# alshai/rowbowt

Hardware: AMD Instinct MI355X
Metric: reads/s (100 bp, count+locate) (higher is better)
Workload: dtype u32/u64

## Files before the change

### include/rbg.h

```cpp
#ifndef RBG_H
#define RBG_H

#include <stddef.h>
#include <stdint.h>

#ifdef __cplusplus
extern "C" {
#endif

#define RBG_ABI_VERSION 3

typedef struct rbg_index rbg_index;

enum { RBG_LOAD_NONE = 0, RBG_LOAD_SA = 1, RBG_LOAD_MA = 2, RBG_LOAD_DL = 4, RBG_LOAD_FT = 8 };

enum {
    RBG_OK = 0,
    RBG_EIO = -1,
    RBG_EFORMAT = -2,
    RBG_ENODEV = -3,
    RBG_EARG = -4,
    RBG_ENOMEM = -5,
    RBG_ENOTLOADED = -6
};

#define RBG_DEVICE_NONE (-1)

int rbg_abi_version(void);
const char *rbg_strerror(int code);


int rbg_load(const char *prefix, int flags, int device, rbg_index **out);

int rbg_build_from_runs(const uint8_t *heads, const uint64_t *lens, uint64_t R,
                        const uint64_t *ssa_y, const uint64_t *esa_y, int device, rbg_index **out);

int rbg_build_from_files(const char *bwt_fname, const char *ssa_fname, const char *esa_fname, int device,
                         rbg_index **out);

int rbg_convert_index(const char *prefix, int flags, const char *out_path);
int rbg_convert_raw(const char *bwt_fname, const char *ssa_fname, const char *esa_fname, const char *mab_fname,
                    const char *docs_fname, const char *out_path);
int rbg_load_cache(const char *path, int flags, int device, rbg_index **out);
int rbg_convert_runs(const uint8_t *heads, const uint64_t *lens, uint64_t R, const uint64_t *ssa_y ,
                     const uint64_t *esa_y, const char *out_path);
int rbg_convert_runs_markers(const uint8_t *heads, const uint64_t *lens, uint64_t R, const uint64_t *ssa_y, const uint64_t *esa_y,
                             const uint64_t *mk_start, const uint64_t *mk_end, uint64_t mk_nruns, const uint64_t *mk_off,
                             const uint64_t *mk_vals, const char *docs_text , const char *out_path);
int rbg_write_ftab(rbg_index *, uint64_t k, const char *path);
int rbg_check_ftab(rbg_index *, const char *path, uint64_t *k_out);
int rbg_set_markers(rbg_index *, const uint64_t *run_start, const uint64_t *run_end, uint64_t nruns,
                    const uint64_t *mk_off, const uint64_t *mk_vals);
int rbg_set_text_markers(rbg_index *, const uint64_t *run_start, const uint64_t *run_end, uint64_t nruns,
                         const uint64_t *mk_off, const uint64_t *mk_vals);
int rbg_load_text_markers(rbg_index *, const char *path);
int rbg_set_docs(rbg_index *, const char *names_joined, const uint64_t *starts, uint64_t ndocs);

void rbg_free(rbg_index *);


typedef struct rbg_info_t {
    uint64_t n;
    uint64_t r;
    uint32_t sigma;
    uint32_t pos_bytes;
    int32_t device;
    uint32_t has_tsa, has_markers, has_docs;
    uint64_t hbm_bytes;
    uint64_t marker_runs, marker_vals;
    uint32_t rank_bucket_shift, phi_bucket_shift;
    uint32_t slot_bytes;
    uint64_t rank_slots, rank_slots_overflow, phi_slots, phi_slots_overflow;
    uint64_t kmer_steps, kmer_symbols, pair_runs, triple_runs, quad_runs;
    uint64_t ftab_k;
    uint64_t quint_runs;
    uint64_t kmer_steps_requested, hbm_free_at_load, hbm_budget;
    uint64_t rank_layout;
    uint64_t replicas;
    uint64_t depth_runs[8];
} rbg_info_t;
enum { RBG_LAYOUT_AUTO = 0, RBG_LAYOUT_SLOTS = 1, RBG_LAYOUT_RUNS = 2, RBG_LAYOUT_PREFER_SLOTS = 3 };
int rbg_info(const rbg_index *, rbg_info_t *out);
int rbg_info_sized(const rbg_index *, rbg_info_t *out, uint64_t out_bytes);

typedef struct rbg_layout_info_t {
    uint32_t run_fmt;
    uint32_t depths_composed;
    uint32_t depth_mask_asked;
    uint32_t depth_mask_kept;
    uint32_t depths_dropped_budget;
    uint32_t rank_directories;
    uint32_t phi_directory;
    uint32_t fill_shift;
    uint64_t entries[8];
    uint64_t fillers[8];
    uint64_t dir_bytes[8];
    uint64_t phi_entries, phi_fillers, phi_dir_bytes, phi_dir_shift;
    uint64_t phi_slots, phi_slot_bytes;
    uint64_t rec_bytes[8];
    uint64_t rec_overflow[8];
    uint64_t budget_raised;
} rbg_layout_info_t;
int rbg_layout_info(const rbg_index *, rbg_layout_info_t *out, uint64_t out_bytes);

typedef struct rbg_jump_info_t {
    uint64_t k;
    uint64_t keys;
    uint64_t bytes;
    uint64_t buckets;
    double build_ms;
} rbg_jump_info_t;
int rbg_jump_info(const rbg_index *, rbg_jump_info_t *out);

int rbg_get_f(const rbg_index *, uint64_t f_out[256]);
int rbg_last_run_sample(const rbg_index *, uint64_t *out);

enum {
    RBG_ARR_RUN_HEADS = 0,
    RBG_ARR_RUN_START = 1,
    RBG_ARR_SAMPLES_LAST = 2,
    RBG_ARR_PRED_POS = 3,
    RBG_ARR_PHI_BASE = 4,
    RBG_ARR_MARKER_START = 5, RBG_ARR_MARKER_END = 6, RBG_ARR_MARKER_OFF = 7, RBG_ARR_MARKER_VALS = 8
};
int rbg_host_array(const rbg_index *, int which, uint64_t *dst, uint64_t cap, uint64_t *count);


int rbg_lf(rbg_index *, const uint64_t *lo, const uint64_t *hi, const uint8_t *sym, uint64_t N,
           uint64_t *lo_out, uint64_t *hi_out);
int rbg_find_range(rbg_index *, const uint8_t *seqs, const uint64_t *off, uint64_t N,
                   uint64_t *lo, uint64_t *hi);
int rbg_count(rbg_index *, const uint8_t *seqs, const uint64_t *off, uint64_t N, uint64_t *count);
int rbg_find_range_spans(rbg_index *, const uint8_t *base, const uint64_t *begin, const uint32_t *len, uint64_t N,
                         uint64_t *lo, uint64_t *hi, uint64_t *ssamp );

int rbg_find_range_w_toehold(rbg_index *, const uint8_t *seqs, const uint64_t *off, uint64_t N,
                             uint64_t *lo, uint64_t *hi, uint64_t *ssamp);
int rbg_locs_at(rbg_index *, const uint64_t *lo, const uint64_t *hi, const uint64_t *k, uint64_t N,
                uint64_t max_hits, uint64_t *loc_off, uint64_t **locs);
int rbg_markers_at(rbg_index *, const uint64_t *lo, const uint64_t *hi, uint64_t N,
                   uint64_t *mk_off, uint64_t **mk);
int rbg_find_range_w_markers(rbg_index *, const uint8_t *seqs, const uint64_t *off, uint64_t N,
                             uint64_t wsize, uint64_t max_range,
                             uint64_t *lo, uint64_t *hi, uint64_t *mk_off, uint64_t **mk);
typedef struct rbg_marker_seed {
    uint64_t lo, hi;
    uint64_t qstart;
    uint64_t qend;
    uint64_t mk_begin;
    uint64_t mk_end;
} rbg_marker_seed_t;
int rbg_get_markers_greedy_seeding(rbg_index *, const uint8_t *seqs, const uint64_t *off, uint64_t N,
                                   uint64_t wsize, uint64_t max_range, uint64_t ftab_k,
                                   uint64_t *seed_off, rbg_marker_seed_t **seeds, uint64_t **mk);
int rbg_get_markers_lmems(rbg_index *, const uint8_t *seqs, const uint64_t *off, uint64_t N,
                          uint64_t wsize, uint64_t max_range, uint64_t ftab_k,
                          uint64_t *seed_off, rbg_marker_seed_t **seeds, uint64_t **mk);
int rbg_greedy_longest_seed(rbg_index *, const uint8_t *seqs, const uint64_t *off, uint64_t N, uint64_t min_length,
                            uint64_t *lo, uint64_t *hi, uint64_t *qstart, uint64_t *qend, uint64_t *ssamp);
#define RBG_SEEDS_W_SAMPLE 1u
int rbg_get_seeds_greedy(rbg_index *, const uint8_t *seqs, const uint64_t *off, uint64_t N, uint64_t min_length, uint32_t flags,
                         uint64_t *seed_off, uint64_t **seeds);
int rbg_find_range_w_toehold_chkpnts(rbg_index *, const uint8_t *seqs, const uint64_t *off, uint64_t N, uint64_t wsize,
                                     uint64_t *seed_off, uint64_t **seeds);
int rbg_find_locs_greedy_seeding(rbg_index *, const uint8_t *seqs, const uint64_t *off, uint64_t N, uint64_t min_length,
                                 uint64_t max_hits, uint64_t *loc_off, uint64_t **locs);
int rbg_markers_at_locs(rbg_index *, const uint64_t *locs, const uint64_t *loc_off, const uint64_t *off, uint64_t N,
                        uint64_t *mk_off, uint64_t **mk);
int rbg_find_loc_markers_greedy_seeding(rbg_index *, const uint8_t *seqs, const uint64_t *off, uint64_t N, uint64_t min_length,
                                        uint64_t max_hits, uint64_t *loc_off, uint64_t **locs, uint64_t *mk_off, uint64_t **mk);
void rbg_free_buffer(void *);

int rbg_resolve_offset(const rbg_index *, uint64_t i, const char **name, uint64_t *offset);
int rbg_doc_table(rbg_index *, uint64_t *ndocs, const uint64_t **sorted_starts, const char *const **names, uint64_t *size);

enum { RBG_TEXT_MARKERS = 1 };
int rbg_align_text(rbg_index *, const uint64_t *lo, const uint64_t *hi, const uint64_t *k, uint64_t N, uint64_t max_hits, uint32_t flags,
                   const char *name_base, const uint64_t *name_begin, const uint32_t *name_len, const char **text, uint64_t *text_len);
int rbg_wait_text(rbg_index *, const char *text);
int rbg_release_text(rbg_index *, const char *text);
int rbg_reserve_text(rbg_index *, uint64_t bytes, int count);
#define RBG_SAM_SECONDARY 1u
int rbg_align_sam(rbg_index *, const char *seq_base, const uint64_t *seq_begin, const uint32_t *seq_len,
                  const char *qual_base , const uint64_t *qual_begin ,
                  const char *name_base, const uint64_t *name_begin, const uint32_t *name_len, uint64_t N,
                  uint64_t min_length, uint64_t max_hits, uint32_t flags, const char **text, uint64_t *text_len);
#define RBG_SAM_MAX_MISMATCH 8
int rbg_align_sam_extend(rbg_index *, const char *seq_base, const uint64_t *seq_begin, const uint32_t *seq_len,
                         const char *qual_base , const uint64_t *qual_begin ,
                         const char *name_base, const uint64_t *name_begin, const uint32_t *name_len, uint64_t N,
                         uint64_t min_length, uint64_t max_hits, uint32_t flags, uint32_t max_mismatch, const char **text, uint64_t *text_len);
typedef struct rbg_extend_t {
    uint32_t ext, nm;
    int32_t score;
    uint32_t steps;
    uint32_t mis_t[8];
    uint8_t mis_ref[8];
} rbg_extend_t;
int rbg_extend_left_dev(rbg_index *, const uint8_t *d_seqs, const uint64_t *d_off, uint64_t N, const uint32_t *d_item_seq ,
                        const uint32_t *d_item_a , const uint64_t *d_item_row , const uint64_t *d_item_limit , uint64_t M,
                        uint32_t max_mismatch, rbg_extend_t *d_out , void *stream);
int rbg_fl_prepare(rbg_index *);
int rbg_fl_info(const rbg_index *, uint64_t out[8]);
int rbg_fl_dev(rbg_index *, const uint64_t *d_rows, uint64_t M, uint8_t *d_sym, uint64_t *d_next, void *stream);
int rbg_extend_right_dev(rbg_index *, const uint8_t *d_seqs, const uint64_t *d_off, uint64_t N, const uint32_t *d_item_seq ,
                         const uint32_t *d_item_b , const uint64_t *d_item_row , const uint32_t *d_item_skip ,
                         const uint64_t *d_item_limit , uint64_t M, uint32_t max_mismatch, rbg_extend_t *d_out , void *stream);
int rbg_align_sam_extend_both(rbg_index *, const char *seq_base, const uint64_t *seq_begin, const uint32_t *seq_len,
                              const char *qual_base , const uint64_t *qual_begin, const char *name_base, const uint64_t *name_begin,
                              const uint32_t *name_len, uint64_t N, uint64_t min_length, uint64_t max_hits, uint32_t flags, uint32_t max_mismatch,
                              const char **text, uint64_t *text_len);
int rbg_sam_header(rbg_index *, const char *pg_line , char **text, uint64_t *text_len);
int rbg_extract_prepare(rbg_index *);
int rbg_extract_info(const rbg_index *, uint64_t out[8]);
int rbg_isa_dev(rbg_index *, const uint64_t *d_pos, uint64_t M, uint64_t *d_row, void *stream);
int rbg_isa(rbg_index *, const uint64_t *pos, uint64_t M, uint64_t *row);
int rbg_extract_dev(rbg_index *, const uint64_t *d_pos, const uint32_t *d_len, const uint64_t *d_out_off, uint64_t M, uint8_t *d_out ,
                    uint32_t *d_got , void *stream);
int rbg_extract(rbg_index *, const uint64_t *pos, const uint64_t *len, uint64_t M, uint8_t *out, uint64_t *got);
size_t rbg_sa_tmp_bytes(uint64_t n, uint32_t pos_bytes);
int rbg_suffix_array_dev(const uint8_t *d_text, uint64_t n, void *d_sa, uint32_t pos_bytes, void *d_tmp, size_t tmp_bytes, void *stream);
int rbg_sa_info(uint64_t out[8]);
size_t rbg_text_runs_tmp_bytes(uint64_t n, uint32_t pos_bytes);
int rbg_text_runs_plan_dev(const uint8_t *d_text, const void *d_sa, uint64_t n, uint32_t pos_bytes, void *d_tmp, size_t tmp_bytes, uint64_t *R, void *stream);
int rbg_text_runs_fill_dev(const uint8_t *d_text, const void *d_sa, uint64_t n, uint32_t pos_bytes, const void *d_tmp, size_t tmp_bytes, uint64_t R,
                           uint8_t *d_heads, uint64_t *d_lens, uint64_t *d_ssa, uint64_t *d_esa, void *stream);
int rbg_build_from_text(const uint8_t *text, uint64_t n, int flags, int device, rbg_index **out);
int rbg_convert_text(const uint8_t *text, uint64_t n, const char *docs_text , int flags, int device, const char *out_path);
#define RBG_REPORT_LMEM 1u
#define RBG_REPORT_HEURISTIC 2u
#define RBG_REPORT_BEST_STRAND 4u
#define RBG_REPORT_CLEAR_CONFLICTING 8u
#define RBG_REPORT_CLEAR_IDENTICAL 16u
typedef struct rbg_report_params {
    uint64_t wsize, max_range, min_range, ftab_k, read_len, min_seed_len;
    uint32_t flags;
} rbg_report_params_t;
typedef struct rbg_report_seed { uint64_t range_size, query_start, query_len, mk_begin, mk_end; uint32_t strand , pad; } rbg_report_seed_t;
int rbg_markers_report(rbg_index *, const uint8_t *seqs, const uint64_t *off, uint64_t N, const uint8_t *first_fwd ,
                       const rbg_report_params_t *params, uint64_t *seed_off, rbg_report_seed_t **seeds, uint64_t **mk);
int rbg_markers_report_text(rbg_index *, const uint8_t *seqs, const uint64_t *off, uint64_t N, const uint8_t *first_fwd ,
                            const rbg_report_params_t *params, const char *name_base, const uint64_t *name_begin, const uint32_t *name_len,
                            const char **text, uint64_t *text_len);
#define RBG_TALLY_PER_READ 1u
#define RBG_TALLY_DROP_SITE_CONFLICTS 2u
typedef struct rbg_tally rbg_tally;
typedef struct rbg_tally_entry { uint64_t marker, n_fwd, n_rev, len_sum; } rbg_tally_entry_t;
int rbg_tally_create(rbg_index *, uint64_t distinct_hint, rbg_tally **out);
void rbg_tally_free(rbg_tally *);
int rbg_tally_reset(rbg_tally *);
int rbg_tally_reserve(rbg_tally *, uint64_t extra);
size_t rbg_tally_add_tmp_bytes(uint64_t R);
int rbg_tally_add_dev(rbg_tally *, const rbg_report_seed_t *d_recs, uint64_t R, const uint64_t *d_mk, uint64_t M_upper, void *d_tmp, size_t tmp_bytes,
                      void *stream);
int rbg_markers_tally(rbg_index *, const uint8_t *seqs, const uint64_t *off, uint64_t N, const uint8_t *first_fwd ,
                      const rbg_report_params_t *params, rbg_tally *);
int rbg_tally_add_entries(rbg_tally *, const rbg_tally_entry_t *entries, uint64_t count);
int rbg_tally_export(rbg_tally *, uint64_t *count, rbg_tally_entry_t **entries);
int rbg_tally_info(rbg_tally *, uint64_t out[6]);
int rbg_markers_tally_reads(rbg_index *, const uint8_t *seqs, const uint64_t *off, uint64_t N, const uint8_t *first_fwd ,
                            const rbg_report_params_t *params, uint32_t tally_flags, rbg_tally *);
size_t rbg_tally_add_reads_tmp_bytes(uint64_t N, uint64_t R);
int rbg_tally_add_reads_dev(rbg_tally *, const rbg_report_seed_t *d_recs, uint64_t R, const uint64_t *d_rep_off , uint64_t N,
                            const uint64_t *d_mk, uint64_t M_upper, uint32_t tally_flags, void *d_tmp, size_t tmp_bytes, void *stream);
int rbg_tally_read_info(rbg_tally *, uint64_t out[4]);

int rbg_find_range_dev(rbg_index *, const uint8_t *d_seqs, const uint64_t *d_off, uint64_t N,
                       uint64_t *d_lo, uint64_t *d_hi, void *stream);
int rbg_find_range_w_toehold_dev(rbg_index *, const uint8_t *d_seqs, const uint64_t *d_off, uint64_t N,
                                 uint64_t *d_lo, uint64_t *d_hi, uint64_t *d_ssamp, void *stream);
size_t rbg_pack_ws_bytes(uint64_t N, uint64_t total_bytes);
int rbg_pack_reads_dev(rbg_index *, const uint8_t *d_seqs, const uint64_t *d_off, uint64_t N, uint64_t total_bytes,
                       void *d_ws, size_t ws_bytes, void *stream);
int rbg_find_range_packed_dev(rbg_index *, const void *d_ws, const uint8_t *d_seqs, const uint64_t *d_off, uint64_t N,
                              uint64_t total_bytes, uint64_t *d_lo, uint64_t *d_hi, void *stream);
int rbg_find_range_w_toehold_packed_dev(rbg_index *, const void *d_ws, const uint8_t *d_seqs, const uint64_t *d_off, uint64_t N,
                                        uint64_t total_bytes, uint64_t *d_lo, uint64_t *d_hi, uint64_t *d_ssamp, void *stream);
size_t rbg_locate_plan_tmp_bytes(uint64_t N);
int rbg_locate_plan_dev(rbg_index *, const uint64_t *d_lo, const uint64_t *d_hi, uint64_t N, uint64_t max_hits,
                        uint64_t *d_loc_off, void *d_tmp, size_t tmp_bytes, void *stream);
size_t rbg_locate_order_ws_bytes(uint64_t N);
int rbg_locate_order_dev(rbg_index *, const uint64_t *d_k, uint64_t N, void *d_ws, size_t ws_bytes, void *stream);
int rbg_locate_fill_dev(rbg_index *, const uint64_t *d_lo, const uint64_t *d_hi, const uint64_t *d_k, uint64_t N,
                        uint64_t max_hits, const uint64_t *d_loc_off, uint64_t *d_locs, const void *d_order, void *stream);
int rbg_locate_fill_dev32(rbg_index *, const uint64_t *d_lo, const uint64_t *d_hi, const uint64_t *d_k, uint64_t N,
                          uint64_t max_hits, const uint64_t *d_loc_off, uint32_t *d_locs32, const void *d_order, void *stream);
int rbg_locate_fill_offset_dev(rbg_index *, const uint64_t *d_lo, const uint64_t *d_hi, const uint64_t *d_k, uint64_t N,
                               uint64_t max_hits, const uint64_t *d_loc_off, uint64_t *d_locs, const uint64_t *d_sub,
                               const void *d_order, void *stream);
int rbg_greedy_longest_seed_dev(rbg_index *, const uint8_t *d_seqs, const uint64_t *d_off, uint64_t N, uint64_t min_length,
                                uint64_t *d_lo, uint64_t *d_hi, uint64_t *d_qstart, uint64_t *d_qend, uint64_t *d_ssamp,
                                void *stream);
int rbg_marker_seeds_plan_dev(rbg_index *, const uint8_t *d_seqs, const uint64_t *d_off, uint64_t N, uint64_t wsize,
                              uint64_t max_range, uint64_t ftab_k, uint64_t *d_seed_off, uint64_t *d_mk_off, void *d_tmp, size_t tmp_bytes,
                              void *stream);
int rbg_marker_seeds_fill_dev(rbg_index *, const uint8_t *d_seqs, const uint64_t *d_off, uint64_t N, uint64_t wsize,
                              uint64_t max_range, uint64_t ftab_k, const uint64_t *d_seed_off, const uint64_t *d_mk_off,
                              rbg_marker_seed_t *d_seeds, uint64_t *d_mk, void *stream);
size_t rbg_marker_seeds_log_bytes(const rbg_index *, uint64_t N, uint32_t seeds_per_read);
int rbg_marker_seeds_plan_log_dev(rbg_index *, const uint8_t *d_seqs, const uint64_t *d_off, uint64_t N, uint64_t wsize,
                                  uint64_t max_range, uint64_t ftab_k, uint64_t *d_seed_off, uint64_t *d_mk_off, void *d_tmp,
                                  size_t tmp_bytes, void *d_log, size_t log_bytes, void *stream);
int rbg_marker_seeds_fill_log_dev(rbg_index *, const uint8_t *d_seqs, const uint64_t *d_off, uint64_t N, uint64_t wsize,
                                  uint64_t max_range, uint64_t ftab_k, const uint64_t *d_seed_off, const uint64_t *d_mk_off,
                                  rbg_marker_seed_t *d_seeds, uint64_t *d_mk, void *d_log, size_t log_bytes, void *stream);
size_t rbg_marker_lmems_tmp_bytes(uint64_t N, uint64_t total);
int rbg_marker_lmems_plan_dev(rbg_index *, const uint8_t *d_seqs, const uint64_t *d_off, uint64_t N, uint64_t total, uint64_t wsize,
                              uint64_t max_range, uint64_t ftab_k, uint64_t *d_mk_off, void *d_tmp, size_t tmp_bytes, void *stream);
int rbg_marker_lmems_fill_dev(rbg_index *, const uint8_t *d_seqs, const uint64_t *d_off, uint64_t N, uint64_t total, uint64_t wsize,
                              uint64_t max_range, uint64_t ftab_k, const void *d_tmp, rbg_marker_seed_t *d_seeds, uint64_t *d_mk, void *stream);
size_t rbg_greedy_seeds_tmp_bytes(uint64_t N);
int rbg_greedy_seeds_plan_dev(rbg_index *, const uint8_t *d_seqs, const uint64_t *d_off, uint64_t N, uint64_t min_length, uint32_t flags,
                              uint64_t *d_seed_off, void *d_tmp, size_t tmp_bytes, void *stream);
int rbg_greedy_seeds_fill_dev(rbg_index *, const uint8_t *d_seqs, const uint64_t *d_off, uint64_t N, uint64_t min_length, uint32_t flags,
                              const uint64_t *d_seed_off, uint64_t *d_lo, uint64_t *d_hi, uint64_t *d_qstart, uint64_t *d_qend,
                              uint64_t *d_ssamp, void *stream);
size_t rbg_toehold_chkpnts_tmp_bytes(uint64_t N);
int rbg_toehold_chkpnts_slots_dev(rbg_index *, const uint64_t *d_off, uint64_t N, uint64_t wsize, uint64_t *d_slot_off, void *d_tmp,
                                  size_t tmp_bytes, void *stream);
int rbg_find_range_w_toehold_chkpnts_dev(rbg_index *, const uint8_t *d_seqs, const uint64_t *d_off, uint64_t N, uint64_t wsize,
                                         const uint64_t *d_slot_off, uint64_t *d_cnt, uint64_t *d_lo, uint64_t *d_hi,
                                         uint64_t *d_qstart, uint64_t *d_qend, uint64_t *d_ssamp, void *stream);
size_t rbg_read_strands_bytes(uint64_t total_bytes);
int rbg_read_strands_dev(rbg_index *, const uint8_t *d_seqs, const uint64_t *d_off, uint64_t N, uint64_t total_bytes, uint8_t *d_seqs2, uint64_t *d_off2,
                         void *stream);
size_t rbg_marker_seeds_canon_tmp_bytes(uint64_t S);
int rbg_marker_seeds_canon_dev(rbg_index *, rbg_marker_seed_t *d_seeds, uint64_t S, uint64_t *d_mk, uint64_t min_range, uint32_t flags, uint64_t read_len,
                               void *d_tmp, size_t tmp_bytes, void *stream);
size_t rbg_report_select_tmp_bytes(uint64_t N);
int rbg_report_select_dev(rbg_index *, const rbg_marker_seed_t *d_seeds, const uint64_t *d_seed_off, const uint64_t *d_off2, uint64_t N,
                          const uint8_t *d_first_fwd, const rbg_report_params_t *params, uint64_t *d_rep_off, rbg_report_seed_t *d_out,
                          uint32_t *d_out_read, void *d_tmp, size_t tmp_bytes, void *stream);
int rbg_markers_plan_dev(rbg_index *, const uint64_t *d_lo, const uint64_t *d_hi, uint64_t N,
                         uint64_t *d_mk_off, void *d_tmp, size_t tmp_bytes, void *stream);
int rbg_markers_fill_dev(rbg_index *, const uint64_t *d_lo, const uint64_t *d_hi, uint64_t N,
                         const uint64_t *d_mk_off, uint64_t *d_mk, void *stream);
size_t rbg_loc_markers_tmp_bytes(uint64_t N);
int rbg_loc_markers_plan_dev(rbg_index *, const uint64_t *d_locs, const uint64_t *d_loc_off, const uint64_t *d_off, uint64_t N,
                             uint64_t *d_mk_off, void *d_tmp, size_t tmp_bytes, void *stream);
int rbg_loc_markers_fill_dev(rbg_index *, const uint64_t *d_locs, const uint64_t *d_loc_off, const uint64_t *d_off, uint64_t N,
                             const uint64_t *d_mk_off, uint64_t *d_mk, void *stream);

#define RBG_DOCS_MAX 65536u
#define RBG_DOC_NONE 0xFFFFFFFFu
int rbg_docs_prepare(rbg_index *);
size_t rbg_doc_hits_words(const rbg_index *);
int rbg_resolve_offsets_dev(rbg_index *, const uint64_t *d_locs, uint64_t M, uint32_t *d_doc, uint64_t *d_offset , void *stream);
int rbg_resolve_offsets_dev32(rbg_index *, const uint32_t *d_locs32, uint64_t M, uint32_t *d_doc, uint64_t *d_offset , void *stream);
int rbg_doc_hits_dev(rbg_index *, const uint64_t *d_locs, const uint64_t *d_loc_off, uint64_t N, uint64_t *d_sets ,
                     uint32_t *d_ndocs , uint32_t *d_nodoc , uint64_t *d_doc_reads ,
                     void *stream);
int rbg_doc_hits_dev32(rbg_index *, const uint32_t *d_locs32, const uint64_t *d_loc_off, uint64_t N, uint64_t *d_sets ,
                       uint32_t *d_ndocs , uint32_t *d_nodoc , uint64_t *d_doc_reads ,
                       void *stream);
int rbg_doc_hits(rbg_index *, const uint8_t *seqs, const uint64_t *off, uint64_t N, uint64_t max_hits, uint64_t *lo, uint64_t *hi, uint64_t *sets ,
                 uint32_t *ndocs , uint32_t *nodoc , uint64_t *doc_reads );
#define RBG_LOCATE_DOCS_MAX 1024u
int rbg_locate_doc_hits_dev(rbg_index *, const uint64_t *d_lo, const uint64_t *d_hi, const uint64_t *d_k, uint64_t N, uint64_t max_hits,
                            const void *d_order , uint64_t *d_sets , uint32_t *d_ndocs ,
                            uint32_t *d_nodoc , uint64_t *d_doc_reads ,
                            uint64_t *d_doc_locs , void *stream);
int rbg_doc_hits_locs(rbg_index *, const uint8_t *seqs, const uint64_t *off, uint64_t N, uint64_t max_hits, uint64_t *lo, uint64_t *hi,
                      uint64_t *sets , uint32_t *ndocs , uint32_t *nodoc ,
                      uint64_t *doc_reads , uint64_t *doc_locs );

int rbg_counters(rbg_index *, uint64_t out[4]);
int rbg_counters_reset(rbg_index *);
int rbg_combine_stats(rbg_index *, uint64_t out[2]);

int rbg_replicate(rbg_index *primary, int device, rbg_index **replica_out);
int rbg_replicate_many(rbg_index *primary, const int *devices, int G, rbg_index **replicas_out );
int rbg_replicate_stats(const rbg_index *replica, double out[3]);
int rbg_replica_pointer_check(const rbg_index *replica, uint64_t out[4]);
int rbg_shard_bounds(uint64_t n_items, int rank, int world, uint64_t *begin, uint64_t *end);
int rbg_find_range_sharded(rbg_index *const *replicas, int G, const uint8_t *seqs, const uint64_t *off, uint64_t N,
                           uint64_t *lo, uint64_t *hi, uint64_t *ssamp );
int rbg_counters_allreduce(rbg_index *, void *nccl_comm, void *stream, uint64_t out[4]);
int rbg_counters_allreduce_local(rbg_index *const *replicas, int G, uint64_t out[4]);
int rbg_comm_cache_clear(void);

enum { RBG_SS_STEPS = 0,
       RBG_SS_SLOTS,
       RBG_SS_DENSE,
       RBG_SS_SEARCH,
       RBG_SS_FTAB,
       RBG_SS_RESAMPLE,
       RBG_SS_CHUNKS,
       RBG_SS_SYMBOLS,
       RBG_SEARCH_STATS };
enum { RBG_LS_PHI_STEPS = 0,
       RBG_LS_PHI_SEARCH,
       RBG_LS_CHAINS,
       RBG_LS_LOCS,
       RBG_LOCATE_STATS };
enum { RBG_SD_MARKER_QUERIES = 8,
       RBG_SD_MARKER_DIR,
       RBG_SD_MARKER_PROBES,
       RBG_SD_MARKER_OFF,
       RBG_SD_MARKER_VALS,
       RBG_SD_SEED_RECS,
       RBG_SD_SEQUENCES,
       RBG_SEED_STATS };
int rbg_greedy_longest_seed_stats_dev(rbg_index *, const uint8_t *d_seqs, const uint64_t *d_off, uint64_t N, uint64_t min_length,
                                      uint64_t *d_lo, uint64_t *d_hi, uint64_t *d_qstart, uint64_t *d_qend, uint64_t *d_ssamp,
                                      uint64_t *d_stats , void *stream);
int rbg_marker_seeds_stats_dev(rbg_index *, const uint8_t *d_seqs, const uint64_t *d_off, uint64_t N, uint64_t wsize, uint64_t max_range,
                               uint64_t *d_seed_off, uint64_t *d_mk_off, void *d_tmp, size_t tmp_bytes, rbg_marker_seed_t *d_seeds,
                               uint64_t *d_mk, uint64_t *d_stats , void *stream);
int rbg_find_range_stats_dev(rbg_index *, const uint8_t *d_seqs, const uint64_t *d_off, uint64_t N, uint64_t *d_lo,
                             uint64_t *d_hi, uint64_t *d_ssamp ,
                             uint64_t *d_stats , void *stream);
int rbg_locate_fill_stats_dev(rbg_index *, const uint64_t *d_lo, const uint64_t *d_hi, const uint64_t *d_k, uint64_t N,
                              uint64_t max_hits, const uint64_t *d_loc_off, uint64_t *d_locs, const void *d_order,
                              uint64_t *d_stats , void *stream);

int rbg_sample_reads_dev(const uint8_t *d_text, uint64_t unit, uint64_t H, uint64_t L, uint64_t m, uint64_t seed,
                         uint64_t first_read, uint64_t N, uint32_t sub_ppm, uint8_t *d_seqs, uint64_t *d_off,
                         uint64_t *d_start , void *stream);
int rbg_sample_reads_pangenome_dev(const uint8_t *d_base, const uint64_t *d_sites, const uint8_t *d_alt, const uint8_t *d_G, uint64_t S,
                                   const uint32_t *d_site_dir, uint32_t site_dir_shift, uint64_t unit, uint64_t H, uint64_t L, uint64_t m,
                                   uint64_t seed, uint64_t first_read, uint64_t N, uint32_t sub_ppm, uint8_t *d_seqs, uint64_t *d_off,
                                   uint64_t *d_start , void *stream);

enum { RBG_OPT_BLOCK_THREADS = 1, RBG_OPT_RANK_BUCKET_SHIFT = 2, RBG_OPT_PHI_BUCKET_SHIFT = 3, RBG_OPT_POS_BYTES = 4,
       RBG_OPT_KMER_STEPS = 5, RBG_OPT_HBM_BUDGET_MB = 6, RBG_OPT_FTAB_K = 7, RBG_OPT_PACKED_READS = 8,
       RBG_OPT_DEEP_BUCKET_SHIFT = 9, RBG_OPT_DENSE_OVERFLOW = 10, RBG_OPT_RANK_LAYOUT = 11,
       RBG_OPT_RUN_DEPTHS = 14 ,
       RBG_OPT_RUN_PHI = 16 ,
       RBG_OPT_RUN_REC = 17 ,
       RBG_OPT_RUN_REC_DEPTHS = 18 ,
       RBG_OPT_EXTRACT_CHUNK = 20 ,
       RBG_OPT_JUMP_K = 19  };
int rbg_set_default_option(int opt, int64_t value);
int rbg_get_default_option(int opt, int64_t *value);

#ifdef __cplusplus
}
#endif
#endif
```

### rowbowt_amd/capi.py

```python
import ctypes as C
import enum
import os
import weakref

import numpy as np

_HERE = os.path.dirname(os.path.abspath(__file__))
_SO = os.path.join(_HERE, "librbg.so")

U64 = C.c_uint64
VP = C.c_void_p
MAXU = 2**64 - 1
DEVICE_NONE = -1

OPT_BLOCK_THREADS, OPT_RANK_BUCKET_SHIFT, OPT_PHI_BUCKET_SHIFT, OPT_POS_BYTES, OPT_KMER_STEPS, OPT_HBM_BUDGET_MB, OPT_FTAB_K, OPT_PACKED_READS, OPT_DEEP_BUCKET_SHIFT, OPT_DENSE_OVERFLOW, OPT_RANK_LAYOUT = range(1, 12)
OPT_RUN_DEPTHS, OPT_RUN_PHI, OPT_RUN_REC, OPT_RUN_REC_DEPTHS = 14, 16, 17, 18
OPT_EXTRACT_CHUNK = 20
OPT_JUMP_K = 19
ABI_VERSION = 3
MAX_KMER_DEPTH = 8
LAYOUT_AUTO, LAYOUT_SLOTS, LAYOUT_RUNS, LAYOUT_PREFER_SLOTS = 0, 1, 2, 3
SEEDS_W_SAMPLE = 1
(ARR_RUN_HEADS, ARR_RUN_START, ARR_SAMPLES_LAST, ARR_PRED_POS, ARR_PHI_BASE,
 ARR_MARKER_START, ARR_MARKER_END, ARR_MARKER_OFF, ARR_MARKER_VALS) = range(9)


class LoadRbwtFlag(enum.IntFlag):
    NONE = 0
    SA = 1
    MA = 2
    DL = 4
    FT = 8


class RbgError(RuntimeError):
    def __init__(self, code, what):
        self.code = code
        super().__init__(f"{what}: {lib().rbg_strerror(code).decode()} ({code})")


class Info(C.Structure):
    _fields_ = [("n", U64), ("r", U64), ("sigma", C.c_uint32), ("pos_bytes", C.c_uint32), ("device", C.c_int32),
                ("has_tsa", C.c_uint32), ("has_markers", C.c_uint32), ("has_docs", C.c_uint32),
                ("hbm_bytes", U64), ("marker_runs", U64), ("marker_vals", U64),
                ("rank_bucket_shift", C.c_uint32), ("phi_bucket_shift", C.c_uint32), ("slot_bytes", C.c_uint32),
                ("rank_slots", U64), ("rank_slots_overflow", U64), ("phi_slots", U64), ("phi_slots_overflow", U64),
                ("kmer_steps", U64), ("kmer_symbols", U64), ("pair_runs", U64), ("triple_runs", U64), ("quad_runs", U64), ("ftab_k", U64), ("quint_runs", U64),
                ("kmer_steps_requested", U64), ("hbm_free_at_load", U64), ("hbm_budget", U64), ("rank_layout", U64), ("replicas", U64),
                ("depth_runs", U64 * 8)]


class LayoutInfo(C.Structure):
    _fields_ = [("run_fmt", C.c_uint32), ("depths_composed", C.c_uint32), ("depth_mask_asked", C.c_uint32), ("depth_mask_kept", C.c_uint32),
                ("depths_dropped_budget", C.c_uint32), ("rank_directories", C.c_uint32),
                ("phi_directory", C.c_uint32), ("fill_shift", C.c_uint32),
                ("entries", U64 * 8), ("fillers", U64 * 8), ("dir_bytes", U64 * 8),
                ("phi_entries", U64), ("phi_fillers", U64), ("phi_dir_bytes", U64), ("phi_dir_shift", U64), ("phi_slots", U64), ("phi_slot_bytes", U64), ("rec_bytes", U64 * 8), ("rec_overflow", U64 * 8), ("budget_raised", U64)]


class JumpInfo(C.Structure):
    _fields_ = [("k", U64), ("keys", U64), ("bytes", U64), ("buckets", U64), ("build_ms", C.c_double)]


class ReportParams(C.Structure):
    _fields_ = [(n, U64) for n in ("wsize", "max_range", "min_range", "ftab_k", "read_len", "min_seed_len")] + [("flags", C.c_uint32)]


REPORT_LMEM, REPORT_HEURISTIC, REPORT_BEST_STRAND, REPORT_CLEAR_CONFLICTING, REPORT_CLEAR_IDENTICAL = 1, 2, 4, 8, 16
REPORT_SEED = np.dtype([("range_size", "<u8"), ("query_start", "<u8"), ("query_len", "<u8"), ("mk_begin", "<u8"), ("mk_end", "<u8"),
                        ("strand", "<u4"), ("pad", "<u4")])


TALLY_ENTRY = np.dtype([("marker", "<u8"), ("n_fwd", "<u8"), ("n_rev", "<u8"), ("len_sum", "<u8")])
TALLY_INFO = ("entries", "capacity", "grows", "records", "elements", "dropped")
TALLY_PER_READ, TALLY_DROP_SITE_CONFLICTS = 1, 2
TALLY_READ_INFO = ("reads", "elements_seen", "lost", "site_dropped")
DOCS_MAX = 1 << 16
SAM_MAX_MISMATCH = 8
EXTEND = np.dtype([("ext", np.uint32), ("nm", np.uint32), ("score", np.int32), ("steps", np.uint32), ("mis_t", np.uint32, 8), ("mis_ref", np.uint8, 8)])
SAM_SECONDARY = 1
LOCATE_DOCS_MAX = 1024
DOC_NONE = 0xFFFFFFFF


def report_params(wsize=19, max_range=1000, min_range=0, ftab_k=0, read_len=101, min_seed_len=0, lmem=False, heuristic=False, best_strand=False,
                  clear_conflicting=False, clear_identical=False):
    flags = ((REPORT_LMEM if lmem else 0) | (REPORT_HEURISTIC if heuristic else 0) | (REPORT_BEST_STRAND if best_strand else 0)
             | (REPORT_CLEAR_CONFLICTING if clear_conflicting else 0) | (REPORT_CLEAR_IDENTICAL if clear_identical else 0))
    return ReportParams(wsize, max_range & MAXU, min_range, ftab_k, read_len, min_seed_len, flags)


_PROTOS = [
    ("rbg_abi_version", C.c_int, []),
    ("rbg_strerror", C.c_char_p, [C.c_int]),
    ("rbg_load", C.c_int, [C.c_char_p, C.c_int, C.c_int, C.POINTER(VP)]),
    ("rbg_build_from_runs", C.c_int, [VP, VP, U64, VP, VP, C.c_int, C.POINTER(VP)]),
    ("rbg_build_from_files", C.c_int, [C.c_char_p, C.c_char_p, C.c_char_p, C.c_int, C.POINTER(VP)]),
    ("rbg_convert_index", C.c_int, [C.c_char_p, C.c_int, C.c_char_p]),
    ("rbg_convert_raw", C.c_int, [C.c_char_p, C.c_char_p, C.c_char_p, C.c_char_p, C.c_char_p, C.c_char_p]),
    ("rbg_load_cache", C.c_int, [C.c_char_p, C.c_int, C.c_int, C.POINTER(VP)]),
    ("rbg_doc_table", C.c_int, [VP, C.POINTER(U64), C.POINTER(VP), C.POINTER(VP), C.POINTER(U64)]),
    ("rbg_align_text", C.c_int, [VP, VP, VP, VP, U64, U64, C.c_uint32, VP, VP, VP, C.POINTER(VP), C.POINTER(U64)]),
    ("rbg_wait_text", C.c_int, [VP, VP]),
    ("rbg_release_text", C.c_int, [VP, VP]),
    ("rbg_reserve_text", C.c_int, [VP, U64, C.c_int]),
    ("rbg_convert_runs", C.c_int, [VP, VP, U64, VP, VP, C.c_char_p]),
    ("rbg_convert_runs_markers", C.c_int, [VP, VP, U64, VP, VP, VP, VP, U64, VP, VP, C.c_char_p, C.c_char_p]),
    ("rbg_write_ftab", C.c_int, [VP, U64, C.c_char_p]),
    ("rbg_check_ftab", C.c_int, [VP, C.c_char_p, C.POINTER(U64)]),
    ("rbg_set_markers", C.c_int, [VP, VP, VP, U64, VP, VP]),
    ("rbg_set_docs", C.c_int, [VP, C.c_char_p, VP, U64]),
    ("rbg_free", None, [VP]),
    ("rbg_info", C.c_int, [VP, C.POINTER(Info)]),
    ("rbg_info_sized", C.c_int, [VP, C.POINTER(Info), U64]),
    ("rbg_layout_info", C.c_int, [VP, C.POINTER(LayoutInfo), U64]),
    ("rbg_jump_info", C.c_int, [VP, C.POINTER(JumpInfo)]),
    ("rbg_get_f", C.c_int, [VP, VP]),
    ("rbg_last_run_sample", C.c_int, [VP, C.POINTER(U64)]),
    ("rbg_host_array", C.c_int, [VP, C.c_int, VP, U64, C.POINTER(U64)]),
    ("rbg_lf", C.c_int, [VP, VP, VP, VP, U64, VP, VP]),
    ("rbg_find_range", C.c_int, [VP, VP, VP, U64, VP, VP]),
    ("rbg_count", C.c_int, [VP, VP, VP, U64, VP]),
    ("rbg_find_range_w_toehold", C.c_int, [VP, VP, VP, U64, VP, VP, VP]),
    ("rbg_find_range_spans", C.c_int, [VP, VP, VP, VP, U64, VP, VP, VP]),
    ("rbg_locs_at", C.c_int, [VP, VP, VP, VP, U64, U64, VP, C.POINTER(VP)]),
    ("rbg_markers_at", C.c_int, [VP, VP, VP, U64, VP, C.POINTER(VP)]),
    ("rbg_find_range_w_markers", C.c_int, [VP, VP, VP, U64, U64, U64, VP, VP, VP, C.POINTER(VP)]),
    ("rbg_get_markers_greedy_seeding", C.c_int, [VP, VP, VP, U64, U64, U64, U64, VP, C.POINTER(VP), C.POINTER(VP)]),
    ("rbg_greedy_longest_seed", C.c_int, [VP, VP, VP, U64, U64, VP, VP, VP, VP, VP]),
    ("rbg_find_locs_greedy_seeding", C.c_int, [VP, VP, VP, U64, U64, U64, VP, C.POINTER(VP)]),
    ("rbg_free_buffer", None, [VP]),
    ("rbg_resolve_offset", C.c_int, [VP, U64, C.POINTER(C.c_char_p), C.POINTER(U64)]),
    ("rbg_find_range_dev", C.c_int, [VP, VP, VP, U64, VP, VP, VP]),
    ("rbg_find_range_w_toehold_dev", C.c_int, [VP, VP, VP, U64, VP, VP, VP, VP]),
    ("rbg_pack_ws_bytes", C.c_size_t, [U64, U64]),
    ("rbg_pack_reads_dev", C.c_int, [VP, VP, VP, U64, U64, VP, C.c_size_t, VP]),
    ("rbg_find_range_packed_dev", C.c_int, [VP, VP, VP, VP, U64, U64, VP, VP, VP]),
    ("rbg_find_range_w_toehold_packed_dev", C.c_int, [VP, VP, VP, VP, U64, U64, VP, VP, VP, VP]),
    ("rbg_locate_plan_tmp_bytes", C.c_size_t, [U64]),
    ("rbg_locate_plan_dev", C.c_int, [VP, VP, VP, U64, U64, VP, VP, C.c_size_t, VP]),
    ("rbg_locate_order_ws_bytes", C.c_size_t, [U64]),
    ("rbg_locate_order_dev", C.c_int, [VP, VP, U64, VP, C.c_size_t, VP]),
    ("rbg_locate_fill_dev", C.c_int, [VP, VP, VP, VP, U64, U64, VP, VP, VP, VP]),
    ("rbg_locate_fill_offset_dev", C.c_int, [VP, VP, VP, VP, U64, U64, VP, VP, VP, VP, VP]),
    ("rbg_greedy_longest_seed_dev", C.c_int, [VP, VP, VP, U64, U64, VP, VP, VP, VP, VP, VP]),
    ("rbg_marker_seeds_plan_dev", C.c_int, [VP, VP, VP, U64, U64, U64, U64, VP, VP, VP, C.c_size_t, VP]),
    ("rbg_marker_seeds_fill_dev", C.c_int, [VP, VP, VP, U64, U64, U64, U64, VP, VP, VP, VP, VP]),
    ("rbg_markers_plan_dev", C.c_int, [VP, VP, VP, U64, VP, VP, C.c_size_t, VP]),
    ("rbg_markers_fill_dev", C.c_int, [VP, VP, VP, U64, VP, VP, VP]),
    ("rbg_marker_seeds_log_bytes", C.c_size_t, [VP, U64, C.c_uint32]),
    ("rbg_marker_seeds_plan_log_dev", C.c_int, [VP, VP, VP, U64, U64, U64, U64, VP, VP, VP, C.c_size_t, VP, C.c_size_t, VP]),
    ("rbg_marker_seeds_fill_log_dev", C.c_int, [VP, VP, VP, U64, U64, U64, U64, VP, VP, VP, VP, VP, C.c_size_t, VP]),
    ("rbg_locate_fill_dev32", C.c_int, [VP, VP, VP, VP, U64, U64, VP, VP, VP, VP]),
    ("rbg_greedy_longest_seed_stats_dev", C.c_int, [VP, VP, VP, U64, U64, VP, VP, VP, VP, VP, VP, VP]),
    ("rbg_marker_seeds_stats_dev", C.c_int, [VP, VP, VP, U64, U64, U64, VP, VP, VP, C.c_size_t, VP, VP, VP, VP]),
    ("rbg_find_range_stats_dev", C.c_int, [VP, VP, VP, U64, VP, VP, VP, VP, VP]),
    ("rbg_locate_fill_stats_dev", C.c_int, [VP, VP, VP, VP, U64, U64, VP, VP, VP, VP, VP]),
    ("rbg_sample_reads_dev", C.c_int, [VP, U64, U64, U64, U64, U64, U64, U64, C.c_uint32, VP, VP, VP, VP]),
    ("rbg_sample_reads_pangenome_dev", C.c_int, [VP, VP, VP, VP, U64, VP, C.c_uint32, U64, U64, U64, U64, U64, U64, U64, C.c_uint32, VP, VP, VP, VP]),
    ("rbg_replicate", C.c_int, [VP, C.c_int, C.POINTER(VP)]),
    ("rbg_replicate_many", C.c_int, [VP, C.POINTER(C.c_int), C.c_int, C.POINTER(VP)]),
    ("rbg_replicate_stats", C.c_int, [VP, C.POINTER(C.c_double)]),
    ("rbg_replica_pointer_check", C.c_int, [VP, VP]),
    ("rbg_comm_cache_clear", C.c_int, []),
    ("rbg_shard_bounds", C.c_int, [U64, C.c_int, C.c_int, C.POINTER(U64), C.POINTER(U64)]),
    ("rbg_find_range_sharded", C.c_int, [VP, C.c_int, VP, VP, U64, VP, VP, VP]),
    ("rbg_counters_allreduce", C.c_int, [VP, VP, VP, VP]),
    ("rbg_counters_allreduce_local", C.c_int, [VP, C.c_int, VP]),
    ("rbg_counters", C.c_int, [VP, VP]),
    ("rbg_counters_reset", C.c_int, [VP]),
    ("rbg_combine_stats", C.c_int, [VP, VP]),
    ("rbg_get_markers_lmems", C.c_int, [VP, VP, VP, U64, U64, U64, U64, VP, C.POINTER(VP), C.POINTER(VP)]),
    ("rbg_marker_lmems_tmp_bytes", C.c_size_t, [U64, U64]),
    ("rbg_marker_lmems_plan_dev", C.c_int, [VP, VP, VP, U64, U64, U64, U64, U64, VP, VP, C.c_size_t, VP]),
    ("rbg_marker_lmems_fill_dev", C.c_int, [VP, VP, VP, U64, U64, U64, U64, U64, VP, VP, VP, VP]),
    ("rbg_get_seeds_greedy", C.c_int, [VP, VP, VP, U64, U64, C.c_uint32, VP, C.POINTER(VP)]),
    ("rbg_greedy_seeds_tmp_bytes", C.c_size_t, [U64]),
    ("rbg_greedy_seeds_plan_dev", C.c_int, [VP, VP, VP, U64, U64, C.c_uint32, VP, VP, C.c_size_t, VP]),
    ("rbg_greedy_seeds_fill_dev", C.c_int, [VP, VP, VP, U64, U64, C.c_uint32, VP, VP, VP, VP, VP, VP, VP]),
    ("rbg_find_range_w_toehold_chkpnts", C.c_int, [VP, VP, VP, U64, U64, VP, C.POINTER(VP)]),
    ("rbg_toehold_chkpnts_tmp_bytes", C.c_size_t, [U64]),
    ("rbg_toehold_chkpnts_slots_dev", C.c_int, [VP, VP, U64, U64, VP, VP, C.c_size_t, VP]),
    ("rbg_find_range_w_toehold_chkpnts_dev", C.c_int, [VP, VP, VP, U64, U64, VP, VP, VP, VP, VP, VP, VP, VP]),
    ("rbg_set_text_markers", C.c_int, [VP, VP, VP, U64, VP, VP]),
    ("rbg_load_text_markers", C.c_int, [VP, C.c_char_p]),
    ("rbg_loc_markers_tmp_bytes", C.c_size_t, [U64]),
    ("rbg_loc_markers_plan_dev", C.c_int, [VP, VP, VP, VP, U64, VP, VP, C.c_size_t, VP]),
    ("rbg_loc_markers_fill_dev", C.c_int, [VP, VP, VP, VP, U64, VP, VP, VP]),
    ("rbg_markers_at_locs", C.c_int, [VP, VP, VP, VP, U64, VP, C.POINTER(VP)]),
    ("rbg_find_loc_markers_greedy_seeding", C.c_int, [VP, VP, VP, U64, U64, U64, VP, C.POINTER(VP), VP, C.POINTER(VP)]),
    ("rbg_read_strands_bytes", C.c_size_t, [U64]),
    ("rbg_read_strands_dev", C.c_int, [VP, VP, VP, U64, U64, VP, VP, VP]),
    ("rbg_marker_seeds_canon_tmp_bytes", C.c_size_t, [U64]),
    ("rbg_marker_seeds_canon_dev", C.c_int, [VP, VP, U64, VP, U64, C.c_uint32, U64, VP, C.c_size_t, VP]),
    ("rbg_report_select_tmp_bytes", C.c_size_t, [U64]),
    ("rbg_report_select_dev", C.c_int, [VP, VP, VP, VP, U64, VP, VP, VP, VP, VP, VP, C.c_size_t, VP]),
    ("rbg_markers_report", C.c_int, [VP, VP, VP, U64, VP, VP, VP, C.POINTER(VP), C.POINTER(VP)]),
    ("rbg_markers_report_text", C.c_int, [VP, VP, VP, U64, VP, VP, VP, VP, VP, C.POINTER(VP), C.POINTER(U64)]),
    ("rbg_tally_create", C.c_int, [VP, U64, C.POINTER(VP)]),
    ("rbg_tally_free", None, [VP]),
    ("rbg_tally_reset", C.c_int, [VP]),
    ("rbg_tally_reserve", C.c_int, [VP, U64]),
    ("rbg_tally_add_tmp_bytes", C.c_size_t, [U64]),
    ("rbg_tally_add_dev", C.c_int, [VP, VP, U64, VP, U64, VP, C.c_size_t, VP]),
    ("rbg_markers_tally", C.c_int, [VP, VP, VP, U64, VP, VP, VP]),
    ("rbg_tally_add_entries", C.c_int, [VP, VP, U64]),
    ("rbg_tally_export", C.c_int, [VP, C.POINTER(U64), C.POINTER(VP)]),
    ("rbg_tally_info", C.c_int, [VP, VP]),
    ("rbg_markers_tally_reads", C.c_int, [VP, VP, VP, U64, VP, VP, C.c_uint32, VP]),
    ("rbg_tally_add_reads_tmp_bytes", C.c_size_t, [U64, U64]),
    ("rbg_tally_add_reads_dev", C.c_int, [VP, VP, U64, VP, U64, VP, U64, C.c_uint32, VP, C.c_size_t, VP]),
    ("rbg_tally_read_info", C.c_int, [VP, VP]),
    ("rbg_docs_prepare", C.c_int, [VP]),
    ("rbg_doc_hits_words", C.c_size_t, [VP]),
    ("rbg_resolve_offsets_dev", C.c_int, [VP, VP, U64, VP, VP, VP]),
    ("rbg_resolve_offsets_dev32", C.c_int, [VP, VP, U64, VP, VP, VP]),
    ("rbg_doc_hits_dev", C.c_int, [VP, VP, VP, U64, VP, VP, VP, VP, VP]),
    ("rbg_doc_hits_dev32", C.c_int, [VP, VP, VP, U64, VP, VP, VP, VP, VP]),
    ("rbg_doc_hits", C.c_int, [VP, VP, VP, U64, U64, VP, VP, VP, VP, VP, VP]),
    ("rbg_locate_doc_hits_dev", C.c_int, [VP, VP, VP, VP, U64, U64, VP, VP, VP, VP, VP, VP, VP]),
    ("rbg_doc_hits_locs", C.c_int, [VP, VP, VP, U64, U64, VP, VP, VP, VP, VP, VP, VP]),
    ("rbg_align_sam", C.c_int, [VP, VP, VP, VP, VP, VP, VP, VP, VP, U64, U64, U64, C.c_uint32, C.POINTER(VP), C.POINTER(U64)]),
    ("rbg_sam_header", C.c_int, [VP, C.c_char_p, C.POINTER(VP), C.POINTER(U64)]),
    ("rbg_align_sam_extend", C.c_int, [VP, VP, VP, VP, VP, VP, VP, VP, VP, U64, U64, U64, C.c_uint32, C.c_uint32, C.POINTER(VP), C.POINTER(U64)]),
    ("rbg_extend_left_dev", C.c_int, [VP, VP, VP, U64, VP, VP, VP, VP, U64, C.c_uint32, VP, VP]),
    ("rbg_fl_prepare", C.c_int, [VP]),
    ("rbg_fl_info", C.c_int, [VP, VP]),
    ("rbg_fl_dev", C.c_int, [VP, VP, U64, VP, VP, VP]),
    ("rbg_extend_right_dev", C.c_int, [VP, VP, VP, U64, VP, VP, VP, VP, VP, U64, C.c_uint32, VP, VP]),
    ("rbg_align_sam_extend_both", C.c_int, [VP, VP, VP, VP, VP, VP, VP, VP, VP, U64, U64, U64, C.c_uint32, C.c_uint32, C.POINTER(VP), C.POINTER(U64)]),
    ("rbg_extract_prepare", C.c_int, [VP]),
    ("rbg_extract_info", C.c_int, [VP, VP]),
    ("rbg_isa_dev", C.c_int, [VP, VP, U64, VP, VP]),
    ("rbg_isa", C.c_int, [VP, VP, U64, VP]),
    ("rbg_extract_dev", C.c_int, [VP, VP, VP, VP, U64, VP, VP, VP]),
    ("rbg_extract", C.c_int, [VP, VP, VP, U64, VP, VP]),
    ("rbg_sa_tmp_bytes", C.c_size_t, [U64, C.c_uint32]),
    ("rbg_suffix_array_dev", C.c_int, [VP, U64, VP, C.c_uint32, VP, C.c_size_t, VP]),
    ("rbg_sa_info", C.c_int, [VP]),
    ("rbg_text_runs_tmp_bytes", C.c_size_t, [U64, C.c_uint32]),
    ("rbg_text_runs_plan_dev", C.c_int, [VP, VP, U64, C.c_uint32, VP, C.c_size_t, C.POINTER(U64), VP]),
    ("rbg_text_runs_fill_dev", C.c_int, [VP, VP, U64, C.c_uint32, VP, C.c_size_t, U64, VP, VP, VP, VP, VP]),
    ("rbg_build_from_text", C.c_int, [VP, U64, C.c_int, C.c_int, C.POINTER(VP)]),
    ("rbg_convert_text", C.c_int, [VP, U64, C.c_char_p, C.c_int, C.c_int, C.c_char_p]),
    ("rbg_set_default_option", C.c_int, [C.c_int, C.c_int64]),
    ("rbg_get_default_option", C.c_int, [C.c_int, C.POINTER(C.c_int64)]),
]
EXPORTS = [p[0] for p in _PROTOS]
_OPTIONAL = {"rbg_jump_info"}

_lib = None


def _one_hip_runtime():
    import importlib.util
    import sys
    if "torch" in sys.modules or os.environ.get("RBG_NO_TORCH_PRELOAD") == "1":
        return
    try:
        if importlib.util.find_spec("torch") is not None:
            import torch
    except Exception:
        pass


def lib():
    global _lib
    if _lib is None:
        if not os.path.exists(_SO):
            raise ImportError(f"{_SO} is missing: build it with `make -C rowbowt_amd/csrc` "
                              "(or __graft_entry__.build()); there is no CPU fallback")
        _one_hip_runtime()
        L = C.CDLL(_SO)
        L.rbg_abi_version.restype = C.c_int
        L.rbg_abi_version.argtypes = []
        have = L.rbg_abi_version()
        if have != ABI_VERSION:
            raise ImportError(f"{_SO} reports ABI {have}, this binding is written against ABI {ABI_VERSION}: rebuild it with `make -C rowbowt_amd/csrc`")
        for name, res, args in _PROTOS:
            if name in _OPTIONAL and not hasattr(L, name):
                continue
            fn = getattr(L, name)
            fn.restype = res
            fn.argtypes = args
        _lib = L
    return _lib


def _check(rc, what):
    if rc != 0:
        raise RbgError(rc, what)


def _p(a):
    return a.ctypes.data_as(VP) if a is not None else None


def _u64(a):
    return np.ascontiguousarray(a, dtype=np.uint64)


def pack_reads(reads):
    off = np.zeros(len(reads) + 1, dtype=np.uint64)
    if len(reads):
        off[1:] = np.cumsum([len(r) for r in reads], dtype=np.uint64)
    seqs = np.frombuffer(b"".join(reads), dtype=np.uint8).copy() if len(reads) else np.zeros(0, np.uint8)
    return seqs, off


def convert_index(prefix, flags, out_path):
    _check(lib().rbg_convert_index(os.fsencode(prefix), int(flags), os.fsencode(out_path)), "rbg_convert_index")


def convert_raw(bwt, ssa=None, esa=None, mab=None, docs=None, out_path=None):
    e = lambda x: os.fsencode(x) if x else None
    _check(lib().rbg_convert_raw(e(bwt), e(ssa), e(esa), e(mab), e(docs), e(out_path)), "rbg_convert_raw")


def convert_runs(heads, lens, ssa=None, esa=None, out_path=None, markers=None, docs_text=None):
    heads = np.ascontiguousarray(heads, dtype=np.uint8)
    lens = np.ascontiguousarray(lens, dtype=np.uint64)
    ssa = None if ssa is None else np.ascontiguousarray(ssa, dtype=np.uint64)
    esa = None if esa is None else np.ascontiguousarray(esa, dtype=np.uint64)
    mk = [None] * 4 if markers is None else [np.ascontiguousarray(a, dtype=np.uint64) for a in markers]
    _check(lib().rbg_convert_runs_markers(_p(heads), _p(lens), len(heads), _p(ssa) if ssa is not None else None, _p(esa) if esa is not None else None,
                                          _p(mk[0]) if markers is not None else None, _p(mk[1]) if markers is not None else None,
                                          len(mk[0]) if markers is not None else 0, _p(mk[2]) if markers is not None else None,
                                          _p(mk[3]) if markers is not None else None, docs_text.encode() if docs_text else None,
                                          os.fsencode(out_path)), "rbg_convert_runs_markers")


SA_INFO = ("rounds", "sorted", "tmp_bytes", "n", "pos_bytes", "tied_after_first")


def _text_bytes(text):
    return np.frombuffer(text, dtype=np.uint8) if isinstance(text, (bytes, bytearray, memoryview)) else np.ascontiguousarray(text, dtype=np.uint8)


def convert_text(text, out_path, docs_text=None, sa=True, device=0):
    t = _text_bytes(text)
    _check(lib().rbg_convert_text(_p(t), len(t), docs_text.encode() if docs_text else None, int(LoadRbwtFlag.SA) if sa else 0, device, os.fsencode(out_path)),
           "rbg_convert_text")


def sa_info():
    out = np.zeros(8, np.uint64)
    _check(lib().rbg_sa_info(_p(out)), "rbg_sa_info")
    return {k: int(v) for k, v in zip(SA_INFO, out)}


def _pos_bytes_of(n, pos_bytes):
    return pos_bytes or (8 if n >= 0xFFFFFFF0 else 4)


def suffix_array(text, pos_bytes=0):
    import torch
    n = int(text.numel())
    pb = _pos_bytes_of(n, pos_bytes)
    assert text.dtype == torch.uint8 and text.is_contiguous()
    with torch.cuda.device(text.device):
        sa = torch.empty(max(n, 1), dtype=torch.int32 if pb == 4 else torch.int64, device=text.device)
        nb = lib().rbg_sa_tmp_bytes(n, pb)
        tmp = torch.empty(nb + 256, dtype=torch.uint8, device=text.device)
        at = (-tmp.data_ptr()) % 256
        rc = lib().rbg_suffix_array_dev(text.data_ptr() if n else None, n, sa.data_ptr(), pb, tmp.data_ptr() + at, nb, torch.cuda.current_stream().cuda_stream)
        torch.cuda.synchronize()
    _check(rc, "rbg_suffix_array_dev")
    return sa[:n]


def text_runs(text, sa):
    import torch
    n = int(text.numel())
    pb = sa.element_size()
    assert text.dtype == torch.uint8 and text.is_contiguous() and sa.is_contiguous() and int(sa.numel()) == n and pb in (4, 8)
    L = lib()
    with torch.cuda.device(text.device):
        nb = L.rbg_text_runs_tmp_bytes(n, pb)
        tmp = torch.empty(nb + 256, dtype=torch.uint8, device=text.device)
        at = (-tmp.data_ptr()) % 256
        st = torch.cuda.current_stream().cuda_stream
        R = U64()
        _check(L.rbg_text_runs_plan_dev(text.data_ptr(), sa.data_ptr(), n, pb, tmp.data_ptr() + at, nb, C.byref(R), st), "rbg_text_runs_plan_dev")
        r = int(R.value)
        heads = torch.empty(r, dtype=torch.uint8, device=text.device)
        lens, ssa, esa = (torch.empty(r, dtype=torch.int64, device=text.device) for _ in range(3))
        rc = L.rbg_text_runs_fill_dev(text.data_ptr(), sa.data_ptr(), n, pb, tmp.data_ptr() + at, nb, r, heads.data_ptr(), lens.data_ptr(), ssa.data_ptr(),
                                      esa.data_ptr(), st)
        torch.cuda.synchronize()
    _check(rc, "rbg_text_runs_fill_dev")
    u = lambda t: t.cpu().numpy().view(np.uint64).copy()
    return dict(heads=heads.cpu().numpy().copy(), lens=u(lens), ssa=u(ssa), esa=u(esa), n=n, r=r)


def set_default_option(opt, value):
    _check(lib().rbg_set_default_option(opt, value), "rbg_set_default_option")


def get_default_option(opt):
    v = C.c_int64(0)
    _check(lib().rbg_get_default_option(opt, C.byref(v)), "rbg_get_default_option")
    return int(v.value)


class default_option:

    def __init__(self, opt, value):
        self.opt, self.value = opt, value

    def __enter__(self):
        self.prev = get_default_option(self.opt)
        set_default_option(self.opt, self.value)
        return self

    def __exit__(self, *exc):
        set_default_option(self.opt, self.prev)
        return False


def _take(ptr, n):
    if n == 0 or not ptr.value:
        lib().rbg_free_buffer(ptr)
        return np.zeros(0, dtype=np.uint64)
    mem = (C.c_char * (n * 8)).from_address(ptr.value)
    weakref.finalize(mem, lib().rbg_free_buffer, VP(ptr.value))
    return np.frombuffer(mem, dtype=np.uint64)


class Tally:

    def __init__(self, rb, distinct_hint=0):
        self.L = lib()
        self.rb = rb
        self.h = VP()
        _check(self.L.rbg_tally_create(rb.h, distinct_hint, C.byref(self.h)), "rbg_tally_create")

    def close(self):
        if self.h:
            self.L.rbg_tally_free(self.h)
            self.h = None

    def __del__(self):
        try:
            if self.rb.h:
                self.close()
        except Exception:
            pass

    def reset(self):
        _check(self.L.rbg_tally_reset(self.h), "rbg_tally_reset")

    def reserve(self, extra):
        _check(self.L.rbg_tally_reserve(self.h, extra), "rbg_tally_reserve")

    def add_entries(self, entries):
        e = np.ascontiguousarray(entries, dtype=TALLY_ENTRY)
        _check(self.L.rbg_tally_add_entries(self.h, _p(e), len(e)), "rbg_tally_add_entries")

    def export(self):
        n, ptr = U64(), VP()
        _check(self.L.rbg_tally_export(self.h, C.byref(n), C.byref(ptr)), "rbg_tally_export")
        return _take(ptr, 4 * n.value).view(TALLY_ENTRY)

    def info(self):
        out = np.zeros(6, np.uint64)
        _check(self.L.rbg_tally_info(self.h, _p(out)), "rbg_tally_info")
        return dict(zip(TALLY_INFO, (int(v) for v in out)))

    def read_info(self):
        out = np.zeros(4, np.uint64)
        _check(self.L.rbg_tally_read_info(self.h, _p(out)), "rbg_tally_read_info")
        return dict(zip(TALLY_READ_INFO, (int(v) for v in out)))


class RowBowt:

    def __init__(self, handle):
        self.h = handle
        self.L = lib()

    def close(self):
        if self.h:
            self.L.rbg_free(self.h)
            self.h = None

    def __del__(self):
        try:
            self.close()
        except Exception:
            pass

    @classmethod
    def from_runs(cls, heads, lens, ssa=None, esa=None, device=0):
        heads = np.ascontiguousarray(heads, dtype=np.uint8)
        lens = _u64(lens)
        ssa = _u64(ssa) if ssa is not None else None
        esa = _u64(esa) if esa is not None else None
        h = VP()
        _check(lib().rbg_build_from_runs(_p(heads), _p(lens), len(heads), _p(ssa), _p(esa), device, C.byref(h)),
               "rbg_build_from_runs")
        return cls(h)

    @classmethod
    def from_text(cls, text, sa=True, device=0):
        t = _text_bytes(text)
        h = VP()
        _check(lib().rbg_build_from_text(_p(t), len(t), int(LoadRbwtFlag.SA) if sa else 0, device, C.byref(h)), "rbg_build_from_text")
        return cls(h)

    @classmethod
    def from_files(cls, bwt, ssa=None, esa=None, device=0):
        h = VP()
        _check(lib().rbg_build_from_files(os.fsencode(bwt), os.fsencode(ssa) if ssa else None,
                                          os.fsencode(esa) if esa else None, device, C.byref(h)), "rbg_build_from_files")
        return cls(h)

    def set_markers(self, run_start, run_end, mk_off, mk_vals):
        a = [_u64(v) for v in (run_start, run_end, mk_off, mk_vals)]
        _check(self.L.rbg_set_markers(self.h, _p(a[0]), _p(a[1]), len(a[0]), _p(a[2]), _p(a[3])), "rbg_set_markers")

    def set_text_markers(self, run_start, run_end, mk_off, mk_vals):
        a = [_u64(v) for v in (run_start, run_end, mk_off, mk_vals)]
        _check(self.L.rbg_set_text_markers(self.h, _p(a[0]), _p(a[1]), len(a[0]), _p(a[2]), _p(a[3])), "rbg_set_text_markers")

    def load_text_markers(self, path):
        _check(self.L.rbg_load_text_markers(self.h, os.fsencode(path)), f"rbg_load_text_markers({path})")

    def set_docs(self, names, starts):
        joined = b"\0".join(n.encode() for n in names) + b"\0"
        s = _u64(starts)
        _check(self.L.rbg_set_docs(self.h, joined, _p(s), len(names)), "rbg_set_docs")

    @classmethod
    def from_cache(cls, path, flags=LoadRbwtFlag.NONE, device=0):
        h = VP()
        _check(lib().rbg_load_cache(os.fsencode(path), int(flags), device, C.byref(h)), "rbg_load_cache")
        return cls(h)

    def write_ftab(self, k, path):
        _check(self.L.rbg_write_ftab(self.h, k, os.fsencode(path)), "rbg_write_ftab")

    def check_ftab(self, path):
        k = U64()
        _check(self.L.rbg_check_ftab(self.h, os.fsencode(path), C.byref(k)), "rbg_check_ftab")
        return k.value

    def info(self):
        i = Info()
        _check(self.L.rbg_info(self.h, C.byref(i)), "rbg_info")
        return i

    def jump_info(self):
        i = JumpInfo()
        _check(self.L.rbg_jump_info(self.h, C.byref(i)), "rbg_jump_info")
        return i

    def layout_info(self):
        i = LayoutInfo()
        _check(self.L.rbg_layout_info(self.h, C.byref(i), C.sizeof(i)), "rbg_layout_info")
        return i

    def get_f(self):
        out = np.zeros(256, dtype=np.uint64)
        _check(self.L.rbg_get_f(self.h, _p(out)), "rbg_get_f")
        return out

    def last_run_sample(self):
        v = U64()
        _check(self.L.rbg_last_run_sample(self.h, C.byref(v)), "rbg_last_run_sample")
        return v.value

    def host_array(self, which):
        cnt = U64()
        _check(self.L.rbg_host_array(self.h, which, None, 0, C.byref(cnt)), "rbg_host_array")
        out = np.zeros(cnt.value, dtype=np.uint64)
        _check(self.L.rbg_host_array(self.h, which, _p(out), cnt.value, C.byref(cnt)), "rbg_host_array")
        return out

    def LF(self, lo, hi, sym):
        lo, hi = _u64(lo), _u64(hi)
        sym = np.ascontiguousarray(sym, dtype=np.uint8)
        N = len(lo)
        nlo, nhi = np.zeros(N, np.uint64), np.zeros(N, np.uint64)
        _check(self.L.rbg_lf(self.h, _p(lo), _p(hi), _p(sym), N, _p(nlo), _p(nhi)), "rbg_lf")
        return nlo, nhi

    def find_range(self, seqs, off):
        N = len(off) - 1
        lo, hi = np.zeros(N, np.uint64), np.zeros(N, np.uint64)
        _check(self.L.rbg_find_range(self.h, _p(seqs), _p(off), N, _p(lo), _p(hi)), "rbg_find_range")
        return lo, hi

    def count(self, seqs, off):
        N = len(off) - 1
        cnt = np.zeros(N, np.uint64)
        _check(self.L.rbg_count(self.h, _p(seqs), _p(off), N, _p(cnt)), "rbg_count")
        return cnt

    def find_range_spans(self, buf, begin, length, toehold=False):
        buf = np.ascontiguousarray(buf, dtype=np.uint8)
        begin = _u64(begin)
        length = np.ascontiguousarray(length, dtype=np.uint32)
        N = len(begin)
        lo, hi = np.zeros(N, np.uint64), np.zeros(N, np.uint64)
        k = np.zeros(N, np.uint64) if toehold else None
        _check(self.L.rbg_find_range_spans(self.h, _p(buf), _p(begin), _p(length), N, _p(lo), _p(hi), _p(k)), "rbg_find_range_spans")
        return (lo, hi, k) if toehold else (lo, hi)

    def find_range_w_toehold(self, seqs, off):
        N = len(off) - 1
        lo, hi, k = np.zeros(N, np.uint64), np.zeros(N, np.uint64), np.zeros(N, np.uint64)
        _check(self.L.rbg_find_range_w_toehold(self.h, _p(seqs), _p(off), N, _p(lo), _p(hi), _p(k)),
               "rbg_find_range_w_toehold")
        return lo, hi, k

    def locs_at(self, lo, hi, k, max_hits=MAXU):
        lo, hi, k = _u64(lo), _u64(hi), _u64(k)
        N = len(lo)
        loc_off = np.zeros(N + 1, np.uint64)
        ptr = VP()
        _check(self.L.rbg_locs_at(self.h, _p(lo), _p(hi), _p(k), N, max_hits, _p(loc_off), C.byref(ptr)), "rbg_locs_at")
        return loc_off, _take(ptr, int(loc_off[N]))

    def markers_at(self, lo, hi):
        lo, hi = _u64(lo), _u64(hi)
        N = len(lo)
        mk_off = np.zeros(N + 1, np.uint64)
        ptr = VP()
        _check(self.L.rbg_markers_at(self.h, _p(lo), _p(hi), N, _p(mk_off), C.byref(ptr)), "rbg_markers_at")
        return mk_off, _take(ptr, int(mk_off[N]))

    def find_range_w_markers(self, seqs, off, wsize, max_range=MAXU):
        N = len(off) - 1
        lo, hi, mk_off = np.zeros(N, np.uint64), np.zeros(N, np.uint64), np.zeros(N + 1, np.uint64)
        ptr = VP()
        _check(self.L.rbg_find_range_w_markers(self.h, _p(seqs), _p(off), N, wsize, max_range & MAXU,
                                               _p(lo), _p(hi), _p(mk_off), C.byref(ptr)), "rbg_find_range_w_markers")
        return lo, hi, mk_off, _take(ptr, int(mk_off[N]))

    def get_markers_greedy_seeding(self, seqs, off, wsize, max_range=MAXU, ftab_k=0):
        N = len(off) - 1
        seed_off = np.zeros(N + 1, np.uint64)
        ps, pm = VP(), VP()
        _check(self.L.rbg_get_markers_greedy_seeding(self.h, _p(seqs), _p(off), N, wsize, max_range & MAXU, ftab_k, _p(seed_off),
                                                     C.byref(ps), C.byref(pm)), "rbg_get_markers_greedy_seeding")
        S = int(seed_off[N])
        seeds = _take(ps, 6 * S).reshape(S, 6)
        nmk = int(seeds[-1, 5]) if S else 0
        return seed_off, seeds, _take(pm, nmk)

    def get_markers_lmems(self, seqs, off, wsize, max_range=MAXU, ftab_k=0):
        N = len(off) - 1
        seed_off = np.zeros(N + 1, np.uint64)
        ps, pm = VP(), VP()
        _check(self.L.rbg_get_markers_lmems(self.h, _p(seqs), _p(off), N, wsize, max_range & MAXU, ftab_k, _p(seed_off),
                                            C.byref(ps), C.byref(pm)), "rbg_get_markers_lmems")
        S = int(seed_off[N])
        seeds = _take(ps, 6 * S).reshape(S, 6)
        nmk = int(seeds[-1, 5]) if S else 0
        return seed_off, seeds, _take(pm, nmk)

    def _seed_arrays(self, seed_off, ptr):
        S = int(seed_off[-1])
        a = _take(ptr, 5 * S).reshape(5, S)
        return (seed_off,) + tuple(a[t] for t in range(5))

    def get_seeds_greedy(self, seqs, off, min_length, w_sample=True):
        N = len(off) - 1
        seed_off = np.zeros(N + 1, np.uint64)
        ptr = VP()
        _check(self.L.rbg_get_seeds_greedy(self.h, _p(seqs), _p(off), N, min_length, SEEDS_W_SAMPLE if w_sample else 0, _p(seed_off),
                                           C.byref(ptr)), "rbg_get_seeds_greedy")
        return self._seed_arrays(seed_off, ptr)

    def find_range_w_toehold_chkpnts(self, seqs, off, wsize):
        N = len(off) - 1
        seed_off = np.zeros(N + 1, np.uint64)
        ptr = VP()
        _check(self.L.rbg_find_range_w_toehold_chkpnts(self.h, _p(seqs), _p(off), N, wsize, _p(seed_off), C.byref(ptr)),
               "rbg_find_range_w_toehold_chkpnts")
        return self._seed_arrays(seed_off, ptr)

    def greedy_longest_seed(self, seqs, off, min_length):
        N = len(off) - 1
        a = [np.zeros(N, np.uint64) for _ in range(5)]
        _check(self.L.rbg_greedy_longest_seed(self.h, _p(seqs), _p(off), N, min_length, *[_p(x) for x in a]),
               "rbg_greedy_longest_seed")
        return a

    def find_locs_greedy_seeding(self, seqs, off, min_length, max_hits=MAXU):
        N = len(off) - 1
        loc_off = np.zeros(N + 1, np.uint64)
        ptr = VP()
        _check(self.L.rbg_find_locs_greedy_seeding(self.h, _p(seqs), _p(off), N, min_length, max_hits, _p(loc_off), C.byref(ptr)),
               "rbg_find_locs_greedy_seeding")
        return loc_off, _take(ptr, int(loc_off[N]))

    def markers_at_locs(self, locs, loc_off, off):
        locs, loc_off, off = _u64(locs), _u64(loc_off), _u64(off)
        N = len(off) - 1
        mk_off = np.zeros(N + 1, np.uint64)
        ptr = VP()
        _check(self.L.rbg_markers_at_locs(self.h, _p(locs), _p(loc_off), _p(off), N, _p(mk_off), C.byref(ptr)), "rbg_markers_at_locs")
        return mk_off, _take(ptr, int(mk_off[N]))

    def find_loc_markers_greedy_seeding(self, seqs, off, min_length, max_hits=MAXU):
        N = len(off) - 1
        loc_off, mk_off = np.zeros(N + 1, np.uint64), np.zeros(N + 1, np.uint64)
        lp, mp = VP(), VP()
        _check(self.L.rbg_find_loc_markers_greedy_seeding(self.h, _p(seqs), _p(off), N, min_length, max_hits, _p(loc_off), C.byref(lp),
                                                          _p(mk_off), C.byref(mp)), "rbg_find_loc_markers_greedy_seeding")
        return loc_off, _take(lp, int(loc_off[N])), mk_off, _take(mp, int(mk_off[N]))

    def resolve_offset(self, i):
        name, off = C.c_char_p(), U64()
        _check(self.L.rbg_resolve_offset(self.h, i, C.byref(name), C.byref(off)), "rbg_resolve_offset")
        return name.value.decode(), off.value

    def docs_prepare(self):
        _check(self.L.rbg_docs_prepare(self.h), "rbg_docs_prepare")

    def doc_hits_words(self):
        return int(self.L.rbg_doc_hits_words(self.h))

    def resolve_offsets(self, locs):
        import torch
        locs = _u64(locs)
        M = len(locs)
        self.docs_prepare()
        info = self.info()
        with torch.cuda.device(info.device):
            d_locs = torch.from_numpy(locs.view(np.int64)).cuda()
            d_doc = torch.empty(max(M, 1), dtype=torch.int32, device="cuda")
            d_off = torch.empty(max(M, 1), dtype=torch.int64, device="cuda")
            st = torch.cuda.current_stream().cuda_stream
            _check(self.L.rbg_resolve_offsets_dev(self.h, d_locs.data_ptr() if M else None, M, d_doc.data_ptr(), d_off.data_ptr(), st), "rbg_resolve_offsets_dev")
            torch.cuda.synchronize()
            return d_doc[:M].cpu().numpy().view(np.uint32), d_off[:M].cpu().numpy().view(np.uint64)

    def locate_doc_hits(self, d_lo, d_hi, d_k, max_hits=MAXU, order=True, doc_locs=False):
        import torch
        N = int(d_lo.numel())
        W = self.doc_hits_words()
        nd = self.doc_table(names=False)[0]
        with torch.cuda.device(d_lo.device):
            st = torch.cuda.current_stream().cuda_stream
            ws = None
            if order and N:
                ws_bytes = int(self.L.rbg_locate_order_ws_bytes(N))
                ws = torch.empty(ws_bytes, dtype=torch.uint8, device=d_lo.device)
                _check(self.L.rbg_locate_order_dev(self.h, d_k.data_ptr(), N, ws.data_ptr(), ws_bytes, st), "rbg_locate_order_dev")
            sets = torch.zeros((N, W), dtype=torch.int64, device=d_lo.device)
            ndocs, nodoc = (torch.zeros(N, dtype=torch.int32, device=d_lo.device) for _ in range(2))
            reads = torch.zeros(nd, dtype=torch.int64, device=d_lo.device)
            locs = torch.zeros(nd, dtype=torch.int64, device=d_lo.device) if doc_locs else None
            _check(self.L.rbg_locate_doc_hits_dev(self.h, d_lo.data_ptr(), d_hi.data_ptr(), d_k.data_ptr(), N, max_hits, ws.data_ptr() if ws is not None else None,
                                                  sets.data_ptr(), ndocs.data_ptr(), nodoc.data_ptr(), reads.data_ptr(),
                                                  locs.data_ptr() if doc_locs else None, st), "rbg_locate_doc_hits_dev")
        return (sets, ndocs, nodoc, reads, locs) if doc_locs else (sets, ndocs, nodoc, reads)

    def doc_hits(self, seqs, off, max_hits=MAXU, doc_locs=False):
        seqs, off = np.ascontiguousarray(seqs, dtype=np.uint8), _u64(off)
        N = len(off) - 1
        self.docs_prepare()
        W = self.doc_hits_words()
        nd = self.doc_table(names=False)[0]
        lo, hi = np.zeros(N, np.uint64), np.zeros(N, np.uint64)
        sets = np.zeros((N, W), np.uint64)
        ndocs, nodoc = np.zeros(N, np.uint32), np.zeros(N, np.uint32)
        doc_reads = np.zeros(nd, np.uint64)
        if doc_locs:
            dl = np.zeros(nd, np.uint64)
            _check(self.L.rbg_doc_hits_locs(self.h, _p(seqs), _p(off), N, max_hits, _p(lo), _p(hi), _p(sets), _p(ndocs), _p(nodoc), _p(doc_reads), _p(dl)),
                   "rbg_doc_hits_locs")
            return lo, hi, sets, ndocs, nodoc, doc_reads, dl
        _check(self.L.rbg_doc_hits(self.h, _p(seqs), _p(off), N, max_hits, _p(lo), _p(hi), _p(sets), _p(ndocs), _p(nodoc), _p(doc_reads)), "rbg_doc_hits")
        return lo, hi, sets, ndocs, nodoc, doc_reads

    def doc_table(self, names=True):
        nd, size, ps, pn = U64(), U64(), VP(), VP()
        _check(self.L.rbg_doc_table(self.h, C.byref(nd), C.byref(ps), C.byref(pn), C.byref(size)), "rbg_doc_table")
        n = int(nd.value)
        starts = np.ctypeslib.as_array(C.cast(ps, C.POINTER(U64)), shape=(n,)).copy()
        got = [C.cast(pn, C.POINTER(C.c_char_p))[j].decode() for j in range(n)] if names else None
        return n, starts, got, int(size.value)

    def align_text(self, lo, hi, k, names, max_hits=MAXU, markers=False):
        lo, hi = (np.ascontiguousarray(a, dtype=np.uint64) for a in (lo, hi))
        k = None if k is None else np.ascontiguousarray(k, dtype=np.uint64)
        blob = b"".join(names)
        nlen = np.array([len(x) for x in names], dtype=np.uint32)
        nbeg = np.zeros(len(names), dtype=np.uint64)
        if len(names) > 1:
            nbeg[1:] = np.cumsum(nlen[:-1], dtype=np.uint64)
        buf = C.create_string_buffer(blob, len(blob) + 1)
        text, n = VP(), U64()
        _check(self.L.rbg_align_text(self.h, _p(lo), _p(hi), _p(k) if k is not None else None, len(names), max_hits, 1 if markers else 0, buf, _p(nbeg), _p(nlen), C.byref(text), C.byref(n)), "rbg_align_text")
        try:
            _check(self.L.rbg_wait_text(self.h, text), "rbg_wait_text")
            return C.string_at(text, n.value)
        finally:
            self.L.rbg_release_text(self.h, text)

    def align_sam_extend(self, seqs, quals, names, min_length=20, max_hits=16, secondary=False, max_mismatch=4, right=False):
        return self._sam_lines(seqs, quals, names, min_length, max_hits, secondary, max_mismatch, right)

    def fl_prepare(self):
        _check(self.L.rbg_fl_prepare(self.h), "rbg_fl_prepare")

    def fl_info(self):
        out = np.zeros(8, np.uint64)
        _check(self.L.rbg_fl_info(self.h, _p(out)), "rbg_fl_info")
        return dict(prepared=bool(out[0]), bytes=int(out[1]), runs=[int(v) for v in out[2:6]], shift=[(int(out[6]) >> (8 * j)) & 0xFF for j in range(4)],
                    dir_entries=int(out[7]))

    def fl(self, rows):
        import torch
        rows = _u64(rows)
        M = len(rows)
        with torch.cuda.device(self.info().device):
            d_rows = torch.from_numpy(rows.view(np.int64)).cuda()
            d_sym = torch.full((max(M, 1),), 0xA5, dtype=torch.uint8, device="cuda")
            d_next = torch.full((max(M, 1),), -6, dtype=torch.int64, device="cuda")
            rc = self.L.rbg_fl_dev(self.h, d_rows.data_ptr() if M else None, M, d_sym.data_ptr(), d_next.data_ptr(), torch.cuda.current_stream().cuda_stream)
            torch.cuda.synchronize()
            sym, nxt = d_sym.cpu().numpy()[:M].copy(), d_next.cpu().numpy()[:M].view(np.uint64).copy()
        _check(rc, "rbg_fl_dev")
        return sym, nxt

    def extract_prepare(self):
        _check(self.L.rbg_extract_prepare(self.h), "rbg_extract_prepare")

    def extract_info(self):
        out = np.zeros(8, np.uint64)
        _check(self.L.rbg_extract_info(self.h, _p(out)), "rbg_extract_info")
        keys = ("bytes", "samples", "shift", "dir_entries", "second_kind", "max_gap", "build_us")
        return dict(prepared=bool(out[0]), **{k: int(v) for k, v in zip(keys, out[1:])})

    def isa(self, pos):
        import torch
        pos = _u64(pos)
        M = len(pos)
        with torch.cuda.device(self.info().device):
            d_pos = torch.from_numpy(pos.view(np.int64)).cuda()
            d_row = torch.full((max(M, 1),), -6, dtype=torch.int64, device="cuda")
            rc = self.L.rbg_isa_dev(self.h, d_pos.data_ptr() if M else None, M, d_row.data_ptr(), torch.cuda.current_stream().cuda_stream)
            torch.cuda.synchronize()
            row = d_row.cpu().numpy()[:M].view(np.uint64).copy()
        _check(rc, "rbg_isa_dev")
        return row

    def extract_dev(self, d_pos, d_len, d_out_off, d_out, d_got):
        import torch
        M = int(d_pos.numel())
        assert int(d_len.numel()) == M and int(d_out_off.numel()) == M and int(d_got.numel()) >= M
        assert d_pos.element_size() == 8 and d_out_off.element_size() == 8 and d_len.element_size() == 4 and d_got.element_size() == 4 and d_out.element_size() == 1
        with torch.cuda.device(self.info().device):
# ... 209 lines not shown
```

### rowbowt_amd/csrc/k_jump.hip

```cpp
#include "rbg_device.hpp"
#include "rbg_jump.h"

namespace rbg {
namespace {

__global__ __launch_bounds__(256) void k_jump_expand(const uint64_t *__restrict__ plo, const uint64_t *__restrict__ phi, const uint64_t base,
                                                     const uint64_t cnt, const uint8_t *__restrict__ major_byte, uint64_t *__restrict__ clo,
                                                     uint64_t *__restrict__ chi, uint8_t *__restrict__ sym) {
    const uint64_t stride = static_cast<uint64_t>(gridDim.x) * blockDim.x;
    for (uint64_t j = static_cast<uint64_t>(blockIdx.x) * blockDim.x + threadIdx.x; j < 4 * cnt; j += stride) {
        const uint64_t par = base + (j >> 2);
        clo[j] = plo[par];
        chi[j] = phi[par];
        sym[j] = major_byte[j & 3u];
    }
}

__global__ __launch_bounds__(256) void k_jump_keep(const uint64_t *__restrict__ nlo, const uint64_t *__restrict__ nhi, const uint4 *__restrict__ pkey,
                                                   const uint64_t base, const uint64_t N, const uint32_t level, uint64_t *__restrict__ olo,
                                                   uint64_t *__restrict__ ohi, uint4 *__restrict__ okey, unsigned long long *__restrict__ count) {
    const uint32_t lane = threadIdx.x & (kWave - 1);
    const uint64_t stride = static_cast<uint64_t>(gridDim.x) * blockDim.x;
    for (uint64_t wb = static_cast<uint64_t>(blockIdx.x) * blockDim.x + (threadIdx.x & ~(kWave - 1)); wb < N; wb += stride) {
        const uint64_t j = wb + lane;
        const bool keep = j < N && nlo[j] <= nhi[j];
        const uint64_t bal = __ballot(keep);
        unsigned long long at = 0;
        if (lane == 0 && bal) at = atomicAdd(count, static_cast<unsigned long long>(__popcll(bal)));
        at = __shfl(at, 0);
        if (keep) {
            const uint64_t o = at + static_cast<uint64_t>(__popcll(bal & ((uint64_t(1) << lane) - 1u)));
            uint4 kk = pkey[base + (j >> 2)];
            JumpKey key{{kk.x, kk.y, kk.z, kk.w}};
            jump_key_set(key, level, static_cast<uint32_t>(j & 3u));
            olo[o] = nlo[j];
            ohi[o] = nhi[j];
            okey[o] = make_uint4(key.w[0], key.w[1], key.w[2], key.w[3]);
        }
    }
}

__global__ __launch_bounds__(256) void k_jump_meta(const uint64_t cnt, const uint32_t K, uint2 *__restrict__ meta) {
    const uint64_t stride = static_cast<uint64_t>(gridDim.x) * blockDim.x;
    for (uint64_t i = static_cast<uint64_t>(blockIdx.x) * blockDim.x + threadIdx.x; i < cnt; i += stride)
        meta[i] = make_uint2(static_cast<uint32_t>(i), K);
}

__global__ __launch_bounds__(256) void k_jump_insert(const uint4 *__restrict__ keys, const uint64_t *__restrict__ lo, const uint64_t *__restrict__ hi,
                                                     const uint64_t *__restrict__ ss, const uint64_t cnt, uint32_t *__restrict__ tab, const uint64_t nb,
                                                     unsigned long long *__restrict__ inserted) {
    const uint64_t stride = static_cast<uint64_t>(gridDim.x) * blockDim.x;
    for (uint64_t i = static_cast<uint64_t>(blockIdx.x) * blockDim.x + threadIdx.x; i < cnt; i += stride) {
        const uint64_t l = lo[i], h = hi[i], k = ss ? ss[i] : 0;
        if (l > h || h > 0xFFFFFFFFull) continue;
        uint32_t kk;
        if (k == ~uint64_t(0)) kk = 0xFFFFFFFFu;
        else if (k >= 0xFFFFFFF0ull) continue;
        else kk = static_cast<uint32_t>(k);
        const uint4 kw = keys[i];
        const JumpKey key{{kw.x, kw.y, kw.z, kw.w}};
        uint64_t b = jump_home(jump_hash(key), nb);
        for (uint64_t step = 0; step < nb; ++step) {
            bool done = false;
            for (uint32_t s = 0; s < 2 && !done; ++s) {
                uint32_t *slot = tab + (2 * b + s) * kJumpSlotWords;
                if (atomicCAS(slot + 7, kJumpEmptyTag, kJumpFullTag) == kJumpEmptyTag) {
                    reinterpret_cast<uint4 *>(slot)[0] = kw;
                    reinterpret_cast<uint4 *>(slot)[1] = make_uint4(static_cast<uint32_t>(l), static_cast<uint32_t>(h), kk, kJumpFullTag);
                    done = true;
                }
            }
            if (done) { atomicAdd(inserted, 1ull); break; }
            b = b + 1 == nb ? 0 : b + 1;
        }
    }
}

struct DevBuf {
    void *p = nullptr;
    size_t bytes = 0;
    ~DevBuf() { if (p) (void)hipFree(p); }
    hipError_t alloc(size_t b) { bytes = b; return hipMalloc(&p, b ? b : 1); }
    template <typename T> T *as() const { return static_cast<T *>(p); }
};

}

constexpr uint64_t kJumpChunkParents = uint64_t(1) << 24;

int launch_build_jump(const DevIndex &ix, const LaunchCfg &cfg, uint32_t K, uint64_t table_budget, uint64_t peak_budget, void **tab,
                      uint64_t *tab_bytes, uint64_t *buckets, uint64_t *keys, const char **why, void *stream) {
    *tab = nullptr; *tab_bytes = 0; *buckets = 0; *keys = 0; *why = nullptr;
    if (ix.pos_bytes != 4) { *why = "8-byte positions (the table holds 4-byte states)"; return 0; }
    if (ix.layout != 2 || ix.nmajor != 4 || !ix.stage_ok) { *why = "only the staged search of the run-indexed layout over four major symbols uses it"; return 0; }
    if (K < kJumpMinK || K > kJumpMaxK) return static_cast<int>(hipErrorInvalidValue);
    hipStream_t st = static_cast<hipStream_t>(stream);
    DevIndex plain = ix;
    plain.jump = nullptr;
    plain.jump_buckets = 0;
    plain.jump_k = 0;
    uint64_t C = kJumpChunkParents;
    while (C > (uint64_t(1) << 12) && 4 * C * 33 > peak_budget / 4) C >>= 1;
    if (4 * C * 33 + 1024 > peak_budget) { *why = "its build scratch exceeds what the HBM budget leaves"; return 0; }
    DevBuf clo, chi, nlo, nhi, sym, mb, cnt_d;
    DevBuf lv_lo[2], lv_hi[2], lv_key[2];
    uint64_t cap[2] = {0, 0};
    hipError_t e = hipSuccess;
    auto scratch = [&]() {
        return clo.bytes + chi.bytes + nlo.bytes + nhi.bytes + sym.bytes + 32 * (cap[0] + cap[1]);
    };
    bool over = false;
    auto grow = [&](int w, uint64_t need, uint64_t used) -> hipError_t {
        if (need <= cap[w]) return hipSuccess;
        const uint64_t nc = std::max<uint64_t>(need, cap[w] + cap[w] / 2);
        if (scratch() + 32 * nc > peak_budget) { over = true; return hipSuccess; }
        DevBuf a, b, c;
        hipError_t r = a.alloc(nc * 8);
        if (r == hipSuccess) r = b.alloc(nc * 8);
        if (r == hipSuccess) r = c.alloc(nc * 16);
        if (r == hipSuccess && used) r = hipMemcpyAsync(a.p, lv_lo[w].p, used * 8, hipMemcpyDeviceToDevice, st);
        if (r == hipSuccess && used) r = hipMemcpyAsync(b.p, lv_hi[w].p, used * 8, hipMemcpyDeviceToDevice, st);
        if (r == hipSuccess && used) r = hipMemcpyAsync(c.p, lv_key[w].p, used * 16, hipMemcpyDeviceToDevice, st);
        if (r == hipSuccess) r = hipStreamSynchronize(st);
        if (r != hipSuccess) return r;
        std::swap(lv_lo[w].p, a.p); std::swap(lv_lo[w].bytes, a.bytes);
        std::swap(lv_hi[w].p, b.p); std::swap(lv_hi[w].bytes, b.bytes);
        std::swap(lv_key[w].p, c.p); std::swap(lv_key[w].bytes, c.bytes);
        cap[w] = nc;
        return hipSuccess;
    };
    e = clo.alloc(4 * C * 8);
    if (e == hipSuccess) e = chi.alloc(4 * C * 8);
    if (e == hipSuccess) e = nlo.alloc(4 * C * 8);
    if (e == hipSuccess) e = nhi.alloc(4 * C * 8);
    if (e == hipSuccess) e = sym.alloc(4 * C);
    if (e == hipSuccess) e = mb.alloc(256);
    if (e == hipSuccess) e = cnt_d.alloc(2 * sizeof(unsigned long long));
    if (e == hipSuccess) {
        uint8_t lut2[256], inv[256] = {0};
        e = hipMemcpy(lut2, ix.lut2, 256, hipMemcpyDeviceToHost);
        for (int b = 0; b < 256; ++b)
            if (lut2[b] != 0xFF) inv[lut2[b] & 3u] = static_cast<uint8_t>(b);
        if (e == hipSuccess) e = hipMemcpy(mb.p, inv, 256, hipMemcpyHostToDevice);
    }
    if (e == hipSuccess) e = grow(0, 1, 0);
    if (e == hipSuccess && over) { *why = "its build scratch exceeds what the HBM budget leaves"; return 0; }
    if (e == hipSuccess) {
        const uint64_t lo0 = 0, hi0 = ix.n - 1;
        const uint4 k0 = make_uint4(0, 0, 0, 0);
        e = hipMemcpy(lv_lo[0].p, &lo0, 8, hipMemcpyHostToDevice);
        if (e == hipSuccess) e = hipMemcpy(lv_hi[0].p, &hi0, 8, hipMemcpyHostToDevice);
        if (e == hipSuccess) e = hipMemcpy(lv_key[0].p, &k0, 16, hipMemcpyHostToDevice);
    }
    if (e != hipSuccess) return static_cast<int>(e);
    uint64_t F = 1;
    int cur = 0;
    for (uint32_t level = 0; level < K; ++level) {
        const int nx = cur ^ 1;
        const unsigned long long zero = 0;
        if ((e = hipMemcpy(cnt_d.p, &zero, sizeof(zero), hipMemcpyHostToDevice)) != hipSuccess) return static_cast<int>(e);
        uint64_t used = 0;
        for (uint64_t base = 0; base < F; base += C) {
            const uint64_t cnt = std::min<uint64_t>(C, F - base);
            if ((e = grow(nx, used + 4 * cnt, used)) != hipSuccess) return static_cast<int>(e);
            if (over) { *why = "its build scratch exceeds what the HBM budget leaves"; return 0; }
            hipLaunchKernelGGL(k_jump_expand, dim3(grid_for(cfg, 4 * cnt)), dim3(256), 0, st, lv_lo[cur].as<uint64_t>(), lv_hi[cur].as<uint64_t>(), base, cnt,
                               mb.as<uint8_t>(), clo.as<uint64_t>(), chi.as<uint64_t>(), sym.as<uint8_t>());
            if ((e = hipGetLastError()) != hipSuccess) return static_cast<int>(e);
            if (int rc = launch_lf(plain, cfg, clo.as<uint64_t>(), chi.as<uint64_t>(), sym.as<uint8_t>(), 4 * cnt, nlo.as<uint64_t>(), nhi.as<uint64_t>(), st)) return rc;
            hipLaunchKernelGGL(k_jump_keep, dim3(grid_for(cfg, 4 * cnt)), dim3(256), 0, st, nlo.as<uint64_t>(), nhi.as<uint64_t>(), lv_key[cur].as<uint4>(), base,
                               4 * cnt, level, lv_lo[nx].as<uint64_t>(), lv_hi[nx].as<uint64_t>(), lv_key[nx].as<uint4>(), cnt_d.as<unsigned long long>());
            if ((e = hipGetLastError()) != hipSuccess) return static_cast<int>(e);
            unsigned long long got = 0;
            if ((e = hipMemcpyAsync(&got, cnt_d.p, sizeof(got), hipMemcpyDeviceToHost, st)) != hipSuccess) return static_cast<int>(e);
            if ((e = hipStreamSynchronize(st)) != hipSuccess) return static_cast<int>(e);
            used = got;
        }
        F = used;
        cur = nx;
        if (F == 0) break;
    }
    *keys = F;
    const uint64_t nb = jump_buckets_for(F);
    const uint64_t bytes = nb * kJumpBucketBytes;
    if (F == 0 || nb >= (uint64_t(1) << 32)) { *why = F ? "more keys than the table addresses" : "no K-mer occurs"; return 0; }
    if (bytes > table_budget || bytes + scratch() > peak_budget) {
        *why = "the table exceeds the bytes allowed for it (what the HBM budget leaves; by default also half the replica)";
        return 0;
    }
    void *t = nullptr;
    if ((e = hipMalloc(&t, bytes)) != hipSuccess) { (void)hipGetLastError(); *why = "hipMalloc of the table failed"; return 0; }
    int rc = static_cast<int>(hipMemsetAsync(t, 0, bytes, st));
    if (!rc) rc = static_cast<int>(hipMemsetAsync(cnt_d.p, 0, sizeof(unsigned long long), st));
    for (uint64_t base = 0; !rc && base < F; base += 4 * C) {
        const uint64_t cnt = std::min<uint64_t>(4 * C, F - base);
        hipLaunchKernelGGL(k_jump_meta, dim3(grid_for(cfg, cnt)), dim3(256), 0, st, cnt, K, clo.as<uint2>());
        rc = static_cast<int>(hipGetLastError());
        if (!rc) rc = launch_find_range_runs_packed(plain, cfg, clo.as<uint2>(), lv_key[cur].as<uint4>() + base, cnt, chi.as<uint64_t>(), nlo.as<uint64_t>(),
                                                    ix.has_tsa ? nhi.as<uint64_t>() : nullptr, st);
        if (!rc) {
            hipLaunchKernelGGL(k_jump_insert, dim3(grid_for(cfg, cnt)), dim3(256), 0, st, lv_key[cur].as<uint4>() + base, chi.as<uint64_t>(), nlo.as<uint64_t>(),
                               ix.has_tsa ? nhi.as<uint64_t>() : nullptr, cnt, static_cast<uint32_t *>(t), nb, cnt_d.as<unsigned long long>());
            rc = static_cast<int>(hipGetLastError());
        }
    }
    unsigned long long ins = 0;
    if (!rc) rc = static_cast<int>(hipMemcpyAsync(&ins, cnt_d.p, sizeof(ins), hipMemcpyDeviceToHost, st));
    if (!rc) rc = static_cast<int>(hipStreamSynchronize(st));
    if (rc) { (void)hipFree(t); return rc; }
    *tab = t;
    *tab_bytes = bytes;
    *buckets = nb;
    *keys = ins;
    return 0;
}

}
```

### rowbowt_amd/csrc/k_runs.hip

```cpp
#include <type_traits>

#include "rbg_runs2_device.hpp"
#include "rbg_chain_walk.hpp"
#include "rbg_locate_docs.hpp"
#include "rbg_jump.h"
#include "rbg_launch.hpp"

namespace rbg {
namespace {

struct PackedBits {
    const uint4 *__restrict__ cp;
    uint4 w;
    uint32_t widx, navail;
    uint64_t sr;
    __device__ __forceinline__ uint32_t next_word() {
        if (widx == 4) { w = *cp++; widx = 0; }
        const uint32_t v = w.x;
        w.x = w.y; w.y = w.z; w.z = w.w;
        ++widx;
        return v;
    }
    __device__ __forceinline__ uint32_t take(uint32_t nb) {
        if (navail < nb) { sr |= static_cast<uint64_t>(next_word()) << navail; navail += 32; }
        const uint32_t v = static_cast<uint32_t>(sr & ((uint64_t(1) << nb) - 1));
        sr >>= nb;
        navail -= nb;
        return v;
    }
};

template <bool GLDS>
__device__ __forceinline__ bool jump_probe_wave(const void *__restrict__ tab, const uint64_t nb, const bool probing, const JumpKey &key, uint32_t v[3],
                                                uint32_t &buckets, lds_byte *tile) {
    uint32_t state = probing ? kJumpNext : kJumpAbsent;
    uint64_t b = probing ? jump_home(jump_hash(key), nb) : 0u;
    uint64_t left = nb;
    while (__ballot(state == kJumpNext)) {
        const bool undecided = state == kJumpNext;
        uint32_t w[16];
        quad_fetch_issue<GLDS>(reinterpret_cast<uint64_t>(tab) + (undecided ? b : 0u) * kJumpBucketBytes, w, tile);
        quad_fetch_take<GLDS>(w, tile);
        if (undecided) {
            ++buckets;
            state = jump_bucket(w, key, v);
            b = jump_next(b, nb);
            if (--left == 0 && state == kJumpNext) state = kJumpAbsent;
        }
    }
    return state <= kJumpHit1;
}

template <typename P, bool TOEHOLD, bool PACKED = false, bool STATS = false, bool GLDS = false, bool STAGE = false>
__global__ __launch_bounds__(512, STATS ? 2 : 4) void k_find_range_runs(const DevIndex ix, const void *__restrict__ src_a,
                                                        const void *__restrict__ src_b, const uint64_t N,
                                                        uint64_t *__restrict__ lo_out, uint64_t *__restrict__ hi_out,
                                                        uint64_t *__restrict__ ss_out, unsigned long long *__restrict__ stats,
                                                        const uint32_t *__restrict__ sel, const uint32_t *__restrict__ nsel) {
    const uint64_t Neff = sel ? static_cast<uint64_t>(*nsel) : N;
    const uint8_t *__restrict__ seqs = static_cast<const uint8_t *>(src_a);
    const uint64_t *__restrict__ off = static_cast<const uint64_t *>(src_b);
    const uint4 *__restrict__ chunks = static_cast<const uint4 *>(src_a);
    const uint2 *__restrict__ meta = static_cast<const uint2 *>(src_b);
    __shared__ uint8_t s_lut[256];
    __shared__ uint8_t s_lut2[256];
    __shared__ uint8_t s_mslot[4];
    __shared__ __align__(16) unsigned char s_tile[GLDS ? 8 * kTileBytes : 16];
    __shared__ uint32_t s_codes[STAGE ? 8 * kStageWords * 64 : 1];
    for (int t = threadIdx.x; t < 256; t += blockDim.x) {
        s_lut[t] = ix.lut[t];
        s_lut2[t] = ix.nmajor ? ix.lut2[t] : 0xFFu;
    }
    RBG_RUN_SEARCH2_SHARED;
    const RunSearch2<P> S2 = stage_run_search2<P>(ix, s_tab_first, s_ent2, s_dir2, s_rec2, s_dyn);
    const uint32_t *tab_first = s_tab_first;
    lds_byte *tile = (lds_byte *)s_tile + (GLDS ? (threadIdx.x >> 6) * kTileBytes : 0u);
    if (PACKED || STAGE) {
        for (int t = threadIdx.x; t < 256; t += blockDim.x)
            if (s_lut2[t] != 0xFFu) s_mslot[s_lut2[t] & 3u] = s_lut[t];
        __syncthreads();
    }
    const uint32_t D = ix.run_ksteps, DMASK = ix.run_depth_mask | 1u;
    const uint32_t M = ix.nmajor;
    const uint32_t lane = threadIdx.x & (kWave - 1);
    lds_u32 *codes = (lds_u32 *)s_codes + (STAGE ? (threadIdx.x >> 6) * (kStageWords * 64u) + lane : 0u);
    const StageTab stage_tab{ix.stage_code[0], ix.stage_code[1], ix.stage_byte[0], ix.stage_byte[1], ix.stage_shift};
    const bool stage_on = STAGE && ix.stage_ok != 0 && M == 4;

    unsigned long long c_occ = 0, c_reads = 0;
    uint32_t c_matched = 0;
    unsigned long long st[kStatSearchN] = {0, 0, 0, 0, 0, 0, 0, 0};
    const uint64_t stride = static_cast<uint64_t>(gridDim.x) * blockDim.x;
    const uint64_t wave_first = static_cast<uint64_t>(blockIdx.x) * blockDim.x + (threadIdx.x & ~(kWave - 1));
    for (uint64_t base = wave_first; base < Neff; base += stride) {
        bool valid = base + lane < Neff;
        const uint64_t i = (sel && valid) ? static_cast<uint64_t>(sel[base + lane]) : base + lane;
        uint64_t beg = 0, p = 0;
        PackedBits bs{chunks, make_uint4(0, 0, 0, 0), 4u, 0u, 0ull};
        if (PACKED) {
            if (valid) {
                const uint2 mt = meta[i];
                if (mt.y & 0x80000000u) valid = false;
                else { p = mt.y; bs.cp = chunks + mt.x; }
            }
        } else if (valid) { beg = off[i]; p = off[i + 1]; }
        bool staged = false;
        if constexpr (STAGE && !PACKED) {
            if (stage_on && __ballot(valid && p - beg > kStageCap) == 0) {
                uint32_t nch = 0;
                const bool bad = valid && stage_read(reinterpret_cast<const uint4 *>(seqs), beg, p, stage_tab, codes, nch);
                if (STATS) st[kStChunks] += nch;
                staged = __ballot(bad) == 0;
                if (staged) { p -= beg; beg = 0; }
                else if (STATS) st[kStChunks] -= nch;
            }
        }
        auto walk = [&](auto staged_tag) __attribute__((always_inline)) {
            constexpr bool STAGED = decltype(staged_tag)::value;
            const uint64_t p_end = p;
            uint64_t p_min = p;
            const uint32_t m32 = static_cast<uint32_t>(p);
            uint64_t lo = 0, hi = ix.n - 1;
            uint64_t k = TOEHOLD ? ix.last_run_sample : 0;
            bool alive = valid;
            bool pend = false;
            uint32_t pend_d = 0, pend_rec = 0;
            uint64_t pend_e = 0;
            ByteCursor rd{reinterpret_cast<const uint4 *>(seqs), ~uint64_t(0), make_uint4(0, 0, 0, 0)};
            bool jumped = false;
            if constexpr (STAGED && sizeof(P) == 4) {
                if (ix.jump) {
                    const bool probing = valid && m32 >= ix.jump_k;
                    JumpKey key{{codes[0], codes[64], codes[128], codes[192]}};
                    jump_key_mask(key, ix.jump_k);
                    uint32_t v[3] = {0, 0, 0}, nbk = 0;
                    if (jump_probe_wave<GLDS>(ix.jump, ix.jump_buckets, probing, key, v, nbk, tile)) {
                        lo = v[0]; hi = v[1];
                        if (TOEHOLD) k = v[2] == 0xFFFFFFFFu ? ~uint64_t(0) : static_cast<uint64_t>(v[2]);
                        p -= ix.jump_k;
                        jumped = true;
                        if (STATS) st[kStSymbols] += ix.jump_k;
                    }
                    if (STATS) st[kStFtab] += nbk;
                }
            }
            if (!jumped && valid && ix.ftab_k && p - beg >= ix.ftab_k) {
                uint64_t idx = 0;
                bool all_major = true;
                PackedBits probe = bs;
                if constexpr (STAGED) {
                    const uint32_t w0 = codes[0];
                    idx = ix.ftab_k >= 16u ? w0 : (w0 & ((1u << (2u * ix.ftab_k)) - 1u));
                } else if (PACKED) {
                    idx = probe.take(2 * ix.ftab_k);
                } else {
                    uint64_t pw = 1;
                    for (uint32_t t = 1; t <= ix.ftab_k; ++t) {
                        const uint32_t mm = s_lut2[rd.at(p - t)];
                        all_major = all_major && mm != 0xFFu;
                        idx += (mm & 3u) * pw;
                        pw *= M;
                    }
                }
                uint64_t flo, fhi2, fk;
                if (STATS) { if (!STAGED) p_min = p - ix.ftab_k; if (all_major) st[kStFtab] += 1; }
                if (all_major && ftab_lookup<P>(ix, idx, flo, fhi2, fk)) {
                    if (PACKED) bs = probe;
                    lo = flo; hi = fhi2;
                    if (TOEHOLD) k = fk;
                    p -= ix.ftab_k;
                    if (STATS) st[kStSymbols] += ix.ftab_k;
                    if (hi < lo) { alive = false; p = beg; }
                }
            }
            struct Pick { uint32_t d, adv, rec; bool ok; };
            auto pick_at = [&](const uint64_t pp) __attribute__((always_inline)) -> Pick {
                Pick s{0u, 1u, 0u, true};
                if constexpr (STAGED) {
                    s.adv = pp < D ? static_cast<uint32_t>(pp) : D;
                    s.adv = 32u - static_cast<uint32_t>(__clz(DMASK & ((2u << (s.adv - 1)) - 1u)));
                    const uint32_t t0 = m32 - static_cast<uint32_t>(pp);
                    const lds_u32 *cw = codes + (t0 >> 4) * 64u;
                    const uint32_t v = __builtin_amdgcn_alignbit(cw[64], cw[0], (t0 & 15u) * 2u) & ((1u << (2u * s.adv)) - 1u);
                    s.rec = run_record(tab_first, s.adv, s.adv == 1 ? static_cast<uint32_t>(s_mslot[v]) : v);
                    s.d = s.adv - 1;
                } else if (PACKED) {
                    s.adv = pp < D ? static_cast<uint32_t>(pp) : D;
                    s.adv = 32u - static_cast<uint32_t>(__clz(DMASK & ((2u << (s.adv - 1)) - 1u)));
                    const uint32_t v = bs.take(2 * s.adv);
                    s.rec = run_record(tab_first, s.adv, s.adv == 1 ? static_cast<uint32_t>(s_mslot[v]) : v);
                    s.d = s.adv - 1;
                } else {
                    const uint64_t q = pp - 1;
                    const uint32_t c = rd.at(q);
                    if (STATS && q < p_min) p_min = q;
                    const uint32_t m0 = s_lut2[c];
                    uint32_t acc = m0;
                    if (m0 != 0xFFu) {
                        uint32_t pw = M, run_acc = m0;
    #pragma unroll 1
                        for (uint32_t t = 1; t < static_cast<uint32_t>(kMaxRunDepth); ++t) {
                            if (t >= D || q < beg + t) break;
                            const uint32_t mm = s_lut2[rd.at(q - t)];
                            if (STATS && q - t < p_min) p_min = q - t;
                            if (mm == 0xFFu) break;
                            run_acc += mm * pw;
                            pw *= M;
                            if ((DMASK >> t) & 1u) { s.adv = t + 1; acc = run_acc; }
                        }
                    }
                    if (s.adv == 1) {
                        const uint32_t slot = s_lut[c];
                        if (slot == 0xFFu || slot >= static_cast<uint32_t>(kLdsSyms)) s.ok = false;
                        else s.rec = run_record(tab_first, 1u, slot);
                    } else {
                        s.d = s.adv - 1;
                        s.rec = run_record(tab_first, s.adv, acc);
                    }
                }
                return s;
            };
            constexpr bool AHEAD = !PACKED || STAGED;
            Pick cur{0u, 1u, 0u, false};
            RunHot Rcur{0, 0};
            if (AHEAD && alive && p > beg) {
                cur = pick_at(p);
                if (cur.ok) Rcur = load_run_tab<P>(S2, cur.d, cur.rec);
            }
            while (__ballot(alive && p > beg)) {
                bool stepping = alive && p > beg;
                if (!AHEAD && stepping) {
                    cur = pick_at(p);
                    if (cur.ok) Rcur = load_run_tab<P>(S2, cur.d, cur.rec);
                }
                if (stepping && !cur.ok) { alive = false; stepping = false; }
                const uint32_t d = cur.d, adv = cur.adv, rec = cur.rec;
                const RunHot R = Rcur;
                const uint64_t p_next = p - adv;
                if (AHEAD && stepping && p_next > beg) {
                    cur = pick_at(p_next);
                    if (cur.ok) Rcur = load_run_tab<P>(S2, cur.d, cur.rec);
                }
                RunStep r;
                lane_lf2_quad<P, STATS, false, GLDS>(S2, stepping, d, rec, R, lo, hi + 1, r, st, tile);
                if (stepping) {
                    if (STATS) st[kStSymbols] += adv;
                    const uint64_t c_inside = r.c_upto - r.c_before;
                    if (c_inside == 0) {
                        alive = false;
                    } else {
                        if (TOEHOLD) {
                            if (r.inside) k = k - adv;
                            else { pend = true; pend_d = d; pend_rec = rec; pend_e = r.samp_e; k = 0; }
                        }
                        lo = r.F + r.c_before;
                        hi = lo + c_inside - 1;
                        p = p_next;
                    }
                }
            }
            if (TOEHOLD && alive && pend) {
                k += run_step_sample2<P>(ix, S2, pend_d, pend_rec, pend_e);
                if (STATS) st[kStResample] += 1;
            }
            if (STATS && !PACKED && !STAGED && p_end > p_min) st[kStChunks] += ((p_end - 1) >> 4) - (p_min >> 4) + 1;
            if (STATS && PACKED && valid) st[kStChunks] += (p_end + 63) >> 6;
            if (!alive) { lo = 1; hi = 0; k = 0; }
            if (valid) {
                lo_out[i] = lo;
                hi_out[i] = hi;
                if (TOEHOLD) ss_out[i] = k;
                c_reads += 1;
                if (alive) { c_matched += 1; c_occ += hi - lo + 1; }
            }
        };
        if (STAGE && staged) walk(std::integral_constant<bool, STAGE>{}); else walk(std::false_type{});
    }
    c_reads = wave_sum(c_reads);
    const unsigned long long w_matched = wave_sum(static_cast<unsigned long long>(c_matched));
    c_occ = wave_sum(c_occ);
    if (lane == 0 && c_reads) {
        atomicAdd(&ix.counters[0], c_reads);
        if (w_matched) atomicAdd(&ix.counters[1], w_matched);
        if (c_occ) atomicAdd(&ix.counters[2], c_occ);
    }
    if (STATS) {
#pragma unroll
        for (int t = 0; t < kStatSearchN; ++t) {
            const unsigned long long v = wave_sum(st[t]);
            if (lane == 0 && v) atomicAdd(&stats[t], v);
        }
    }
}

template <typename P> struct ChunkR { static constexpr int v = 8; };

template <typename P, typename OUT = uint64_t, bool STATS = false, bool SUB = false, bool HI8 = false>
__global__ __launch_bounds__(256, 4) void k_locate_fill_runs2(const DevIndex ix, const uint64_t *__restrict__ lo,
                                                          const uint64_t *__restrict__ hi, const uint64_t *__restrict__ k,
                                                          const uint64_t N, const uint64_t max_hits,
                                                          const uint64_t *__restrict__ loc_off, OUT *__restrict__ locs,
                                                          const uint64_t *__restrict__ sub, const uint32_t *__restrict__ order,
                                                          const uint64_t *__restrict__ skeys, unsigned long long *__restrict__ stats) {
    constexpr int kChunkR = ChunkR<P>::v;
    using Stage = ChainStage<P, kChunkR, SUB, true, HI8>;
    __shared__ Stage S;
    chain_fill_walk<P, OUT, STATS, SUB, HI8, kChunkR, 1>(ix, S, lo, hi, k, N, max_hits, loc_off, locs, sub, order, skeys, stats,
                                                         [&](const uint64_t k1, unsigned long long &cost) { return run_phi<P, STATS>(ix, k1, cost); });
}

extern __shared__ unsigned long long locate_docs_lds[];
template <typename P, bool LOCS>
__global__ __launch_bounds__(kLocDocBlock) void k_locate_docs_runs2(const DevIndex ix, const DocTable t, const uint64_t *__restrict__ lo,
                                                                   const uint64_t *__restrict__ hi, const uint64_t *__restrict__ k, const uint64_t N,
                                                                   const uint64_t max_hits, const uint32_t *__restrict__ order,
                                                                   const uint64_t *__restrict__ skeys, uint64_t *__restrict__ sets,
                                                                   uint32_t *__restrict__ ndocs_out, uint32_t *__restrict__ nodoc_out,
                                                                   unsigned long long *__restrict__ doc_reads, unsigned long long *__restrict__ doc_locs) {
    locate_docs_walk<P, LOCS>(ix, t, locate_docs_lds, lo, hi, k, N, max_hits, order, skeys, sets, ndocs_out, nodoc_out, doc_reads, doc_locs,
                              [&](const uint64_t k1, unsigned long long &cost) { return run_phi<P>(ix, k1, cost); });
}

}

int launch_find_range_runs_impl(const DevIndex &ix, const LaunchCfg &cfg, const void *src_a, const void *src_b, uint64_t N,
                                uint64_t *lo, uint64_t *hi, uint64_t *ssamp, void *stream, bool packed, unsigned long long *stats,
                                const uint32_t *sel = nullptr, const uint32_t *nsel = nullptr) {
    if (N == 0) return 0;
    const size_t lds = run_search2_lds(ix);
    static const bool glds = [] { const char *e = std::getenv("RBG_REC_FETCH"); return !(e && std::strcmp(e, "quad") == 0); }();
    static const bool stage = [] { const char *e = std::getenv("RBG_STAGE_READS"); return !(e && e[0] == '0'); }();
    if (stats && packed) return static_cast<int>(hipErrorNotSupported);
    const LaunchCfg c = runs512_cfg(cfg);
    const dim3 grid(sel ? std::min(grid_for(c, N), 256) : grid_for(c, N)), block(512);
    return with_pos(ix.pos_bytes, [&](auto p) { return with_flag(ssamp != nullptr, [&](auto toe) {
        auto search = [&](auto pk, auto sts, auto gl, auto sg) {
            constexpr bool GL = decltype(gl)::value, SG = decltype(sg)::value;
            return launch_lds(k_find_range_runs<pos_t<decltype(p)>, decltype(toe)::value, decltype(pk)::value, decltype(sts)::value, GL, SG>, grid, block, lds,
                              (GL ? 8 * kTileBytes : 0) + (SG ? 8 * kStageWaveBytes : 0), stream, ix, src_a, src_b, N, lo, hi, ssamp, stats, sel, nsel);
        };
        auto fetch = [&](auto pk, auto sts) {
            if constexpr (!decltype(pk)::value) { if (glds && stage && !sel) return search(no, sts, yes, yes); }
            return glds ? search(pk, sts, yes, no) : search(pk, sts, no, no);
        };
        if (stats) return fetch(no, yes);
        return packed ? fetch(yes, no) : fetch(no, no);
    }); });
}

int launch_find_range_runs(const DevIndex &ix, const LaunchCfg &cfg, const uint8_t *seqs, const uint64_t *off, uint64_t N,
                           uint64_t *lo, uint64_t *hi, uint64_t *ssamp, void *stream, unsigned long long *stats) {
    return launch_find_range_runs_impl(ix, cfg, seqs, off, N, lo, hi, ssamp, stream, false, stats);
}

int launch_find_range_runs_sel(const DevIndex &ix, const LaunchCfg &cfg, const uint8_t *seqs, const uint64_t *off, uint64_t N, uint64_t *lo,
                               uint64_t *hi, uint64_t *ssamp, const uint32_t *sel, const uint32_t *nsel, void *stream) {
    return launch_find_range_runs_impl(ix, cfg, seqs, off, N, lo, hi, ssamp, stream, false, nullptr, sel, nsel);
}

int launch_find_range_runs_packed(const DevIndex &ix, const LaunchCfg &cfg, const uint2 *meta, const uint4 *chunks, uint64_t N,
                                  uint64_t *lo, uint64_t *hi, uint64_t *ssamp, void *stream) {
    return launch_find_range_runs_impl(ix, cfg, chunks, meta, N, lo, hi, ssamp, stream, true, nullptr);
}

int launch_locate_fill_runs(const DevIndex &ix, const LaunchCfg &cfg, const uint64_t *lo, const uint64_t *hi, const uint64_t *k,
                            uint64_t N, uint64_t max_hits, const uint64_t *loc_off, uint64_t *locs, const uint64_t *sub,
                            const void *order, const uint64_t *skeys, void *stream, unsigned long long *stats, uint32_t *locs32) {
    if (N == 0) return 0;
    const dim3 grid(grid_for(cfg, N)), block(256);
    const uint32_t *perm = static_cast<const uint32_t *>(order);
    return chain_fill_variants(ix, stats, sub, locs, locs32, [&](auto p, auto sts, auto sb, auto h8, auto *dst) {
        return launch_grid(k_locate_fill_runs2<pos_t<decltype(p)>, std::remove_pointer_t<decltype(dst)>, decltype(sts)::value, decltype(sb)::value, decltype(h8)::value>,
                           grid, block, 0, stream, ix, lo, hi, k, N, max_hits, loc_off, dst, sub, perm, skeys, stats);
    });
}

int launch_locate_doc_hits_runs(const DevIndex &ix, const DocTable &t, const uint64_t *lo, const uint64_t *hi, const uint64_t *k, uint64_t N, uint64_t max_hits,
                                const void *order, const uint64_t *skeys, uint64_t *sets, uint32_t *ndocs_out, uint32_t *nodoc_out, uint64_t *doc_reads,
                                uint64_t *doc_locs, void *stream) {
    if (t.ndocs == 0 || t.ndocs > kLocDocLdsDocs) return static_cast<int>(hipErrorInvalidValue);
    if (N == 0) return 0;
    const dim3 grid(locate_docs_grid(N)), block(kLocDocBlock);
    const uint32_t *perm = static_cast<const uint32_t *>(order);
    unsigned long long *dr = reinterpret_cast<unsigned long long *>(doc_reads), *dl = reinterpret_cast<unsigned long long *>(doc_locs);
    const size_t lds = locate_docs_lds_bytes(t.ndocs, t.ndir, doc_locs != nullptr);
    return with_pos(ix.pos_bytes, [&](auto p) { return with_flag(doc_locs != nullptr, [&](auto lc) {
        return launch_lds(k_locate_docs_runs2<pos_t<decltype(p)>, decltype(lc)::value>, grid, block, lds, 0, stream,
                          ix, t, lo, hi, k, N, max_hits, perm, skeys, sets, ndocs_out, nodoc_out, dr, dl);
    }); });
}

}
```

### rowbowt_amd/csrc/rbg_dev.h

```cpp
#pragma once

#include <hip/hip_runtime.h>

#include <algorithm>
#include <cstddef>
#include <cstdint>
#include <cstdio>
#include <vector>

#include "rbg_mkdir.hpp"
#include "rbg_fl.hpp"
#include "rbg_isa.hpp"

namespace rbg {

template <typename P>
struct RunEnt {
    P start;
    P cum;
};

template <typename P>
struct PhiEnt {
    P pos;
    P base;
};

struct Samp48 {
    uint16_t w[3];
};
struct Ent48 {
    uint32_t key_lo, val_lo;
    uint16_t key_hi, val_hi;
};
static_assert(sizeof(Ent48) == 12, "three words per entry");
template <typename P> struct PhiFmt;
template <> struct PhiFmt<uint32_t> {
    static constexpr size_t ent_bytes = 8, spare = 1;
    static void put_ent(void *base, uint64_t i, uint64_t key, uint64_t val) { static_cast<PhiEnt<uint32_t> *>(base)[i] = {static_cast<uint32_t>(key), static_cast<uint32_t>(val)}; }
};
template <> struct PhiFmt<uint64_t> {
    static constexpr size_t ent_bytes = sizeof(Ent48), spare = 3;
    static void put_ent(void *base, uint64_t i, uint64_t key, uint64_t val) {
        static_cast<Ent48 *>(base)[i] = {static_cast<uint32_t>(key), static_cast<uint32_t>(val), static_cast<uint16_t>(key >> 32), static_cast<uint16_t>(val >> 32)};
    }
};
template <typename P> struct RunsFmt;
template <> struct RunsFmt<uint32_t> {
    static constexpr size_t ent_bytes = 8, samp_bytes = 4, spare = 1;
    static void put_ent(void *base, uint64_t i, uint64_t key, uint64_t val) { static_cast<RunEnt<uint32_t> *>(base)[i] = {static_cast<uint32_t>(key), static_cast<uint32_t>(val)}; }
    static void put_samp(void *base, uint64_t i, uint64_t v) { static_cast<uint32_t *>(base)[i] = static_cast<uint32_t>(v); }
};
template <> struct RunsFmt<uint64_t> {
    static constexpr size_t ent_bytes = 16, samp_bytes = sizeof(Samp48), spare = 1;
    static void put_ent(void *base, uint64_t i, uint64_t key, uint64_t val) { static_cast<RunEnt<uint64_t> *>(base)[i] = {key, val}; }
    static void put_samp(void *base, uint64_t i, uint64_t v) {
        static_cast<Samp48 *>(base)[i] = {{static_cast<uint16_t>(v), static_cast<uint16_t>(v >> 16), static_cast<uint16_t>(v >> 32)}};
    }
};

struct alignas(16) RankSlot {
    uint32_t r0, w1, w2, w3;
};
constexpr int kSlotRuns = 4;
constexpr int kSlotRunsWide = 2;
constexpr uint32_t kMaxNarrowShift = 8, kMaxWideShift = 12;
template <typename P>
struct alignas(4 * sizeof(P)) PhiSlot {
    P dprev, d0, d1, meta;
};
struct alignas(16) PhiSlotPacked {
    uint64_t w0, w1;
};
constexpr uint32_t kPhiPackedPosBits = 38, kPhiPackedMaxShift = 6;
constexpr uint32_t kSlotOvf = 7;
constexpr uint32_t kPhiOvf = 3;
constexpr uint32_t kMaxSlotShift = 8;

struct DevSym {
    const void *ent;
    const void *samp;
    const void *slots;
    const uint32_t *ord;
    uint64_t F;
    uint32_t shift;
    uint32_t nruns;
};

constexpr int kLdsSyms = 8;
constexpr int kMaxMajor = 4;

struct DevRunTab2 {
    uint64_t F;
    uint64_t first;
    uint64_t dir_off;
    uint32_t dir_shift, pad;
};
static_assert(sizeof(DevRunTab2) == 32, "two 16-byte reads per record");
constexpr uint32_t kRunHotShiftBit = 56;
struct RunDir64 { uint32_t count, hi; };
constexpr uint32_t kRec2Pivots = 12;
constexpr uint32_t kRec2Overflow = 16u;
constexpr uint32_t kRec2Compact = 32u;
constexpr uint32_t kRec2CompactIn = 10;
struct alignas(64) RunRec2 {
    uint32_t e0;
    uint32_t hi;
    uint32_t meta;
    uint32_t cum_end;
    uint32_t ent[kRec2Pivots];
};
static_assert(sizeof(RunRec2) == 64, "one sector per bucket");
constexpr uint32_t kRunFillShift = 30;
struct PhiEnt12 { uint32_t pos_lo, base_lo, base_hi; };
static_assert(sizeof(PhiEnt12) == 12, "three words per entry");
constexpr uint32_t kPhiSuperShift = 16;

constexpr int kMaxRunDepth = 8;
constexpr int kLdsRunDepth = 5;
constexpr int kMaxLdsRunTabs = kLdsSyms + 16 + 64 + 256 + 1024 + kLdsRunDepth;


struct DevIndex {
    uint64_t n, r;
    uint64_t last_run_sample;
    const DevSym *syms;
    uint32_t sigma;
    uint32_t pos_bytes;
    const void *phi_ent;
    const void *phi_slots;
    const uint32_t *phi_ord;
    uint32_t phi_shift;
    uint32_t has_tsa;
    const uint64_t *mk_start, *mk_end, *mk_off, *mk_vals;
    uint64_t mk_nruns;
    const uint32_t *mk_bucket;
    uint32_t mk_shift;
    const MkRec *mk_rec;
    unsigned long long *counters;
    const uint8_t *lut;
    const DevSym *pairs;
    const DevSym *triples;
    const DevSym *quads;
    const DevSym *quints;
    const uint8_t *lut2;
    uint32_t nmajor;
    uint32_t kmer_steps;
    const void *ftab;
    uint32_t ftab_k;
    uint32_t phi_packed;
    const uint8_t *dense;
    uint32_t layout;
    uint32_t run_ksteps;
    uint32_t run_ntabs;
    const void *run_samp[kMaxRunDepth];
    uint32_t run_tab_first[kMaxRunDepth + 1];
    const uint32_t *phi_dir;
    uint32_t phi_dir_shift;
    uint32_t run_depth_mask;
    uint32_t phi_super_shift;
    uint32_t run_fill_shift;
    const void *run_ent2[kMaxRunDepth];
    const void *run_dir2[kMaxRunDepth];
    const DevRunTab2 *run_tabs2;
    const uint64_t *run_hot;
    uint32_t run_uni_depth;
    uint32_t run_uni_stride;
    uint32_t run_uni_shift;
    const RunRec2 *run_rec2[kMaxRunDepth];
    const uint64_t *phi_super;
    uint64_t phi_m;
    uint64_t phi_last_pos, phi_last_base;
    const uint64_t *order_docs;
    uint32_t order_ndocs, order_dbits, order_lowbits, order_obits;
    uint32_t stage_ok, stage_shift;
    uint32_t stage_code[2];
    uint32_t stage_byte[2];
    const void *jump;
    uint64_t jump_buckets;
    uint32_t jump_k;
    uint32_t tmk_shift;
    const uint64_t *tmk_start, *tmk_end, *tmk_off, *tmk_vals;
    uint64_t tmk_nruns;
    const uint32_t *tmk_bucket;
    const MkRec *tmk_rec;
};

enum SearchStat {
    kStSteps = 0,
    kStSlots,
    kStDense,
    kStSearch,
    kStFtab,
    kStResample,
    kStChunks,
    kStSymbols,
    kStatSearchN
};
static_assert(kMkStatRuns == kStatSearchN + 2, "marker_span_arrays counts the run starts / ends it reads behind the search counters");
enum LocateStat {
    kLsPhiSteps = 0,
    kLsPhiOvf,
    kLsChains,
    kLsLocs,
    kStatLocateN
};

template <typename P>
struct SeedLogRec {
    P lo, hi;
    uint32_t qs, qe, mb, me;
};
struct SeedLogWin {
    uint32_t src, cnt;
};
struct SeedLog {
    unsigned char *base;
    uint64_t stride;
    uint32_t qs, qw;
    uint32_t *nsel;
    unsigned long long *stats = nullptr;
};
enum SeedStat {
    kSdMarkerQueries = kStatSearchN,
    kSdMarkerDir,
    kSdMarkerProbes,
    kSdMarkerOff,
    kSdMarkerVals,
    kSdSeedRecs,
    kSdSequences,
    kSeedStatN
};
constexpr uint32_t kSeedLogOverflow = 0xFFFFFFFFu;
constexpr uint32_t kSeedLogWindows = 6, kSeedLogSeedsDefault = 12;
inline size_t seed_log_rec_bytes(uint32_t pos_bytes) { return pos_bytes == 4 ? sizeof(SeedLogRec<uint32_t>) : sizeof(SeedLogRec<uint64_t>); }
inline size_t seed_log_stride(uint32_t pos_bytes, uint32_t seeds_per_read) {
    return 8 + static_cast<size_t>(seeds_per_read) * seed_log_rec_bytes(pos_bytes) + kSeedLogWindows * sizeof(SeedLogWin);
}
inline size_t seed_log_bytes(uint64_t N, uint32_t pos_bytes, uint32_t seeds_per_read) {
    return static_cast<size_t>(N) * seed_log_stride(pos_bytes, seeds_per_read) + 64 + (N + 4) * 4;
}
inline SeedLog make_seed_log(void *scratch, size_t bytes, uint64_t N, uint32_t pos_bytes) {
    SeedLog lg{nullptr, 0, 0, kSeedLogWindows, nullptr, nullptr};
    if (!scratch || N == 0 || (reinterpret_cast<uintptr_t>(scratch) & 15)) return lg;
    const size_t tail = 64 + (N + 4) * 4, fixed = 8 + kSeedLogWindows * sizeof(SeedLogWin), rec = seed_log_rec_bytes(pos_bytes);
    if (bytes < tail + N * (fixed + 2 * rec)) return lg;
    size_t q = ((bytes - tail) / N - fixed) / rec;
    if (q > 255) q = 255;
    lg.qs = static_cast<uint32_t>(q);
    lg.stride = fixed + q * rec;
    lg.base = static_cast<unsigned char *>(scratch);
    lg.nsel = reinterpret_cast<uint32_t *>(lg.base + ((N * lg.stride + 15) & ~size_t(15)));
    return lg;
}

struct ComposeTable {
    const void *ent;
    const void *samp;
    uint64_t nruns, total, F;
};
struct ComposedLevel {
    void *ent = nullptr;
    void *samp = nullptr;
    uint64_t entries = 0;
    std::vector<uint64_t> nruns, total, F, first;
};
int compose_levels_device(uint32_t pos_bytes, uint64_t n, uint32_t M, const ComposeTable *major, const void *g_start, const uint32_t *g_id,
                          const void *g_samp, uint64_t g_n, uint32_t kmax, bool with_samples, std::vector<ComposedLevel> &out, void *stream,
                          uint32_t keep_mask = 0 ,
                          bool *inputs_released = nullptr );

inline double host_memory_available() {
    double avail = 1e18;
    if (FILE *f = std::fopen("/proc/meminfo", "r")) {
        char line[256];
        while (std::fgets(line, sizeof line, f)) {
            unsigned long long kb = 0;
            if (std::sscanf(line, "MemAvailable: %llu kB", &kb) == 1) { avail = static_cast<double>(kb) * 1024.0; break; }
        }
        std::fclose(f);
    }
    unsigned long long mx = 0, cur = 0;
    bool have_mx = false, have_cur = false;
    if (FILE *f = std::fopen("/sys/fs/cgroup/memory.max", "r")) { have_mx = std::fscanf(f, "%llu", &mx) == 1; std::fclose(f); }
    if (FILE *f = std::fopen("/sys/fs/cgroup/memory.current", "r")) { have_cur = std::fscanf(f, "%llu", &cur) == 1; std::fclose(f); }
    if (have_mx && have_cur && mx > cur) avail = std::min(avail, static_cast<double>(mx - cur));
    else if (have_mx && have_cur) avail = 0;
    return avail;
}


struct LaunchCfg {
    int block_threads = 256;
    int max_blocks = 0;
};

int launch_find_range(const DevIndex &ix, const LaunchCfg &cfg, const uint8_t *seqs, const uint64_t *off, uint64_t N,
                      uint64_t *lo, uint64_t *hi, uint64_t *ssamp , void *stream);
int launch_find_range_runs(const DevIndex &ix, const LaunchCfg &cfg, const uint8_t *seqs, const uint64_t *off, uint64_t N,
                           uint64_t *lo, uint64_t *hi, uint64_t *ssamp , void *stream,
                           unsigned long long *stats = nullptr );
int launch_find_range_runs_sel(const DevIndex &ix, const LaunchCfg &cfg, const uint8_t *seqs, const uint64_t *off, uint64_t N, uint64_t *lo,
                               uint64_t *hi, uint64_t *ssamp , const uint32_t *sel, const uint32_t *nsel, void *stream);
int launch_find_range_runs_packed(const DevIndex &ix, const LaunchCfg &cfg, const uint2 *meta, const uint4 *chunks, uint64_t N,
                                  uint64_t *lo, uint64_t *hi, uint64_t *ssamp , void *stream);
int launch_locate_fill_runs(const DevIndex &ix, const LaunchCfg &cfg, const uint64_t *lo, const uint64_t *hi, const uint64_t *k,
                            uint64_t N, uint64_t max_hits, const uint64_t *loc_off, uint64_t *locs, const uint64_t *sub,
                            const void *order, const uint64_t *skeys, void *stream, unsigned long long *stats = nullptr ,
                            uint32_t *locs32 = nullptr);
int launch_lf_runs(const DevIndex &ix, const LaunchCfg &cfg, const uint64_t *lo, const uint64_t *hi, const uint8_t *sym, uint64_t N,
                   uint64_t *lo_out, uint64_t *hi_out, void *stream);
int launch_find_range_markers_runs(const DevIndex &ix, const LaunchCfg &cfg, const uint8_t *seqs, const uint64_t *off, uint64_t N,
                                   uint64_t wsize, uint64_t max_range, uint64_t *lo, uint64_t *hi, uint64_t *cnt, const uint64_t *mk_off,
                                   uint64_t *mk, bool fill, void *stream);
int launch_greedy_seed_runs(const DevIndex &ix, const LaunchCfg &cfg, const uint8_t *seqs, const uint64_t *off, uint64_t N,
                            uint64_t min_length, uint64_t *lo, uint64_t *hi, uint64_t *qs, uint64_t *qe, uint64_t *ss, void *stream,
                            unsigned long long *stats = nullptr );
int launch_marker_seeds_runs(const DevIndex &ix, const LaunchCfg &cfg, const uint8_t *seqs, const uint64_t *off, uint64_t N, uint64_t wsize,
                             uint64_t max_range, uint64_t *seed_cnt, uint64_t *mk_cnt, const uint64_t *seed_off, const uint64_t *mk_off,
                             uint64_t *seeds, uint64_t *mk, bool fill, void *stream, const SeedLog &lg, uint64_t ftab_k = 0 );
int launch_marker_lmems_runs(const DevIndex &ix, const LaunchCfg &cfg, const uint8_t *seqs, const uint64_t *off, uint64_t N, uint64_t total,
                             uint64_t wsize, uint64_t max_range, uint64_t ftab_k, uint64_t *rec_off, uint64_t *seeds, uint64_t *mk, bool fill,
                             void *stream);
int launch_greedy_seeds_list_runs(const DevIndex &ix, const LaunchCfg &cfg, const uint8_t *seqs, const uint64_t *off, uint64_t N, uint64_t min_length,
                                  bool w_sample, uint64_t *seed_cnt, const uint64_t *seed_off, uint64_t *lo, uint64_t *hi, uint64_t *qs, uint64_t *qe,
                                  uint64_t *ss , bool fill, void *stream);
int launch_toehold_chkpnts_runs(const DevIndex &ix, const LaunchCfg &cfg, const uint8_t *seqs, const uint64_t *off, uint64_t N, uint64_t wsize,
                                const uint64_t *slot_off, uint64_t *cnt, uint64_t *lo, uint64_t *hi, uint64_t *qs, uint64_t *qe, uint64_t *ss,
                                void *stream);
int launch_find_range_stats(const DevIndex &ix, const LaunchCfg &cfg, const uint8_t *seqs, const uint64_t *off, uint64_t N,
                            uint64_t *lo, uint64_t *hi, uint64_t *ssamp , unsigned long long *stats ,
                            void *stream);
size_t scan_tmp_bytes(uint64_t N);
int launch_locate_plan(const DevIndex &ix, const LaunchCfg &cfg, const uint64_t *lo, const uint64_t *hi, uint64_t N,
                       uint64_t max_hits, uint64_t *loc_off, void *tmp, size_t tmp_bytes, void *stream);
int launch_locate_fill(const DevIndex &ix, const LaunchCfg &cfg, const uint64_t *lo, const uint64_t *hi,
                       const uint64_t *k, uint64_t N, uint64_t max_hits, const uint64_t *loc_off, uint64_t *locs,
                       const uint64_t *sub ,
                       const void *order , void *stream,
                       unsigned long long *stats = nullptr ,
                       uint32_t *locs32 = nullptr );
size_t locate_order_ws_bytes(uint64_t N);
int launch_locate_order(const DevIndex &ix, const LaunchCfg &cfg, const uint64_t *k, uint64_t N, void *ws, size_t ws_bytes,
                        void *stream);
int launch_build_rank_slots(uint32_t pos_bytes, const void *ent, uint64_t nruns, uint64_t n, uint32_t shift, void *slots,
                            uint32_t *ord, unsigned long long *overflow, unsigned long long *dense_cursor, void *stream);
int launch_fill_dense(uint32_t pos_bytes, const void *ent, uint64_t n, uint32_t shift, const void *slots, const uint32_t *ord,
                      uint8_t *dense, void *stream);
size_t text_ws_bytes(uint64_t E);
int launch_copy16(const void *pinned_src, void *dst, uint64_t bytes, void *stream);
int launch_text_plan(const uint64_t *lo, const uint64_t *hi, const uint64_t *loc_off, const uint64_t *locs, uint64_t N, uint64_t E, const char *names,
                     const uint32_t *name_off, const uint64_t *doc_start, const char *doc_names, const uint32_t *doc_name_off, uint64_t ndocs,
                     uint64_t text_size, bool with_locs, const uint64_t *mk_off, const uint64_t *mk, void *ws, size_t ws_bytes, unsigned int *d_bad, void *stream);
void text_total_ptrs(void *ws, uint64_t E, const uint64_t **last_at, const uint32_t **last_len);
int launch_text_fill(const uint64_t *lo, const uint64_t *hi, const uint64_t *loc_off, const uint64_t *locs, uint64_t N, uint64_t E, const char *names,
                     const uint32_t *name_off, const uint64_t *doc_start, const char *doc_names, const uint32_t *doc_name_off, uint64_t ndocs,
                     uint64_t text_size, bool with_locs, const uint64_t *mk_off, const uint64_t *mk, void *ws, uint64_t total, char *text, void *stream);
struct SamBatch {
    uint64_t N, E;
    const uint64_t *lo, *hi, *a, *b;
    const uint8_t *rev;
    const uint64_t *line_off, *loc_off, *locs;
    const char *seqs, *quals;
    const uint64_t *roff;
    const char *names;
    const uint32_t *name_off;
    const uint64_t *doc_start;
    const char *doc_names;
    const uint32_t *doc_name_off;
    uint64_t ndocs, text_size;
};
int launch_sam_strands(const uint8_t *seqs, const uint64_t *off, uint64_t N, uint64_t total, uint8_t *out, uint64_t *off2, uint32_t cap, void *stream);
size_t sam_pick_tmp_bytes(uint64_t N);
int launch_sam_pick(const uint64_t *lo2, const uint64_t *hi2, const uint64_t *qs2, const uint64_t *qe2, const uint64_t *ss2, uint64_t N, uint64_t max_hits,
                    uint64_t *lo, uint64_t *hi, uint64_t *k, uint64_t *a, uint64_t *b, uint8_t *rev, uint64_t *nlines, uint64_t *line_off,
                    unsigned long long *counters, void *tmp, size_t tmp_bytes, uint32_t cap, void *stream);
size_t sam_ws_bytes(uint64_t E);
int launch_sam_plan(const SamBatch &B, void *ws, size_t ws_bytes, unsigned int *d_bad, uint32_t cap, void *stream);
void sam_total_ptrs(void *ws, uint64_t E, const uint64_t **last_at, const uint64_t **last_len);
int launch_sam_fill(const SamBatch &B, void *ws, uint64_t total, char *text, uint32_t cap, void *stream);
int launch_sam_offsets(void *ws, uint64_t E, void *stream);
int launch_extend_left(const DevIndex &ix, const uint8_t *seqs, const uint64_t *off, uint64_t N, const uint32_t *item_seq, const uint32_t *item_a,
                       const uint64_t *item_row, const uint64_t *item_limit, uint64_t M, uint32_t max_mismatch, void *out, unsigned int *d_err, uint32_t cap,
                       void *stream);
int launch_sam_ext_items(const SamBatch &B, void *ws, uint32_t *item_seq, uint32_t *item_a, uint64_t *item_row, uint64_t *item_limit, unsigned int *d_bad,
                         uint32_t cap, void *stream);
int launch_sam_ext_len(const SamBatch &B, void *ws, const void *ext, uint32_t cap, void *stream);
int launch_sam_ext_fill(const SamBatch &B, void *ws, const void *ext, uint64_t total, char *text, uint32_t cap, void *stream);
int launch_fl_rows(const FlView &v, uint32_t pos_bytes, uint64_t n, const uint64_t *rows, uint64_t M, uint8_t *sym, uint64_t *next, unsigned int *d_err,
                   uint32_t cap, void *stream);
int launch_extend_right(const FlView &v, uint32_t pos_bytes, uint64_t n, const uint8_t *seqs, const uint64_t *off, uint64_t N, const uint32_t *item_seq,
                        const uint32_t *item_b, const uint64_t *item_row, const uint32_t *item_skip, const uint64_t *item_limit, const uint32_t *item_k, uint64_t M,
                        uint32_t max_mismatch, void *out, unsigned int *d_err, uint32_t cap, void *stream);
int launch_sam_right_items(const SamBatch &B, void *ws, const void *ext_left, uint64_t n, uint32_t K, uint32_t *item_seq, uint32_t *item_b, uint64_t *item_row,
                           uint32_t *item_skip, uint64_t *item_limit, uint32_t *item_k, uint32_t cap, void *stream);
int launch_sam_both_len(const SamBatch &B, void *ws, const void *ext, const void *ext_right, uint32_t cap, void *stream);
int launch_sam_both_fill(const SamBatch &B, void *ws, const void *ext, const void *ext_right, uint64_t total, char *text, uint32_t cap, void *stream);
int launch_isa_rows(const FlView &fl, const IsaView &isa, uint32_t pos_bytes, const uint64_t *pos, uint64_t M, uint64_t *row, unsigned int *d_err, uint32_t cap,
                    void *stream);
int launch_extract(const FlView &fl, const IsaView &isa, uint32_t pos_bytes, const uint64_t *pos, const uint32_t *len, const uint64_t *out_off, uint64_t M,
                   uint8_t *out, uint32_t *got, unsigned int *d_err, uint32_t cap, void *stream);
size_t sa_tmp_bytes(uint64_t n, uint32_t pos_bytes);
int sa_build(const uint8_t *text, uint64_t n, void *sa, uint32_t pos_bytes, void *tmp, size_t tmp_bytes, void *stream, uint64_t info[8]);
size_t text_runs_tmp_bytes(uint64_t n, uint32_t pos_bytes);
int text_runs_plan(const uint8_t *text, const void *sa, uint64_t n, uint32_t pos_bytes, void *tmp, size_t tmp_bytes, uint64_t *R, void *stream);
int text_runs_fill(const uint8_t *text, const void *sa, uint64_t n, uint32_t pos_bytes, const void *tmp, size_t tmp_bytes, uint64_t R, uint8_t *heads,
                   uint64_t *lens, uint64_t *ssa, uint64_t *esa, void *stream);
int launch_run_dirs(uint32_t pos_bytes, const void *ent, const uint64_t *first, const uint64_t *nruns, const uint64_t *doff, const uint32_t *dshift,
                    uint32_t T, uint64_t total, uint32_t *dir, void *stream);
int launch_pack_samp48(const uint64_t *in, uint64_t n, void *out, void *stream);
int launch_fill_count(const void *ent, uint64_t m, uint64_t n, uint32_t fill_shift, uint64_t *arr , unsigned long long *total, void *stream);
int launch_scan_u64(uint64_t *vals, uint64_t N, void *tmp, size_t tmp_bytes, void *stream);
int launch_fill_expand(bool phi, const void *ent, const uint64_t *samp, uint64_t m, uint64_t n, uint32_t fill_shift, const uint64_t *pos, void *ent_out, uint64_t *samp_out, void *stream);
int launch_gather_u64(const uint64_t *src, const uint64_t *idx, uint64_t count, uint64_t *out, void *stream);
int launch_pack_pairs32(const void *ent, uint64_t m, uint64_t spare, void *out, void *stream);
int launch_pack_phi12(const void *ent, uint64_t m, uint64_t spare, void *out, void *stream);
int launch_run_dirs2(const void *ent, const uint64_t *first, const uint64_t *nruns, const uint64_t *doff, const uint32_t *dshift, uint32_t T, uint64_t total,
                     void *dir, void *stream);
int launch_fold_F(uint32_t pos_bytes, void *ent, const uint64_t *first, const uint64_t *F, uint32_t T, uint64_t total, void *stream);
int launch_run_recs2(uint32_t pos_bytes, const void *ent, const uint64_t *first, const uint64_t *nruns, const uint64_t *roff, const uint32_t *rshift, uint32_t T, uint64_t total,
                     void *recs, unsigned long long *overflow, void *stream);
int launch_phi_dir(uint32_t pos_bytes, const void *ent, uint64_t m, uint32_t shift, uint64_t nb, uint32_t *dir, uint32_t ss, uint64_t *super, void *stream);
int launch_build_phi_slots(uint32_t pos_bytes, bool packed, const void *ent, uint64_t r, uint64_t n, uint32_t shift, void *slots, uint32_t *ord,
                           unsigned long long *overflow, void *stream);
size_t pack_ws_bytes(uint64_t N, uint64_t total_bytes);
int launch_pack_reads(const DevIndex &ix, const LaunchCfg &cfg, const uint8_t *seqs, const uint64_t *off, uint64_t N,
                      uint64_t total_bytes, void *ws, size_t ws_bytes, void *stream);
int launch_find_range_packed(const DevIndex &ix, const LaunchCfg &cfg, const void *ws, const uint8_t *seqs, const uint64_t *off,
                             uint64_t N, uint64_t total_bytes, uint64_t *lo, uint64_t *hi, uint64_t *ssamp, void *stream);
int launch_find_range_packed_only(const DevIndex &ix, const LaunchCfg &cfg, const uint2 *meta, const uint4 *chunks, uint64_t N,
                                  uint64_t *lo, uint64_t *hi, uint64_t *ssamp , void *stream);
int launch_marker_seeds_plan(const DevIndex &ix, const LaunchCfg &cfg, const uint8_t *seqs, const uint64_t *off, uint64_t N,
                             uint64_t wsize, uint64_t max_range, uint64_t ftab_k, uint64_t *seed_off, uint64_t *mk_off, void *tmp,
                             size_t tmp_bytes, void *stream, void *log = nullptr, size_t log_bytes = 0, unsigned long long *stats = nullptr );
int launch_marker_seeds_fill(const DevIndex &ix, const LaunchCfg &cfg, const uint8_t *seqs, const uint64_t *off, uint64_t N,
                             uint64_t wsize, uint64_t max_range, uint64_t ftab_k, const uint64_t *seed_off, const uint64_t *mk_off,
                             uint64_t *seeds, uint64_t *mk, void *stream, void *log = nullptr, size_t log_bytes = 0, unsigned long long *stats = nullptr);
size_t marker_lmems_tmp_bytes(uint64_t total);
int launch_marker_lmems_plan(const DevIndex &ix, const LaunchCfg &cfg, const uint8_t *seqs, const uint64_t *off, uint64_t N, uint64_t total,
                             uint64_t wsize, uint64_t max_range, uint64_t ftab_k, uint64_t *mk_off, void *tmp, size_t tmp_bytes, void *stream);
int launch_marker_lmems_fill(const DevIndex &ix, const LaunchCfg &cfg, const uint8_t *seqs, const uint64_t *off, uint64_t N, uint64_t total,
                             uint64_t wsize, uint64_t max_range, uint64_t ftab_k, const void *tmp, uint64_t *seeds, uint64_t *mk, void *stream);
int launch_greedy_seeds_plan(const DevIndex &ix, const LaunchCfg &cfg, const uint8_t *seqs, const uint64_t *off, uint64_t N, uint64_t min_length,
                             bool w_sample, uint64_t *seed_off, void *tmp, size_t tmp_bytes, void *stream);
int launch_greedy_seeds_fill(const DevIndex &ix, const LaunchCfg &cfg, const uint8_t *seqs, const uint64_t *off, uint64_t N, uint64_t min_length,
                             bool w_sample, const uint64_t *seed_off, uint64_t *lo, uint64_t *hi, uint64_t *qs, uint64_t *qe, uint64_t *ss, void *stream);
int launch_toehold_chkpnts_slots(const LaunchCfg &cfg, const uint64_t *off, uint64_t N, uint64_t wsize, uint64_t *slot_off, void *tmp, size_t tmp_bytes,
                                 void *stream);
int launch_toehold_chkpnts(const DevIndex &ix, const LaunchCfg &cfg, const uint8_t *seqs, const uint64_t *off, uint64_t N, uint64_t wsize,
                           const uint64_t *slot_off, uint64_t *cnt, uint64_t *lo, uint64_t *hi, uint64_t *qs, uint64_t *qe, uint64_t *ss, void *stream);
int launch_greedy_seed(const DevIndex &ix, const LaunchCfg &cfg, const uint8_t *seqs, const uint64_t *off, uint64_t N,
                       uint64_t min_length, uint64_t *lo, uint64_t *hi, uint64_t *qs, uint64_t *qe, uint64_t *ss, void *stream, unsigned long long *stats = nullptr);
int launch_markers_plan(const DevIndex &ix, const LaunchCfg &cfg, const uint64_t *lo, const uint64_t *hi, uint64_t N,
                        uint64_t *mk_off, void *tmp, size_t tmp_bytes, void *stream);
int launch_markers_fill(const DevIndex &ix, const LaunchCfg &cfg, const uint64_t *lo, const uint64_t *hi, uint64_t N,
                        const uint64_t *mk_off, uint64_t *mk, void *stream);
int loc_markers_group();
int launch_loc_markers_plan(const DevIndex &ix, const LaunchCfg &cfg, const uint64_t *locs, const uint64_t *loc_off, const uint64_t *off, uint64_t N,
                            uint64_t *mk_off, void *tmp, size_t tmp_bytes, int group, void *stream);
int launch_loc_markers_fill(const DevIndex &ix, const LaunchCfg &cfg, const uint64_t *locs, const uint64_t *loc_off, const uint64_t *off, uint64_t N,
                            const uint64_t *mk_off, uint64_t *mk, int group, void *stream);
int docs_group();
int launch_resolve_offsets(const uint64_t *sorted, const uint32_t *dir, uint64_t size, uint32_t ndocs, uint32_t shift, uint32_t ndir, const void *locs,
                           bool locs32, uint64_t M, uint32_t *doc, uint64_t *offset, void *stream);
int launch_doc_hits(const uint64_t *sorted, const uint32_t *dir, uint64_t size, uint32_t ndocs, uint32_t shift, uint32_t ndir, const void *locs, bool locs32,
                    const uint64_t *loc_off, uint64_t N, uint64_t *sets, uint32_t *ndocs_out, uint32_t *nodoc_out, uint64_t *doc_reads, int group,
                    void *stream);
constexpr uint32_t kLocDocLdsDocs = 1024;
struct DocTable {
    const uint64_t *sorted;
    const uint32_t *dir;
    uint64_t size;
    uint32_t ndocs, shift, ndir;
};
int launch_locate_doc_hits(const DevIndex &ix, const LaunchCfg &cfg, const DocTable &t, const uint64_t *lo, const uint64_t *hi, const uint64_t *k, uint64_t N,
                           uint64_t max_hits, const void *order, uint64_t *sets, uint32_t *ndocs_out, uint32_t *nodoc_out, uint64_t *doc_reads,
                           uint64_t *doc_locs, void *stream);
int launch_locate_doc_hits_runs(const DevIndex &ix, const DocTable &t, const uint64_t *lo, const uint64_t *hi, const uint64_t *k, uint64_t N, uint64_t max_hits,
                                const void *order, const uint64_t *skeys, uint64_t *sets, uint32_t *ndocs_out, uint32_t *nodoc_out, uint64_t *doc_reads,
                                uint64_t *doc_locs, void *stream);
int launch_doc_locs(const uint64_t *sorted, const uint32_t *dir, uint64_t size, uint32_t ndocs, uint32_t shift, uint32_t ndir, const void *locs, bool locs32,
                    uint64_t M, uint64_t *doc_locs, void *stream);
int launch_read_strands(const uint8_t *seqs, const uint64_t *off, uint64_t N, uint64_t total, uint8_t *out, uint64_t *off2, void *stream);
int report_canon_group();
size_t seed_canon_tmp_bytes(uint64_t S);
int launch_seed_canon(const LaunchCfg &cfg, uint64_t *seeds, uint64_t S, uint64_t *mk, uint64_t min_range, uint32_t flags, uint64_t read_len, void *tmp,
                      size_t tmp_bytes, int group, void *stream);
int launch_report_select(const uint64_t *seeds, const uint64_t *seed_off, const uint64_t *off2, uint64_t N, const uint8_t *first_fwd, uint64_t read_len,
                         uint64_t min_seed_len, uint32_t flags, uint64_t *rep_off, void *out, uint32_t *out_read, void *tmp, size_t tmp_bytes, void *stream);
int launch_report_melem(const void *recs, uint64_t R, uint64_t *melem, void *tmp, size_t tmp_bytes, void *stream);
size_t report_text_ws_bytes(uint64_t E);
int launch_report_map(const uint64_t *melem, uint64_t R, uint64_t E, void *ws, size_t ws_bytes, void *stream);
int launch_report_gather(const void *recs, const uint64_t *melem, const uint64_t *mk, uint64_t R, uint64_t E, void *ws, size_t ws_bytes, void *recs_out,
                         uint64_t *dense, void *stream);
int launch_report_text_plan(const void *recs, const uint32_t *rec_read, const uint64_t *melem, const uint64_t *mk, uint64_t R, uint64_t E, const char *names,
                            const uint32_t *name_off, void *ws, size_t ws_bytes, void *stream);
void report_text_total_ptrs(void *ws, uint64_t E, const uint64_t **last_at, const uint32_t **last_len);
int launch_report_text_fill(const void *recs, const uint32_t *rec_read, const uint64_t *melem, const uint64_t *mk, uint64_t R, uint64_t E, const char *names,
                            const uint32_t *name_off, void *ws, size_t ws_bytes, uint64_t total, char *text, void *stream);
const uint32_t *report_map_erec(const void *ws);
bool tally_combine_default();
int launch_tally_clear(uint64_t *slots, uint64_t cap, void *stream);
int launch_tally_add(uint64_t *slots, uint64_t cap, uint64_t *hdr, const void *recs, const uint64_t *melem, const uint64_t *mk, const uint32_t *erec, uint64_t R,
                     uint64_t E, bool combine, void *stream);
int launch_tally_add_reads(uint64_t *slots, uint64_t cap, uint64_t *hdr, uint64_t *xhdr, const void *recs, const uint64_t *melem, const uint64_t *mk,
                           const uint32_t *erec, const uint64_t *rep_off, uint64_t N, void *span, uint64_t R, uint64_t E, uint32_t flags, bool combine, void *stream);
int launch_tally_add_entries(uint64_t *slots, uint64_t cap, uint64_t *hdr, const void *entries, uint64_t count, void *stream);
int launch_tally_rehash(const uint64_t *old_slots, uint64_t old_cap, uint64_t *new_slots, uint64_t new_cap, uint64_t *hdr, void *stream);
size_t tally_compact_tmp_bytes(uint64_t cap);
int launch_tally_compact_plan(const uint64_t *slots, uint64_t cap, uint64_t *pos, void *tmp, size_t tmp_bytes, void *stream);
int launch_tally_compact_fill(uint64_t *slots, uint64_t cap, uint64_t *hdr, const uint64_t *pos, void *out, void *stream);
int launch_find_range_markers_plan(const DevIndex &ix, const LaunchCfg &cfg, const uint8_t *seqs, const uint64_t *off,
                                   uint64_t N, uint64_t wsize, uint64_t max_range, uint64_t *lo, uint64_t *hi,
                                   uint64_t *mk_off, void *tmp, size_t tmp_bytes, void *stream);
int launch_find_range_markers_fill(const DevIndex &ix, const LaunchCfg &cfg, const uint8_t *seqs, const uint64_t *off,
                                   uint64_t N, uint64_t wsize, uint64_t max_range, const uint64_t *mk_off, uint64_t *mk,
                                   void *stream);
int launch_lf(const DevIndex &ix, const LaunchCfg &cfg, const uint64_t *lo, const uint64_t *hi, const uint8_t *sym,
              uint64_t N, uint64_t *lo_out, uint64_t *hi_out, void *stream);
int launch_build_ftab(const DevIndex &ix, const LaunchCfg &cfg, uint32_t k, void *tab, void *stream);
size_t ftab_build_scratch_bytes(uint64_t words, uint32_t k);
int launch_build_jump(const DevIndex &ix, const LaunchCfg &cfg, uint32_t K, uint64_t table_budget, uint64_t peak_budget, void **tab,
                      uint64_t *tab_bytes, uint64_t *buckets, uint64_t *keys, const char **why, void *stream);
int launch_sample_reads(const uint8_t *text, uint64_t unit, uint64_t H, uint64_t L, uint64_t m, uint64_t seed, uint64_t first,
                        uint64_t N, uint32_t sub_ppm, uint8_t *seqs, uint64_t *off, uint64_t *start_out , void *stream);
int launch_sample_reads_pg(const uint8_t *base, const uint64_t *sites, const uint8_t *alt, const uint8_t *G, uint64_t S, const uint32_t *site_dir, uint32_t site_dir_shift,
                           uint64_t unit, uint64_t H, uint64_t L, uint64_t m, uint64_t seed, uint64_t first, uint64_t N, uint32_t sub_ppm, uint8_t *seqs, uint64_t *off,
                           uint64_t *start_out, void *stream);
int launch_count_from_ranges(const uint64_t *lo, const uint64_t *hi, uint64_t N, uint64_t *count, void *stream);

}
```

### rowbowt_amd/csrc/rbg_jump.h

```cpp
#pragma once

#include <cstdint>

#if defined(__HIPCC__)
#define RBG_JUMP_HD __host__ __device__ __forceinline__
#else
#define RBG_JUMP_HD inline
#endif

namespace rbg {

constexpr uint32_t kJumpMaxK = 64;
constexpr uint32_t kJumpMinK = 16;
constexpr uint32_t kJumpSlotWords = 8;
constexpr uint32_t kJumpBucketBytes = 64;
constexpr uint32_t kJumpEmptyTag = 0, kJumpFullTag = 1;
constexpr uint32_t kJumpDefaultK = 60;
constexpr uint64_t kJumpAutoMinBytes = uint64_t(256) << 20;

struct JumpKey {
    uint32_t w[4];
};

RBG_JUMP_HD void jump_key_mask(JumpKey &key, uint32_t K) {
    for (uint32_t i = 0; i < 4; ++i) {
        const uint32_t lo_sym = 16u * i;
        const uint32_t keep = K <= lo_sym ? 0u : (K - lo_sym >= 16u ? 16u : K - lo_sym);
        key.w[i] = keep == 16u ? key.w[i] : (key.w[i] & ((1u << (2u * keep)) - 1u));
    }
}

RBG_JUMP_HD void jump_key_set(JumpKey &key, uint32_t t, uint32_t c) {
    key.w[t >> 4] |= (c & 3u) << (2u * (t & 15u));
}

RBG_JUMP_HD uint64_t jump_hash(const JumpKey &key) {
    const uint64_t a = key.w[0] | (static_cast<uint64_t>(key.w[1]) << 32);
    const uint64_t b = key.w[2] | (static_cast<uint64_t>(key.w[3]) << 32);
    uint64_t h = (a * 0x9E3779B97F4A7C15ull) ^ ((b + 0x632BE59BD9B4E019ull) * 0xC2B2AE3D27D4EB4Full);
    h ^= h >> 29;
    h *= 0xBF58476D1CE4E5B9ull;
    h ^= h >> 32;
    return h;
}

RBG_JUMP_HD uint64_t jump_home(uint64_t h, uint64_t nb) {
    return ((h >> 32) * nb) >> 32;
}

constexpr uint32_t kJumpHit0 = 0, kJumpHit1 = 1, kJumpAbsent = 2, kJumpNext = 3;
RBG_JUMP_HD uint32_t jump_bucket(const uint32_t w[16], const JumpKey &key, uint32_t v[3]) {
    for (uint32_t s = 0; s < 2; ++s) {
        const uint32_t *sl = w + kJumpSlotWords * s;
        if (sl[7] == kJumpEmptyTag) return kJumpAbsent;
        if (sl[0] == key.w[0] && sl[1] == key.w[1] && sl[2] == key.w[2] && sl[3] == key.w[3]) {
            v[0] = sl[4]; v[1] = sl[5]; v[2] = sl[6];
            return s;
        }
    }
    return kJumpNext;
}

RBG_JUMP_HD uint64_t jump_next(uint64_t b, uint64_t nb) { return b + 1 == nb ? 0 : b + 1; }

template <typename Load>
RBG_JUMP_HD bool jump_probe(const Load &load, uint64_t nb, const JumpKey &key, uint32_t v[3], uint32_t &buckets) {
    uint64_t b = jump_home(jump_hash(key), nb);
    for (uint64_t step = 0; step < nb; ++step) {
        ++buckets;
        uint32_t w[16];
        load(b, 0, w, w + 4);
        load(b, 1, w + 8, w + 12);
        const uint32_t r = jump_bucket(w, key, v);
        if (r != kJumpNext) return r != kJumpAbsent;
        b = jump_next(b, nb);
    }
    return false;
}

inline uint64_t jump_buckets_for(uint64_t keys) { return keys ? keys : 1; }

}
```

### rowbowt_amd/csrc/rbg_load_plan.hpp

```cpp
#ifndef RBG_LOAD_PLAN_HPP
#define RBG_LOAD_PLAN_HPP

#include <algorithm>
#include <cstddef>
#include <cstdint>
#include <vector>

#include "../../include/rbg.h"
#include "rbg_host.hpp"
#include "rbg_jump.h"

namespace rbg {

struct LoadConsts {
    uint32_t max_narrow_shift, max_wide_shift;
    uint32_t lds_syms;
    size_t slot_bytes;
    size_t arena_align;
    size_t runs_samp_bytes[2], phi_ent_bytes[2];
    uint32_t lds_run_depth;
    uint32_t uni_stride_bits, uni_shift_bits, uni_first_bits;
    uint32_t phi_packed_pos_bits, phi_packed_max_shift;
    size_t phi_slot_bytes[2], phi_slot_packed_bytes, phi_pair_bytes[2];
};
// ... 23 lines not shown
        --K;
    }
    return K;
}

inline bool runs_certain(int64_t layout_opt, bool auto_runs) { return layout_opt == RBG_LAYOUT_RUNS || auto_runs; }
inline double slot_level1_estimate(uint64_t n, uint32_t sigma, uint32_t pos_bytes, const LoadConsts &c) {
    return static_cast<double>(sigma) * static_cast<double>((n >> c.max_narrow_shift) + 2) * static_cast<double>(c.slot_bytes) +
           static_cast<double>((n >> 6) + 2) * (4.0 * pos_bytes + 4);
}
inline int slot_levels_fitting(uint64_t n, double major, int slot_steps, uint32_t shift, double budget, const LoadConsts &c) {
    const double per_table = static_cast<double>((n >> shift) + 2) * static_cast<double>(c.slot_bytes);
    double total = major * per_table, tables = major;
    int keep = 1;
    for (int k = 2; k <= slot_steps; ++k) {
        tables *= major;
        total += tables * per_table;
        if (total > budget) break;
        keep = k;
    }
    return keep;
}
inline bool runs_layout_fits(uint64_t r, double budget) { return 110.0 * static_cast<double>(r) <= budget; }

struct BudgetRaise {
    bool raise;
    double raised;
    uint32_t want;
};
inline BudgetRaise budget_raise(double r, int kmer_steps, size_t free_b, size_t whole_b, int64_t opt_mb, int64_t layout_opt, double budget) {
    BudgetRaise b{false, 0.75 * static_cast<double>(free_b), static_cast<uint32_t>(std::min(kmer_steps, 4))};
    const bool device_to_itself = static_cast<double>(free_b) >= 0.9 * static_cast<double>(whole_b);
    const uint32_t K0 = static_cast<uint32_t>(kmer_steps);
    const uint32_t from_quarter = planned_depth(r, true, K0, static_cast<double>(free_b), budget, true);
    b.raise = opt_mb == 0 && layout_opt == RBG_LAYOUT_AUTO && device_to_itself && from_quarter < b.want &&
              planned_depth(r, true, K0, static_cast<double>(free_b), b.raised, true) > from_quarter;
    return b;
}

inline uint32_t bucket_shift(double runs, double per, uint64_t n, uint32_t max_shift) {
    uint32_t sh = 0;
    runs = std::max(1.0, runs);
    while (sh < max_shift && runs * static_cast<double>(uint64_t(2) << sh) <= per * static_cast<double>(n)) ++sh;
    return sh;
}
inline uint64_t bucket_count(uint64_t n, uint32_t shift) { return (n >> shift) + 2; }

inline bool deepest_with_records(const std::vector<double> &rec_per, uint32_t mask, uint32_t d, uint32_t D) {
    for (uint32_t d2 = d + 1; d2 < D; ++d2)
        if ((mask >> d2 & 1u) && rec_per[d2] > 0) return false;
    return true;
}
inline bool uniform_stride_fits(uint64_t stride, const LoadConsts &c) { return !(stride >> c.uni_stride_bits); }
struct UniformCandidate {
    bool eligible;
    uint32_t shift;
    uint64_t stride;
};
inline UniformCandidate uniform_candidate(bool deepest_recs, uint32_t depth_index, size_t tables, size_t tables_before, double total_runs, uint64_t own_records,
                                          double per, uint64_t n, uint32_t max_shift, int uni_switch, const LoadConsts &c) {
    UniformCandidate u{false, 0, 0};
    if (!(deepest_recs && depth_index >= c.lds_run_depth && uni_switch != 0 && tables > 1)) return u;
    u.shift = bucket_shift(total_runs / static_cast<double>(tables), per, n, max_shift);
    u.stride = bucket_count(n, u.shift);
    u.eligible = uniform_stride_fits(u.stride, c) && u.shift < (1u << c.uni_shift_bits) && tables_before + tables < (size_t(1) << c.uni_first_bits) &&
                 (uni_switch == 1 || static_cast<double>(u.stride) * static_cast<double>(tables) <= 1.1 * static_cast<double>(own_records));
    return u;
}
inline bool uniform_needs_comparison(uint64_t novf, uint64_t records, int uni_switch) {
    return uni_switch != 1 && static_cast<double>(novf) * 256.0 > static_cast<double>(records);
}
inline bool uniform_stays(uint64_t novf_uni, uint64_t novf_own, uint64_t records_uni) {
    return static_cast<double>(novf_uni) <= 1.25 * static_cast<double>(novf_own) + static_cast<double>(records_uni) / 256.0;
}

struct PhiSlotBuckets {
    uint32_t shift;
    uint64_t buckets;
};
inline PhiSlotBuckets phi_slot_buckets(uint64_t n, uint64_t r, uint32_t phi_shift) {
    PhiSlotBuckets b{0, 0};
    const double rows_per_sample = static_cast<double>(n) / static_cast<double>(std::max<uint64_t>(1, r));
    while (b.shift < 8 && static_cast<double>(uint64_t(2) << b.shift) <= rows_per_sample) ++b.shift;
    if (b.shift < phi_shift) b.shift = phi_shift;
    b.buckets = bucket_count(n, b.shift);
    return b;
}
struct PhiSlotGeometry {
    uint32_t shift;
    bool packed;
    size_t bucket_bytes;
    uint64_t buckets;
    size_t reserve;
    size_t slot_bytes() const { return bucket_bytes - 4; }
};
inline PhiSlotGeometry phi_slot_geometry(uint64_t n, uint64_t r, uint32_t phi_shift, uint32_t pos_bytes, const LoadConsts &c) {
    const PhiSlotBuckets b = phi_slot_buckets(n, r, phi_shift);
    PhiSlotGeometry g{b.shift, false, 0, b.buckets, 0};
    const bool wide = pos_bytes == 8;
    g.packed = wide && (n >> c.phi_packed_pos_bits) == 0 && g.shift <= c.phi_packed_max_shift;
    g.bucket_bytes = (g.packed ? c.phi_slot_packed_bytes : c.phi_slot_bytes[wide]) + 4;
    g.reserve = g.buckets * g.bucket_bytes + (r + 1) * c.phi_pair_bytes[wide];
    return g;
}
inline bool phi_by_slots(int64_t run_phi_opt, const PhiSlotGeometry &g, uint64_t r, uint64_t hbm_bytes, uint64_t hbm_budget) {
    return run_phi_opt == 2 || (run_phi_opt == 0 && hbm_budget && g.buckets <= 2 * r && hbm_bytes + g.reserve <= hbm_budget);
}
inline uint32_t phi_dir_shift(uint64_t r, uint64_t n, double per, uint32_t max_shift) {
    uint32_t ds = 2;
    while (ds < max_shift && ds < 30 && (static_cast<double>(r) * static_cast<double>(uint64_t(1) << ds)) / static_cast<double>(n) < per) ++ds;
    return ds;
}
struct StageTables {
    bool ok;
    uint32_t shift;
    uint8_t code[8], byte[8];
};
inline StageTables stage_tables(const uint8_t major_byte[4]) {
    StageTables s{false, 0, {0, 0, 0, 0, 0, 0, 0, 0}, {0, 0, 0, 0, 0, 0, 0, 0}};
    for (uint32_t sh = 0; sh <= 5 && !s.ok; ++sh) {
        uint8_t code[8] = {0, 0, 0, 0, 0, 0, 0, 0}, byte[8] = {0, 0, 0, 0, 0, 0, 0, 0};
        bool used[8] = {false, false, false, false, false, false, false, false}, distinct = true;
        for (uint32_t m = 0; m < 4; ++m) {
            const uint32_t t = (major_byte[m] >> sh) & 7u;
            if (used[t]) distinct = false;
            used[t] = true;
            code[t] = static_cast<uint8_t>(m);
            byte[t] = major_byte[m];
        }
        if (!distinct) continue;
        for (uint32_t t = 0; t < 8; ++t)
            if (!used[t]) byte[t] = static_cast<uint8_t>(((t ^ 1u) & 7u) << sh);
        s.ok = true;
        s.shift = sh;
        std::copy(code, code + 8, s.code);
        std::copy(byte, byte + 8, s.byte);
    }
    return s;
}

struct IndexShape {
    uint64_t n = 0, r = 0;
    bool has_tsa = false;
    uint32_t pos_bytes = 4, phi_shift = 0;
    std::vector<uint64_t> nruns[kMaxKmerDepth];
};
inline IndexShape shape_of(const HostIndex &h) {
    IndexShape s;
    s.n = h.n; s.r = h.r; s.has_tsa = h.has_tsa; s.pos_bytes = h.pos_bytes; s.phi_shift = h.phi_shift;
    for (uint32_t di = 0; di < static_cast<uint32_t>(kMaxKmerDepth); ++di)
        for (const SymTable &t : di == 0 ? h.sym : h.kmer(di + 1)) s.nruns[di].push_back(t.nruns);
    return s;
}
inline uint64_t depth_entries(const IndexShape &s, uint32_t depth_index) {
    uint64_t entries = 0;
    for (const uint64_t nr : s.nruns[depth_index]) entries += nr + 1;
    return entries;
}
inline size_t runs_replica_bytes(const IndexShape &s, const LoadConsts &c, uint32_t mask = ~0u) {
    size_t total = 0;
    const bool wide = s.pos_bytes == 8;
    const size_t ent_bytes = 8, dir_per_entry = wide ? 4 : 2;
    for (uint32_t di = 0; di < static_cast<uint32_t>(kMaxKmerDepth); ++di) {
        if (!((mask | 1u) >> di & 1u)) continue;
        const size_t entries = depth_entries(s, di);
        total += entries * (ent_bytes + (s.has_tsa ? c.runs_samp_bytes[wide] : 0)) + entries * dir_per_entry + s.nruns[di].size() * 8 + 8 * c.arena_align;
    }
    if (s.has_tsa) total += (s.r + 1) * c.phi_ent_bytes[wide] + s.r * 4;
    return total + 16 * c.arena_align;
}
inline double runs_record_count(const IndexShape &s, uint32_t depth_index, double per, uint32_t max_shift) {
    double nrec = 0;
    for (const uint64_t nr : s.nruns[depth_index]) nrec += static_cast<double>(bucket_count(s.n, bucket_shift(static_cast<double>(nr), per, s.n, max_shift)));
    return nrec;
}
inline double runs_phi_slot_bytes(const IndexShape &s) {
    if (!s.has_tsa) return 0;
    const double nb = static_cast<double>(phi_slot_buckets(s.n, s.r, s.phi_shift).buckets);
    return nb <= 2.0 * static_cast<double>(s.r) ? nb * (s.pos_bytes == 8 ? 36.0 : 20.0) : 0.0;
}
inline double runs_bytes_before_records(const IndexShape &s, const LoadConsts &c, uint32_t mask, int64_t run_phi_opt) {
    double bytes = static_cast<double>(runs_replica_bytes(s, c, mask));
    if (run_phi_opt != 1) bytes += runs_phi_slot_bytes(s);
    return bytes;
}
constexpr double kRecBytes = 64.0;
constexpr double kRecPers[3] = {2.5, 4.0, 6.0};

struct TrimStep {
    enum Kind { kLevelAboveMask, kLeaveOutDepth, kDropDeepest, kLevelWithoutData, kEndsOnly } kind;
    uint32_t depth;
    size_t tables;
    double need, with_ends;
    bool drops_level() const { return kind == kLevelAboveMask || kind == kDropDeepest || kind == kLevelWithoutData; }
};
struct RunTrim {
    uint32_t mask = 0, levels = 1, depths_dropped_budget = 0;
    std::vector<TrimStep> steps;
};
inline RunTrim trim_run_depths(const IndexShape &s, const LoadConsts &c, uint32_t asked_mask, uint32_t levels, size_t budget, uint32_t has_data) {
    RunTrim t;
    t.mask = asked_mask;
    t.levels = levels;
    auto drop = [&](TrimStep::Kind kind, double need) { t.steps.push_back({kind, t.levels, s.nruns[t.levels - 1].size(), need, 0}); --t.levels; };
    while (t.levels > 1 && !(t.mask >> (t.levels - 1) & 1u)) drop(TrimStep::kLevelAboveMask, 0);
    t.mask &= (1u << t.levels) - 1u;
    for (size_t need; (need = runs_replica_bytes(s, c, t.mask)) > budget && t.levels > 1;) {
        uint32_t mid = 0;
        for (uint32_t d = t.levels - 1; d >= 2 && !mid; --d)
            if (t.mask >> (d - 1) & 1u) mid = d;
        if (mid) {
            t.steps.push_back({TrimStep::kLeaveOutDepth, mid, 0, static_cast<double>(need), 0});
            t.mask &= ~(1u << (mid - 1));
            t.depths_dropped_budget |= 1u << (mid - 1);
            continue;
        }
        t.depths_dropped_budget |= 1u << (t.levels - 1);
        drop(TrimStep::kDropDeepest, static_cast<double>(need));
        while (t.levels > 1 && !(has_data >> (t.levels - 1) & 1u)) drop(TrimStep::kLevelWithoutData, 0);
        t.mask = (t.mask & ((1u << t.levels) - 1u)) | (1u << (t.levels - 1));
    }
    return t;
}
inline bool ends_only_rule_applies(int64_t run_depths_opt, int64_t run_rec_opt, uint32_t levels) { return run_depths_opt == 0 && run_rec_opt == 0 && levels > 2; }
inline void trim_to_ends_for_records(const IndexShape &s, const LoadConsts &c, RunTrim &t, size_t budget, uint32_t max_shift, int64_t run_phi_opt) {
    const uint32_t ends = 1u | (1u << (t.levels - 1));
    auto with_records = [&](uint32_t m) {
        double bytes = runs_bytes_before_records(s, c, m, run_phi_opt);
        for (uint32_t d = 0; d < t.levels; ++d)
            if (m >> d & 1u) bytes += runs_record_count(s, d, kRecPers[2], max_shift) * kRecBytes;
        return bytes;
    };
    if (t.mask != ends && with_records(t.mask) > static_cast<double>(budget) && with_records(ends) <= static_cast<double>(budget)) {
        t.steps.push_back({TrimStep::kEndsOnly, t.levels, 0, with_records(t.mask), with_records(ends)});
        t.depths_dropped_budget |= t.mask & ~ends;
        t.mask = ends;
    }
}

inline std::vector<double> run_record_plan(const IndexShape &s, const LoadConsts &c, uint32_t mask, uint32_t D, uint64_t hbm_budget, int64_t run_rec_opt,
                                           int64_t run_rec_depths_opt, double rec_asked, uint32_t max_shift, int64_t run_phi_opt) {
    std::vector<double> rec_per(D, 0.0);
    if (run_rec_opt == 2) {
        const uint32_t want = run_rec_depths_opt ? static_cast<uint32_t>(run_rec_depths_opt) : ~0u;
        for (uint32_t d = 0; d < D; ++d)
            if ((mask >> d & 1u) && (want >> d & 1u)) rec_per[d] = rec_asked > 0 ? rec_asked : kRecPers[0];
    } else if (run_rec_opt == 0 && hbm_budget) {
        double total = runs_bytes_before_records(s, c, mask, run_phi_opt);
        const double budget = static_cast<double>(hbm_budget);
        std::vector<double> widest(D, 0.0), entries(D, 0.0);
        double all_widest = 0;
        bool every = true;
        for (uint32_t d = 0; d < D; ++d) {
            if (!(mask >> d & 1u)) continue;
            entries[d] = static_cast<double>(depth_entries(s, d));
            widest[d] = runs_record_count(s, d, rec_asked > 0 ? rec_asked : kRecPers[2], max_shift) * kRecBytes;
            all_widest += widest[d];
            every = every && widest[d] <= entries[d] * kRecBytes;
        }
        every = every && total + all_widest <= budget;
        double shallower_widest = all_widest;
        for (int d = static_cast<int>(D) - 1; d >= 0; --d) {
            if (!(mask >> d & 1u)) continue;
            shallower_widest -= widest[d];
            for (const double per : kRecPers) {
                if (rec_asked > 0 && per != kRecPers[0]) break;
                const double use = rec_asked > 0 ? rec_asked : per;
                const double bytes = runs_record_count(s, static_cast<uint32_t>(d), use, max_shift) * kRecBytes;
                if (bytes <= entries[d] * kRecBytes && total + bytes + (every ? shallower_widest : 0.0) <= budget) {
                    rec_per[d] = use;
                    total += bytes;
                    break;
                }
            }
        }
    }
    return rec_per;
}

inline uint32_t widened_shift(uint64_t n, uint64_t nruns, uint32_t shift, const LoadConsts &c) {
    if (n >> 40) return shift;
    const double rows_per_run = static_cast<double>(n) / static_cast<double>(std::max<uint64_t>(1, nruns));
    uint32_t want = 0;
    while (want < c.max_wide_shift && static_cast<double>(uint64_t(2) << want) <= rows_per_run) ++want;
    return std::max(want, shift);
}
inline int64_t auto_ftab_k(uint32_t nmajor, uint64_t n) {
    int64_t fk = 0;
    double w = 1;
    while (nmajor >= 2 && fk < 12 && w * nmajor <= static_cast<double>(n) / 16) { w *= nmajor; ++fk; }
    return fk;
}
inline double ftab_words(uint32_t nmajor, int64_t fk) {
    double words = 1;
    for (int64_t t = 0; t < fk; ++t) words *= nmajor;
    return words;
}
inline size_t ftab_entry_bytes(uint32_t pos_bytes) { return pos_bytes == 4 ? 16 : 32; }
inline bool ftab_fits(double words, size_t entry_bytes, size_t scratch_bytes, size_t free_b) {
    return words < 4.0e9 && words * static_cast<double>(entry_bytes) + static_cast<double>(scratch_bytes) < 0.5 * static_cast<double>(free_b);
}
inline int64_t auto_jump_k(uint64_t hbm_bytes) { return hbm_bytes > kJumpAutoMinBytes ? kJumpDefaultK : 0; }
struct JumpBudgets {
    uint64_t room, peak_budget, table_budget;
};
inline JumpBudgets jump_budgets(uint64_t hbm_budget, uint64_t hbm_bytes, size_t free_b, bool jump_auto) {
    JumpBudgets j;
    j.room = hbm_budget > hbm_bytes ? hbm_budget - hbm_bytes : 0;
    j.peak_budget = std::min<uint64_t>(j.room, free_b / 2);
    j.table_budget = std::min<uint64_t>(j.room, free_b / 4);
    if (jump_auto) j.table_budget = std::min<uint64_t>(j.table_budget, hbm_bytes / 2);
    return j;
}

}
#endif
```

Baseline: 2.165 billion.

## Add a second-level jump table keyed on parent range for longer k-mer skips

Builds an optional second hash table that maps a further K2 symbols plus the first-level result's lo value to the resulting BWT range. In the staged search, the kernel probes level 1 and then, on a hit, level 2, so it can skip up to K+K2 LF steps per read. It is enabled by default when the auto jump K is in use, within a combined HBM budget, and the build falls back to level 1 only if scratch space runs out. The cost is extra memory, a longer build, and an additional dependent probe per read.

Result: faster. 2.307 billion (median of 6 runs) (+6.6%).

```diff
diff --git a/include/rbg.h b/include/rbg.h
--- a/include/rbg.h
+++ b/include/rbg.h
@@ -109,8 +109,14 @@
     uint64_t bytes;
     uint64_t buckets;
     double build_ms;
+    uint64_t k2;
+    uint64_t keys2;
+    uint64_t bytes2;
+    uint64_t buckets2;
+    double build2_ms;
 } rbg_jump_info_t;
 int rbg_jump_info(const rbg_index *, rbg_jump_info_t *out);
+int rbg_jump_info_sized(const rbg_index *, rbg_jump_info_t *out, uint64_t out_bytes);
 
 int rbg_get_f(const rbg_index *, uint64_t f_out[256]);
 int rbg_last_run_sample(const rbg_index *, uint64_t *out);
@@ -430,7 +436,8 @@
        RBG_OPT_RUN_REC = 17 ,
        RBG_OPT_RUN_REC_DEPTHS = 18 ,
        RBG_OPT_EXTRACT_CHUNK = 20 ,
-       RBG_OPT_JUMP_K = 19  };
+       RBG_OPT_JUMP_K = 19 ,
+       RBG_OPT_JUMP2_K = 21  };
 int rbg_set_default_option(int opt, int64_t value);
 int rbg_get_default_option(int opt, int64_t *value);
 
diff --git a/rowbowt_amd/capi.py b/rowbowt_amd/capi.py
--- a/rowbowt_amd/capi.py
+++ b/rowbowt_amd/capi.py
@@ -17,6 +17,7 @@
 OPT_RUN_DEPTHS, OPT_RUN_PHI, OPT_RUN_REC, OPT_RUN_REC_DEPTHS = 14, 16, 17, 18
 OPT_EXTRACT_CHUNK = 20
 OPT_JUMP_K = 19
+OPT_JUMP2_K = 21
 ABI_VERSION = 3
 MAX_KMER_DEPTH = 8
 LAYOUT_AUTO, LAYOUT_SLOTS, LAYOUT_RUNS, LAYOUT_PREFER_SLOTS = 0, 1, 2, 3
@@ -59,7 +60,8 @@
 
 
 class JumpInfo(C.Structure):
-    _fields_ = [("k", U64), ("keys", U64), ("bytes", U64), ("buckets", U64), ("build_ms", C.c_double)]
+    _fields_ = [("k", U64), ("keys", U64), ("bytes", U64), ("buckets", U64), ("build_ms", C.c_double),
+                ("k2", U64), ("keys2", U64), ("bytes2", U64), ("buckets2", U64), ("build2_ms", C.c_double)]
 
 
 class ReportParams(C.Structure):
@@ -115,6 +117,7 @@
     ("rbg_info_sized", C.c_int, [VP, C.POINTER(Info), U64]),
     ("rbg_layout_info", C.c_int, [VP, C.POINTER(LayoutInfo), U64]),
     ("rbg_jump_info", C.c_int, [VP, C.POINTER(JumpInfo)]),
+    ("rbg_jump_info_sized", C.c_int, [VP, C.POINTER(JumpInfo), U64]),
     ("rbg_get_f", C.c_int, [VP, VP]),
     ("rbg_last_run_sample", C.c_int, [VP, C.POINTER(U64)]),
     ("rbg_host_array", C.c_int, [VP, C.c_int, VP, U64, C.POINTER(U64)]),
@@ -247,7 +250,7 @@
     ("rbg_get_default_option", C.c_int, [C.c_int, C.POINTER(C.c_int64)]),
 ]
 EXPORTS = [p[0] for p in _PROTOS]
-_OPTIONAL = {"rbg_jump_info"}
+_OPTIONAL = {"rbg_jump_info", "rbg_jump_info_sized"}
 
 _lib = None
 
@@ -552,7 +555,10 @@
 
     def jump_info(self):
         i = JumpInfo()
-        _check(self.L.rbg_jump_info(self.h, C.byref(i)), "rbg_jump_info")
+        if hasattr(self.L, "rbg_jump_info_sized"):
+            _check(self.L.rbg_jump_info_sized(self.h, C.byref(i), C.sizeof(i)), "rbg_jump_info_sized")
+        else:
+            _check(self.L.rbg_jump_info(self.h, C.byref(i)), "rbg_jump_info")
         return i
 
     def layout_info(self):
diff --git a/rowbowt_amd/csrc/k_jump.hip b/rowbowt_amd/csrc/k_jump.hip
--- a/rowbowt_amd/csrc/k_jump.hip
+++ b/rowbowt_amd/csrc/k_jump.hip
@@ -1,8 +1,14 @@
+#include <chrono>
+
 #include "rbg_device.hpp"
 #include "rbg_jump.h"
 
 namespace rbg {
 namespace {
+
+constexpr uint32_t kJumpWide = 0x80000000u;
+constexpr uint32_t kJumpStamp = 0x40000000u;
+inline uint64_t jump_insert_nb(uint64_t nb, uint32_t K, uint32_t K2) { return nb | (static_cast<uint64_t>(K) << 32) | (static_cast<uint64_t>(K2) << 40); }
 
 __global__ __launch_bounds__(256) void k_jump_expand(const uint64_t *__restrict__ plo, const uint64_t *__restrict__ phi, const uint64_t base,
                                                      const uint64_t cnt, const uint8_t *__restrict__ major_byte, uint64_t *__restrict__ clo,
@@ -20,6 +26,8 @@
                                                    const uint64_t base, const uint64_t N, const uint32_t level, uint64_t *__restrict__ olo,
                                                    uint64_t *__restrict__ ohi, uint4 *__restrict__ okey, unsigned long long *__restrict__ count) {
     const uint32_t lane = threadIdx.x & (kWave - 1);
+    const bool wide = (level & kJumpWide) != 0;
+    const uint32_t pos = level & 0xFFFFu;
     const uint64_t stride = static_cast<uint64_t>(gridDim.x) * blockDim.x;
     for (uint64_t wb = static_cast<uint64_t>(blockIdx.x) * blockDim.x + (threadIdx.x & ~(kWave - 1)); wb < N; wb += stride) {
         const uint64_t j = wb + lane;
@@ -30,25 +38,39 @@
         at = __shfl(at, 0);
         if (keep) {
             const uint64_t o = at + static_cast<uint64_t>(__popcll(bal & ((uint64_t(1) << lane) - 1u)));
-            uint4 kk = pkey[base + (j >> 2)];
-            JumpKey key{{kk.x, kk.y, kk.z, kk.w}};
-            jump_key_set(key, level, static_cast<uint32_t>(j & 3u));
+            const uint64_t par = base + (j >> 2);
             olo[o] = nlo[j];
             ohi[o] = nhi[j];
-            okey[o] = make_uint4(key.w[0], key.w[1], key.w[2], key.w[3]);
+            if (!wide) {
+                uint4 kk = pkey[par];
+                JumpKey key{{kk.x, kk.y, kk.z, kk.w}};
+                jump_key_set(key, pos, static_cast<uint32_t>(j & 3u));
+                okey[o] = make_uint4(key.w[0], key.w[1], key.w[2], key.w[3]);
+            } else {
+                const uint4 a = pkey[2 * par], b = pkey[2 * par + 1];
+                JumpKey ka{{a.x, a.y, a.z, a.w}}, kb{{b.x, b.y, b.z, b.w}};
+                if (pos < 64u) jump_key_set(ka, pos, static_cast<uint32_t>(j & 3u));
+                else jump_key_set(kb, pos - 64u, static_cast<uint32_t>(j & 3u));
+                if (level & kJumpStamp) kb.w[3] = static_cast<uint32_t>(nlo[j]);
+                okey[2 * o] = make_uint4(ka.w[0], ka.w[1], ka.w[2], ka.w[3]);
+                okey[2 * o + 1] = make_uint4(kb.w[0], kb.w[1], kb.w[2], kb.w[3]);
+            }
         }
     }
 }
 
 __global__ __launch_bounds__(256) void k_jump_meta(const uint64_t cnt, const uint32_t K, uint2 *__restrict__ meta) {
+    const uint32_t per = (K & kJumpWide) ? 2u : 1u, len = K & 0xFFFFu;
     const uint64_t stride = static_cast<uint64_t>(gridDim.x) * blockDim.x;
     for (uint64_t i = static_cast<uint64_t>(blockIdx.x) * blockDim.x + threadIdx.x; i < cnt; i += stride)
-        meta[i] = make_uint2(static_cast<uint32_t>(i), K);
+        meta[i] = make_uint2(static_cast<uint32_t>(per * i), len);
 }
 
 __global__ __launch_bounds__(256) void k_jump_insert(const uint4 *__restrict__ keys, const uint64_t *__restrict__ lo, const uint64_t *__restrict__ hi,
-                                                     const uint64_t *__restrict__ ss, const uint64_t cnt, uint32_t *__restrict__ tab, const uint64_t nb,
+                                                     const uint64_t *__restrict__ ss, const uint64_t cnt, uint32_t *__restrict__ tab, const uint64_t nb_k,
                                                      unsigned long long *__restrict__ inserted) {
+    const uint64_t nb = nb_k & 0xFFFFFFFFull;
+    const uint32_t K = static_cast<uint32_t>(nb_k >> 32) & 0xFFu, K2 = static_cast<uint32_t>(nb_k >> 40) & 0xFFu;
     const uint64_t stride = static_cast<uint64_t>(gridDim.x) * blockDim.x;
     for (uint64_t i = static_cast<uint64_t>(blockIdx.x) * blockDim.x + threadIdx.x; i < cnt; i += stride) {
         const uint64_t l = lo[i], h = hi[i], k = ss ? ss[i] : 0;
@@ -57,7 +79,19 @@
         if (k == ~uint64_t(0)) kk = 0xFFFFFFFFu;
         else if (k >= 0xFFFFFFF0ull) continue;
         else kk = static_cast<uint32_t>(k);
-        const uint4 kw = keys[i];
+        uint4 kw = keys[K ? 2 * i : i];
+        if (K2) {
+            const uint4 b = keys[2 * i + 1];
+            const uint32_t f[7] = {kw.x, kw.y, kw.z, kw.w, b.x, b.y, b.z};
+            const auto word = [&](const uint32_t j) {
+                uint32_t v = 0;
+#pragma unroll
+                for (uint32_t t = 0; t < 7; ++t) v = t == j ? f[t] : v;
+                return v;
+            };
+            const JumpKey k2 = jump2_key_from_codes(word, K, K2, b.w);
+            kw = make_uint4(k2.w[0], k2.w[1], k2.w[2], k2.w[3]);
+        }
         const JumpKey key{{kw.x, kw.y, kw.z, kw.w}};
         uint64_t b = jump_home(jump_hash(key), nb);
         for (uint64_t step = 0; step < nb; ++step) {
@@ -88,39 +122,50 @@
 
 constexpr uint64_t kJumpChunkParents = uint64_t(1) << 24;
 
-int launch_build_jump(const DevIndex &ix, const LaunchCfg &cfg, uint32_t K, uint64_t table_budget, uint64_t peak_budget, void **tab,
-                      uint64_t *tab_bytes, uint64_t *buckets, uint64_t *keys, const char **why, void *stream) {
+static int build_jump(const DevIndex &ix, const LaunchCfg &cfg, uint32_t K, uint64_t table_budget, uint64_t peak_budget, void **tab,
+                      uint64_t *tab_bytes, uint64_t *buckets, uint64_t *keys, const char **why, void *stream, uint32_t K2, uint64_t both_budget,
+                      JumpLevel2 *l2, bool *retry) {
     *tab = nullptr; *tab_bytes = 0; *buckets = 0; *keys = 0; *why = nullptr;
+    if (l2) *l2 = JumpLevel2{};
+    if (!l2) K2 = 0;
     if (ix.pos_bytes != 4) { *why = "8-byte positions (the table holds 4-byte states)"; return 0; }
     if (ix.layout != 2 || ix.nmajor != 4 || !ix.stage_ok) { *why = "only the staged search of the run-indexed layout over four major symbols uses it"; return 0; }
     if (K < kJumpMinK || K > kJumpMaxK) return static_cast<int>(hipErrorInvalidValue);
+    if (K2 && (K2 < kJump2MinK || K2 > kJump2MaxK)) return static_cast<int>(hipErrorInvalidValue);
     hipStream_t st = static_cast<hipStream_t>(stream);
     DevIndex plain = ix;
     plain.jump = nullptr;
     plain.jump_buckets = 0;
     plain.jump_k = 0;
+    plain.jump2_buckets = 0;
+    plain.jump2_k = 0;
+    auto again_without_level2 = [&]() { *retry = true; return 0; };
+    const bool wide = K2 != 0;
+    const uint64_t wbytes = wide ? 48 : 32, kq = wide ? 2 : 1;
+    const uint32_t wflag = wide ? kJumpWide : 0u;
     uint64_t C = kJumpChunkParents;
     while (C > (uint64_t(1) << 12) && 4 * C * 33 > peak_budget / 4) C >>= 1;
     if (4 * C * 33 + 1024 > peak_budget) { *why = "its build scratch exceeds what the HBM budget leaves"; return 0; }
     DevBuf clo, chi, nlo, nhi, sym, mb, cnt_d;
     DevBuf lv_lo[2], lv_hi[2], lv_key[2];
+    uint64_t held = 0;
     uint64_t cap[2] = {0, 0};
     hipError_t e = hipSuccess;
     auto scratch = [&]() {
-        return clo.bytes + chi.bytes + nlo.bytes + nhi.bytes + sym.bytes + 32 * (cap[0] + cap[1]);
+        return clo.bytes + chi.bytes + nlo.bytes + nhi.bytes + sym.bytes + wbytes * (cap[0] + cap[1]);
     };
     bool over = false;
     auto grow = [&](int w, uint64_t need, uint64_t used) -> hipError_t {
         if (need <= cap[w]) return hipSuccess;
         const uint64_t nc = std::max<uint64_t>(need, cap[w] + cap[w] / 2);
-        if (scratch() + 32 * nc > peak_budget) { over = true; return hipSuccess; }
+        if (held + scratch() + wbytes * nc > peak_budget) { over = true; return hipSuccess; }
         DevBuf a, b, c;
         hipError_t r = a.alloc(nc * 8);
         if (r == hipSuccess) r = b.alloc(nc * 8);
-        if (r == hipSuccess) r = c.alloc(nc * 16);
+        if (r == hipSuccess) r = c.alloc(nc * 16 * kq);
         if (r == hipSuccess && used) r = hipMemcpyAsync(a.p, lv_lo[w].p, used * 8, hipMemcpyDeviceToDevice, st);
         if (r == hipSuccess && used) r = hipMemcpyAsync(b.p, lv_hi[w].p, used * 8, hipMemcpyDeviceToDevice, st);
-        if (r == hipSuccess && used) r = hipMemcpyAsync(c.p, lv_key[w].p, used * 16, hipMemcpyDeviceToDevice, st);
+        if (r == hipSuccess && used) r = hipMemcpyAsync(c.p, lv_key[w].p, used * 16 * kq, hipMemcpyDeviceToDevice, st);
         if (r == hipSuccess) r = hipStreamSynchronize(st);
         if (r != hipSuccess) return r;
         std::swap(lv_lo[w].p, a.p); std::swap(lv_lo[w].bytes, a.bytes);
@@ -144,75 +189,148 @@
         if (e == hipSuccess) e = hipMemcpy(mb.p, inv, 256, hipMemcpyHostToDevice);
     }
     if (e == hipSuccess) e = grow(0, 1, 0);
-    if (e == hipSuccess && over) { *why = "its build scratch exceeds what the HBM budget leaves"; return 0; }
+    if (e == hipSuccess && over) {
+        if (wide) return again_without_level2();
+        *why = "its build scratch exceeds what the HBM budget leaves";
+        return 0;
+    }
     if (e == hipSuccess) {
         const uint64_t lo0 = 0, hi0 = ix.n - 1;
-        const uint4 k0 = make_uint4(0, 0, 0, 0);
+        const uint4 k0[2] = {make_uint4(0, 0, 0, 0), make_uint4(0, 0, 0, 0)};
         e = hipMemcpy(lv_lo[0].p, &lo0, 8, hipMemcpyHostToDevice);
         if (e == hipSuccess) e = hipMemcpy(lv_hi[0].p, &hi0, 8, hipMemcpyHostToDevice);
-        if (e == hipSuccess) e = hipMemcpy(lv_key[0].p, &k0, 16, hipMemcpyHostToDevice);
+        if (e == hipSuccess) e = hipMemcpy(lv_key[0].p, k0, 16 * kq, hipMemcpyHostToDevice);
     }
     if (e != hipSuccess) return static_cast<int>(e);
     uint64_t F = 1;
     int cur = 0;
-    for (uint32_t level = 0; level < K; ++level) {
-        const int nx = cur ^ 1;
-        const unsigned long long zero = 0;
-        if ((e = hipMemcpy(cnt_d.p, &zero, sizeof(zero), hipMemcpyHostToDevice)) != hipSuccess) return static_cast<int>(e);
-        uint64_t used = 0;
-        for (uint64_t base = 0; base < F; base += C) {
-            const uint64_t cnt = std::min<uint64_t>(C, F - base);
-            if ((e = grow(nx, used + 4 * cnt, used)) != hipSuccess) return static_cast<int>(e);
-            if (over) { *why = "its build scratch exceeds what the HBM budget leaves"; return 0; }
-            hipLaunchKernelGGL(k_jump_expand, dim3(grid_for(cfg, 4 * cnt)), dim3(256), 0, st, lv_lo[cur].as<uint64_t>(), lv_hi[cur].as<uint64_t>(), base, cnt,
-                               mb.as<uint8_t>(), clo.as<uint64_t>(), chi.as<uint64_t>(), sym.as<uint8_t>());
-            if ((e = hipGetLastError()) != hipSuccess) return static_cast<int>(e);
-            if (int rc = launch_lf(plain, cfg, clo.as<uint64_t>(), chi.as<uint64_t>(), sym.as<uint8_t>(), 4 * cnt, nlo.as<uint64_t>(), nhi.as<uint64_t>(), st)) return rc;
-            hipLaunchKernelGGL(k_jump_keep, dim3(grid_for(cfg, 4 * cnt)), dim3(256), 0, st, nlo.as<uint64_t>(), nhi.as<uint64_t>(), lv_key[cur].as<uint4>(), base,
-                               4 * cnt, level, lv_lo[nx].as<uint64_t>(), lv_hi[nx].as<uint64_t>(), lv_key[nx].as<uint4>(), cnt_d.as<unsigned long long>());
-            if ((e = hipGetLastError()) != hipSuccess) return static_cast<int>(e);
-            unsigned long long got = 0;
-            if ((e = hipMemcpyAsync(&got, cnt_d.p, sizeof(got), hipMemcpyDeviceToHost, st)) != hipSuccess) return static_cast<int>(e);
-            if ((e = hipStreamSynchronize(st)) != hipSuccess) return static_cast<int>(e);
-            used = got;
-        }
-        F = used;
-        cur = nx;
-        if (F == 0) break;
+    auto extend = [&](const uint32_t first, const uint32_t last) -> int {
+        for (uint32_t level = first; level < last; ++level) {
+            const int nx = cur ^ 1;
+            const unsigned long long zero = 0;
+            if ((e = hipMemcpy(cnt_d.p, &zero, sizeof(zero), hipMemcpyHostToDevice)) != hipSuccess) return static_cast<int>(e);
+            uint64_t used = 0;
+            for (uint64_t base = 0; base < F; base += C) {
+                const uint64_t cnt = std::min<uint64_t>(C, F - base);
+                if ((e = grow(nx, used + 4 * cnt, used)) != hipSuccess) return static_cast<int>(e);
+                if (over) return 0;
+                hipLaunchKernelGGL(k_jump_expand, dim3(grid_for(cfg, 4 * cnt)), dim3(256), 0, st, lv_lo[cur].as<uint64_t>(), lv_hi[cur].as<uint64_t>(), base, cnt,
+                                   mb.as<uint8_t>(), clo.as<uint64_t>(), chi.as<uint64_t>(), sym.as<uint8_t>());
+                if ((e = hipGetLastError()) != hipSuccess) return static_cast<int>(e);
+                if (int rc = launch_lf(plain, cfg, clo.as<uint64_t>(), chi.as<uint64_t>(), sym.as<uint8_t>(), 4 * cnt, nlo.as<uint64_t>(), nhi.as<uint64_t>(), st)) return rc;
+                hipLaunchKernelGGL(k_jump_keep, dim3(grid_for(cfg, 4 * cnt)), dim3(256), 0, st, nlo.as<uint64_t>(), nhi.as<uint64_t>(), lv_key[cur].as<uint4>(), base,
+                                   4 * cnt, level | wflag | (wide && level < K ? kJumpStamp : 0u), lv_lo[nx].as<uint64_t>(), lv_hi[nx].as<uint64_t>(),
+                                   lv_key[nx].as<uint4>(), cnt_d.as<unsigned long long>());
+                if ((e = hipGetLastError()) != hipSuccess) return static_cast<int>(e);
+                unsigned long long got = 0;
+                if ((e = hipMemcpyAsync(&got, cnt_d.p, sizeof(got), hipMemcpyDeviceToHost, st)) != hipSuccess) return static_cast<int>(e);
+                if ((e = hipStreamSynchronize(st)) != hipSuccess) return static_cast<int>(e);
+                used = got;
+            }
+            F = used;
+            cur = nx;
+            if (F == 0) break;
+        }
+        return 0;
+    };
+    if (int rc = extend(0, K)) return rc;
+    if (over) {
+        if (wide) return again_without_level2();
+        *why = "its build scratch exceeds what the HBM budget leaves";
+        return 0;
     }
     *keys = F;
     const uint64_t nb = jump_buckets_for(F);
     const uint64_t bytes = nb * kJumpBucketBytes;
     if (F == 0 || nb >= (uint64_t(1) << 32)) { *why = F ? "more keys than the table addresses" : "no K-mer occurs"; return 0; }
-    if (bytes > table_budget || bytes + scratch() > peak_budget) {
+    if (bytes > table_budget) {
+        *why = "the table exceeds the bytes allowed for it (what the HBM budget leaves; by default also half the replica)";
+        return 0;
+    }
+    if (bytes + scratch() > peak_budget) {
+        if (wide) return again_without_level2();
         *why = "the table exceeds the bytes allowed for it (what the HBM budget leaves; by default also half the replica)";
         return 0;
     }
     void *t = nullptr;
     if ((e = hipMalloc(&t, bytes)) != hipSuccess) { (void)hipGetLastError(); *why = "hipMalloc of the table failed"; return 0; }
-    int rc = static_cast<int>(hipMemsetAsync(t, 0, bytes, st));
-    if (!rc) rc = static_cast<int>(hipMemsetAsync(cnt_d.p, 0, sizeof(unsigned long long), st));
-    for (uint64_t base = 0; !rc && base < F; base += 4 * C) {
-        const uint64_t cnt = std::min<uint64_t>(4 * C, F - base);
-        hipLaunchKernelGGL(k_jump_meta, dim3(grid_for(cfg, cnt)), dim3(256), 0, st, cnt, K, clo.as<uint2>());
-        rc = static_cast<int>(hipGetLastError());
-        if (!rc) rc = launch_find_range_runs_packed(plain, cfg, clo.as<uint2>(), lv_key[cur].as<uint4>() + base, cnt, chi.as<uint64_t>(), nlo.as<uint64_t>(),
-                                                    ix.has_tsa ? nhi.as<uint64_t>() : nullptr, st);
-        if (!rc) {
-            hipLaunchKernelGGL(k_jump_insert, dim3(grid_for(cfg, cnt)), dim3(256), 0, st, lv_key[cur].as<uint4>() + base, chi.as<uint64_t>(), nlo.as<uint64_t>(),
-                               ix.has_tsa ? nhi.as<uint64_t>() : nullptr, cnt, static_cast<uint32_t *>(t), nb, cnt_d.as<unsigned long long>());
+    unsigned long long ins = 0;
+    auto fill = [&](void *table, const uint64_t nbt, const uint32_t len, const uint32_t k2) -> int {
+        int rc = static_cast<int>(hipMemsetAsync(table, 0, nbt * kJumpBucketBytes, st));
+        if (!rc) rc = static_cast<int>(hipMemsetAsync(cnt_d.p, 0, sizeof(unsigned long long), st));
+        for (uint64_t base = 0; !rc && base < F; base += 4 * C) {
+            const uint64_t cnt = std::min<uint64_t>(4 * C, F - base);
+            const uint4 *recs = lv_key[cur].as<uint4>() + kq * base;
+            hipLaunchKernelGGL(k_jump_meta, dim3(grid_for(cfg, cnt)), dim3(256), 0, st, cnt, len | wflag, clo.as<uint2>());
             rc = static_cast<int>(hipGetLastError());
-        }
-    }
-    unsigned long long ins = 0;
-    if (!rc) rc = static_cast<int>(hipMemcpyAsync(&ins, cnt_d.p, sizeof(ins), hipMemcpyDeviceToHost, st));
-    if (!rc) rc = static_cast<int>(hipStreamSynchronize(st));
-    if (rc) { (void)hipFree(t); return rc; }
+            if (!rc) rc = launch_find_range_runs_packed(plain, cfg, clo.as<uint2>(), recs, cnt, chi.as<uint64_t>(), nlo.as<uint64_t>(),
+                                                        ix.has_tsa ? nhi.as<uint64_t>() : nullptr, st);
+            if (!rc) {
+                hipLaunchKernelGGL(k_jump_insert, dim3(grid_for(cfg, cnt)), dim3(256), 0, st, recs, chi.as<uint64_t>(), nlo.as<uint64_t>(),
+                                   ix.has_tsa ? nhi.as<uint64_t>() : nullptr, cnt, static_cast<uint32_t *>(table), jump_insert_nb(nbt, wide ? K : 0u, k2),
+                                   cnt_d.as<unsigned long long>());
+                rc = static_cast<int>(hipGetLastError());
+            }
+        }
+        if (!rc) rc = static_cast<int>(hipMemcpyAsync(&ins, cnt_d.p, sizeof(ins), hipMemcpyDeviceToHost, st));
+        if (!rc) rc = static_cast<int>(hipStreamSynchronize(st));
+        return rc;
+    };
+    if (int rc = fill(t, nb, K, 0)) { (void)hipFree(t); return rc; }
     *tab = t;
     *tab_bytes = bytes;
     *buckets = nb;
     *keys = ins;
+    if (!wide) return 0;
+
+    const auto t2_0 = std::chrono::steady_clock::now();
+    held = bytes;
+    auto give_up = [&](const char *w) { (void)hipGetLastError(); l2->why = w; return 0; };
+    auto fail2 = [&](int err) {
+        if (err == static_cast<int>(hipErrorOutOfMemory)) return give_up("out of device memory while building it");
+        (void)hipFree(t);
+        *tab = nullptr; *tab_bytes = 0; *buckets = 0;
+        return err;
+    };
+    if (int err = extend(K, K + K2)) return fail2(err);
+    if (over) return give_up("its build scratch exceeds what the HBM budget leaves");
+    l2->keys = F;
+    const uint64_t nb2 = jump_buckets_for(F);
+    const uint64_t bytes2 = nb2 * kJumpBucketBytes;
+    if (F == 0 || nb2 >= (uint64_t(1) << 32)) return give_up(F ? "more keys than the table addresses" : "no word of K + K2 symbols occurs");
+    if (held + bytes2 > both_budget || 2 * held + bytes2 + scratch() > peak_budget)
+        return give_up("the table exceeds the bytes allowed for it (what the HBM budget leaves after the first table; by default both together at most the replica)");
+    void *tc = nullptr;
+    if (hipMalloc(&tc, bytes + bytes2) != hipSuccess) return give_up("hipMalloc of the table failed");
+    hipError_t ce = hipMemcpyAsync(tc, t, bytes, hipMemcpyDeviceToDevice, st);
+    if (ce == hipSuccess) ce = hipStreamSynchronize(st);
+    if (ce != hipSuccess) { (void)hipFree(tc); return fail2(static_cast<int>(ce)); }
+    (void)hipFree(t);
+    t = tc;
+    *tab = tc;
+    void *t2 = static_cast<char *>(tc) + bytes;
+    if (int rc = fill(t2, nb2, K + K2, K2)) {
+        (void)hipFree(t);
+        *tab = nullptr; *tab_bytes = 0; *buckets = 0;
+        return rc;
+    }
+    l2->tab = t2;
+    l2->bytes = bytes2;
+    l2->buckets = nb2;
+    l2->keys = ins;
+    l2->build_ms = std::chrono::duration<double, std::milli>(std::chrono::steady_clock::now() - t2_0).count();
     return 0;
 }
 
-}
+int launch_build_jump(const DevIndex &ix, const LaunchCfg &cfg, uint32_t K, uint64_t table_budget, uint64_t peak_budget, void **tab,
+                      uint64_t *tab_bytes, uint64_t *buckets, uint64_t *keys, const char **why, void *stream, uint32_t K2, uint64_t both_budget,
+                      JumpLevel2 *l2) {
+    bool retry = false;
+    int rc = build_jump(ix, cfg, K, table_budget, peak_budget, tab, tab_bytes, buckets, keys, why, stream, K2, both_budget, l2, &retry);
+    if (!retry) return rc;
+    rc = build_jump(ix, cfg, K, table_budget, peak_budget, tab, tab_bytes, buckets, keys, why, stream, 0, 0, nullptr, &retry);
+    l2->why = "its build scratch exceeds what the HBM budget leaves";
+    return rc;
+}
+
+}
diff --git a/rowbowt_amd/csrc/k_runs.hip b/rowbowt_amd/csrc/k_runs.hip
--- a/rowbowt_amd/csrc/k_runs.hip
+++ b/rowbowt_amd/csrc/k_runs.hip
@@ -51,6 +51,17 @@
     return state <= kJumpHit1;
 }
 
+__device__ __forceinline__ uint64_t uniform_u64(const uint64_t v) {
+    const uint32_t lo = static_cast<uint32_t>(__builtin_amdgcn_readfirstlane(static_cast<uint32_t>(v)));
+    const uint32_t hi = static_cast<uint32_t>(__builtin_amdgcn_readfirstlane(static_cast<uint32_t>(v >> 32)));
+    return static_cast<uint64_t>(lo) | (static_cast<uint64_t>(hi) << 32);
+}
+
+struct StagedWords {
+    const lds_u32 *codes;
+    __device__ __forceinline__ uint32_t operator()(const uint32_t j) const { return codes[64u * j]; }
+};
+
 template <typename P, bool TOEHOLD, bool PACKED = false, bool STATS = false, bool GLDS = false, bool STAGE = false>
 __global__ __launch_bounds__(512, STATS ? 2 : 4) void k_find_range_runs(const DevIndex ix, const void *__restrict__ src_a,
                                                         const void *__restrict__ src_b, const uint64_t N,
@@ -67,9 +78,17 @@
     __shared__ uint8_t s_mslot[4];
     __shared__ __align__(16) unsigned char s_tile[GLDS ? 8 * kTileBytes : 16];
     __shared__ uint32_t s_codes[STAGE ? 8 * kStageWords * 64 : 1];
+    __shared__ uint64_t s_jump[STAGE ? 4 : 1];
+    __shared__ uint32_t s_jump_k[STAGE ? 2 : 1];
     for (int t = threadIdx.x; t < 256; t += blockDim.x) {
         s_lut[t] = ix.lut[t];
         s_lut2[t] = ix.nmajor ? ix.lut2[t] : 0xFFu;
+    }
+    if (STAGE && threadIdx.x < 2) {
+        const uint32_t t = threadIdx.x;
+        s_jump[2 * t] = reinterpret_cast<uint64_t>(ix.jump) + (t ? ix.jump_buckets * kJumpBucketBytes : 0u);
+        s_jump[2 * t + 1] = t ? ix.jump2_buckets : ix.jump_buckets;
+        s_jump_k[t] = t ? ix.jump2_k : ix.jump_k;
     }
     RBG_RUN_SEARCH2_SHARED;
     const RunSearch2<P> S2 = stage_run_search2<P>(ix, s_tab_first, s_ent2, s_dir2, s_rec2, s_dyn);
@@ -130,18 +149,28 @@
             bool jumped = false;
             if constexpr (STAGED && sizeof(P) == 4) {
                 if (ix.jump) {
-                    const bool probing = valid && m32 >= ix.jump_k;
-                    JumpKey key{{codes[0], codes[64], codes[128], codes[192]}};
-                    jump_key_mask(key, ix.jump_k);
-                    uint32_t v[3] = {0, 0, 0}, nbk = 0;
-                    if (jump_probe_wave<GLDS>(ix.jump, ix.jump_buckets, probing, key, v, nbk, tile)) {
-                        lo = v[0]; hi = v[1];
-                        if (TOEHOLD) k = v[2] == 0xFFFFFFFFu ? ~uint64_t(0) : static_cast<uint64_t>(v[2]);
-                        p -= ix.jump_k;
-                        jumped = true;
-                        if (STATS) st[kStSymbols] += ix.jump_k;
+                    const uint32_t nlev = ix.jump2_k ? 2u : 1u;
+                    bool hit = valid;
+                    uint32_t from = 0;
+#pragma unroll 1
+                    for (uint32_t lev = 0; lev < nlev; ++lev) {
+                        const uint32_t K = __builtin_amdgcn_readfirstlane(s_jump_k[lev]);
+                        const uint64_t tab = uniform_u64(s_jump[2 * lev]), nb = uniform_u64(s_jump[2 * lev + 1]);
+                        const bool probing = hit && static_cast<uint32_t>(p) >= K;
+                        JumpKey key = jump_key_from_codes(StagedWords{codes}, from, K);
+                        if (lev) key.w[3] = static_cast<uint32_t>(lo);
+                        from = K;
+                        uint32_t v[3] = {0, 0, 0}, nbk = 0;
+                        hit = jump_probe_wave<GLDS>(reinterpret_cast<const void *>(tab), nb, probing, key, v, nbk, tile);
+                        if (hit) {
+                            lo = v[0]; hi = v[1];
+                            if (TOEHOLD) k = v[2] == 0xFFFFFFFFu ? ~uint64_t(0) : static_cast<uint64_t>(v[2]);
+                            p -= K;
+                            jumped = true;
+                            if (STATS) st[kStSymbols] += K;
+                        }
+                        if (STATS) st[kStFtab] += nbk;
                     }
-                    if (STATS) st[kStFtab] += nbk;
                 }
             }
             if (!jumped && valid && ix.ftab_k && p - beg >= ix.ftab_k) {
diff --git a/rowbowt_amd/csrc/rbg_dev.h b/rowbowt_amd/csrc/rbg_dev.h
--- a/rowbowt_amd/csrc/rbg_dev.h
+++ b/rowbowt_amd/csrc/rbg_dev.h
@@ -179,6 +179,8 @@
     const void *jump;
     uint64_t jump_buckets;
     uint32_t jump_k;
+    uint32_t jump2_k;
+    uint64_t jump2_buckets;
     uint32_t tmk_shift;
     const uint64_t *tmk_start, *tmk_end, *tmk_off, *tmk_vals;
     uint64_t tmk_nruns;
@@ -520,8 +522,15 @@
               uint64_t N, uint64_t *lo_out, uint64_t *hi_out, void *stream);
 int launch_build_ftab(const DevIndex &ix, const LaunchCfg &cfg, uint32_t k, void *tab, void *stream);
 size_t ftab_build_scratch_bytes(uint64_t words, uint32_t k);
+struct JumpLevel2 {
+    void *tab = nullptr;
+    uint64_t bytes = 0, buckets = 0, keys = 0;
+    double build_ms = 0.0;
+    const char *why = nullptr;
+};
 int launch_build_jump(const DevIndex &ix, const LaunchCfg &cfg, uint32_t K, uint64_t table_budget, uint64_t peak_budget, void **tab,
-                      uint64_t *tab_bytes, uint64_t *buckets, uint64_t *keys, const char **why, void *stream);
+                      uint64_t *tab_bytes, uint64_t *buckets, uint64_t *keys, const char **why, void *stream, uint32_t K2 = 0,
+                      uint64_t both_budget = 0, JumpLevel2 *l2 = nullptr);
 int launch_sample_reads(const uint8_t *text, uint64_t unit, uint64_t H, uint64_t L, uint64_t m, uint64_t seed, uint64_t first,
                         uint64_t N, uint32_t sub_ppm, uint8_t *seqs, uint64_t *off, uint64_t *start_out , void *stream);
 int launch_sample_reads_pg(const uint8_t *base, const uint64_t *sites, const uint8_t *alt, const uint8_t *G, uint64_t S, const uint32_t *site_dir, uint32_t site_dir_shift,
diff --git a/rowbowt_amd/csrc/rbg_jump.h b/rowbowt_amd/csrc/rbg_jump.h
--- a/rowbowt_amd/csrc/rbg_jump.h
+++ b/rowbowt_amd/csrc/rbg_jump.h
@@ -78,6 +78,41 @@
     return false;
 }
 
+constexpr uint32_t kJump2MaxK = 48;
+constexpr uint32_t kJump2MinK = 16;
+constexpr uint32_t kJump2DefaultK = 40;
+
+RBG_JUMP_HD JumpKey jump2_key(uint32_t s0, uint32_t s1, uint32_t s2, uint32_t K2, uint32_t parent_lo) {
+    JumpKey key{{s0, s1, s2, 0u}};
+    jump_key_mask(key, K2);
+    key.w[3] = parent_lo;
+    return key;
+}
+
+template <typename Word>
+RBG_JUMP_HD JumpKey jump_key_from_codes(const Word &word, uint32_t from, uint32_t K) {
+    const uint32_t w0 = from >> 4, sh = 2u * (from & 15u);
+    const uint32_t c0 = word(w0), c1 = word(w0 + 1), c2 = word(w0 + 2), c3 = word(w0 + 3), c4 = word(w0 + 4);
+    const auto funnel = [sh](uint32_t lo, uint32_t hi) { return static_cast<uint32_t>(((static_cast<uint64_t>(hi) << 32) | lo) >> sh); };
+    JumpKey key{{funnel(c0, c1), funnel(c1, c2), funnel(c2, c3), funnel(c3, c4)}};
+    jump_key_mask(key, K);
+    return key;
+}
+
+template <typename Word>
+RBG_JUMP_HD JumpKey jump2_key_from_codes(const Word &word, uint32_t K1, uint32_t K2, uint32_t parent_lo) {
+    JumpKey key = jump_key_from_codes(word, K1, K2);
+    key.w[3] = parent_lo;
+    return key;
+}
+
+RBG_JUMP_HD JumpKey jump2_key_from_text(const uint8_t *codes, uint32_t K2, uint32_t parent_lo) {
+    JumpKey key{{0, 0, 0, 0}};
+    for (uint32_t t = 0; t < K2; ++t) jump_key_set(key, t, codes[K2 - 1 - t]);
+    key.w[3] = parent_lo;
+    return key;
+}
+
 inline uint64_t jump_buckets_for(uint64_t keys) { return keys ? keys : 1; }
 
 }
diff --git a/rowbowt_amd/csrc/rbg_load_plan.hpp b/rowbowt_amd/csrc/rbg_load_plan.hpp
--- a/rowbowt_amd/csrc/rbg_load_plan.hpp
+++ b/rowbowt_amd/csrc/rbg_load_plan.hpp
@@ -349,16 +349,24 @@
 }
 inline int64_t auto_jump_k(uint64_t hbm_bytes) { return hbm_bytes > kJumpAutoMinBytes ? kJumpDefaultK : 0; }
 struct JumpBudgets {
-    uint64_t room, peak_budget, table_budget;
+    uint64_t room, peak_budget, table_budget, both_budget;
 };
 inline JumpBudgets jump_budgets(uint64_t hbm_budget, uint64_t hbm_bytes, size_t free_b, bool jump_auto) {
     JumpBudgets j;
     j.room = hbm_budget > hbm_bytes ? hbm_budget - hbm_bytes : 0;
     j.peak_budget = std::min<uint64_t>(j.room, free_b / 2);
     j.table_budget = std::min<uint64_t>(j.room, free_b / 4);
-    if (jump_auto) j.table_budget = std::min<uint64_t>(j.table_budget, hbm_bytes / 2);
+    j.both_budget = j.peak_budget;
+    if (jump_auto) {
+        j.table_budget = std::min<uint64_t>(j.table_budget, hbm_bytes / 2);
+        j.both_budget = std::min<uint64_t>(j.both_budget, hbm_bytes);
+    }
     return j;
 }
+inline int64_t jump2_k_for(int64_t opt, bool jump_auto, int64_t jk) {
+    if (opt >= 0) return opt;
+    return jump_auto && jk == static_cast<int64_t>(kJumpDefaultK) ? static_cast<int64_t>(kJump2DefaultK) : 0;
+}
 
 }
 #endif
```
